# CompVis/stable-diffusion

Hardware: AMD Instinct MI355X
Metric: 512x512 images/sec, SD-v1-4 50-step PLMS CFG=7.5 (higher is better)
Workload: dtype f16

## Files before the change

### include/sdmi.h

```cpp
#ifndef SDMI_H_
#define SDMI_H_

#include <stdint.h>

#ifdef __cplusplus
extern "C" {
#endif

#define SDMI_ABI_VERSION 17

typedef struct sdmi_unet sdmi_unet;

typedef struct sdmi_unet_cfg {
  int32_t in_channels;
  int32_t out_channels;
  int32_t model_channels;
  int32_t num_res_blocks;
  int32_t n_levels;
  int32_t channel_mult[8];
  int32_t n_attention_resolutions;
  int32_t attention_resolutions[8];
  int32_t num_heads;
  int32_t transformer_depth;
  int32_t context_dim;
// ... 87 lines not shown


typedef struct sdmi_clip sdmi_clip;
typedef struct sdmi_clip_cfg {
  int32_t vocab_size;
  int32_t hidden_size;
  int32_t intermediate_size;
  int32_t num_layers;
  int32_t num_heads;
  int32_t max_positions;
} sdmi_clip_cfg;
int sdmi_clip_create(const sdmi_clip_cfg* cfg, sdmi_clip** out);
int sdmi_clip_destroy(sdmi_clip* h);
int sdmi_clip_num_weights(const sdmi_clip* h);
int sdmi_clip_weight_info(const sdmi_clip* h, int idx, char* key_buf, int key_buf_len, int64_t* shape4, int* ndim);
int sdmi_clip_set_weight(sdmi_clip* h, const char* key, const float* ptr, const int64_t* shape, int ndim, void* stream);
int sdmi_clip_finalize(sdmi_clip* h);
int64_t sdmi_clip_workspace_bytes(sdmi_clip* h, int B, int L);
int sdmi_clip_forward(sdmi_clip* h, const int64_t* ids, float* out, int B, int L, void* workspace, int64_t workspace_bytes,
                      void* stream);

typedef struct sdmi_bert sdmi_bert;
typedef struct sdmi_bert_cfg {
  int32_t vocab_size;
  int32_t dim;
  int32_t depth;
  int32_t heads;
  int32_t dim_head;
  int32_t ff_inner;
  int32_t max_seq_len;
} sdmi_bert_cfg;
int sdmi_bert_create(const sdmi_bert_cfg* cfg, sdmi_bert** out);
int sdmi_bert_destroy(sdmi_bert* h);
int sdmi_bert_num_weights(const sdmi_bert* h);
int sdmi_bert_weight_info(const sdmi_bert* h, int idx, char* key_buf, int key_buf_len, int64_t* shape4, int* ndim);
int sdmi_bert_set_weight(sdmi_bert* h, const char* key, const float* ptr, const int64_t* shape, int ndim, void* stream);
int sdmi_bert_finalize(sdmi_bert* h);
int64_t sdmi_bert_workspace_bytes(sdmi_bert* h, int B, int L);
int sdmi_bert_forward(sdmi_bert* h, const int64_t* ids, float* out, int B, int L, void* workspace, int64_t workspace_bytes,
                      void* stream);

typedef struct sdmi_igemm_desc {
  const void* a0; const void* a1; const void* a2;
  int32_t c0, c1, c2, lda0, lda1, lda2;
  int32_t B, Hin, Win, Hout, Wout, ksize, stride, up;
  const void* w;
  int32_t N;
  int32_t mode;
  const float* bias; const float* rowvec; int32_t ld_rowvec;
  const float* residual; int32_t ldr;
  float* out_f32; void* out_f16; int32_t ldo;
  void* seg_dst[3]; int32_t seg_kind[3];
  int32_t heads, dh, ntok, ntok_pad, segC;
  int32_t splitk;
  float* splitk_ws; int64_t splitk_ws_floats;
  int32_t tile;
  int32_t dma;
  int32_t asym_pad;
  int32_t gn_n; void* gn_acc[2]; int32_t gn_cpg[2]; int32_t gn_cbase[2];
  int32_t* splitk_cnt; int32_t splitk_cnt_ints;
  int32_t split16;
  const float* f16_scale; float* lnp_out;
  const float* lnf_part; int32_t lnf_npart; float lnf_eps; const float* lnf_cs; const float* lnf_d;
  const float* pgn_gamma; const float* pgn_beta; float pgn_eps; int32_t pgn_silu;
  void* pgn_out; int32_t pgn_keep_f32; int32_t* pgn_applied;
  void* out_lo;
} sdmi_igemm_desc;
int sdmi_k_igemm(const sdmi_igemm_desc* d, void* stream);
int sdmi_k_ff_tail(const sdmi_igemm_desc* proj_out, const void* ln_f16, const float* lnp, float ln_eps, const float* csd,
                   const void* wgg_f16, const void* wff2_f16, const float* bff2, const float* t, void* stream);
int sdmi_k_st_tail(const sdmi_igemm_desc* proj_out, const void* a_f16, const void* wo_f16, const float* bo, float* t, const float* ln_gamma,
                   float ln_eps, const float* csd, const void* wgg_f16, const void* wff2_f16, const float* bff2, void* stream);
int sdmi_k_gn_conv3(const sdmi_igemm_desc* conv, const float* x0, const float* x1, int c0, int c1, float* gn_ws, int64_t gn_ws_floats,
                    const float* gn_gamma, const float* gn_beta, float gn_eps, void* stream);
int sdmi_k_st_head(const float* x, float* gn_ws, int64_t gn_ws_floats, const float* gn_gamma, const float* gn_beta, float gn_eps,
                   const void* w_in3, const float* b_in, float* t, const float* ln_gamma, float ln_eps, const void* wqkv_f16,
                   const float* lnf_cs, const float* lnf_d, void* q, void* k, void* vt, int B, int ntok, int ntok_pad, int heads, int dh,
                   int C, void* stream);
int sdmi_k_st_mid(const void* a_f16, const void* wo_f16, const float* bo, float* t, const float* ln_gamma, float ln_eps, const void* wq_f16,
                  const float* lnf_cs, const float* lnf_d, void* q, int B, int ntok, int heads, int dh, int C, void* stream);
int sdmi_k_st_mid_ctx(const void* a_f16, const void* wo_f16, const float* bo, float* t, const float* ln_gamma, float ln_eps, const void* wq_f16,
                      const float* lnf_cs, const float* lnf_d, const void* ctx_k, const void* ctx_vt, int nkv, int nkv_pad, float scale, void* ao_out,
                      int B, int ntok, int heads, int dh, int C, void* stream);
int sdmi_k_ln_fold_prep(const void* w_f16, int N, int K, int ldw, const float* gamma, const float* beta, const float* bias,
                        float* cs, float* d, void* stream);
int sdmi_k_attention(const void* q, const void* k, const void* vt, void* out, int BH, int heads, int nq, int nkv,
                     int nkv_pad, int d, float scale, void* stream);
int sdmi_k_attention_split16(const void* q, const void* q_lo, const void* k, const void* k_lo, const void* vt, const void* vt_lo, void* out,
                             void* out_lo, int BH, int heads, int nq, int nkv, int nkv_pad, int d, float scale, void* stream);
int sdmi_k_attention_causal(const void* q, const void* k, const void* vt, void* out, int BH, int heads, int n, int n_pad,
                            int d, float scale, void* stream);
int sdmi_k_groupnorm(const float* x0, const float* x1, int c0, int c1, int B, int HW, const float* gamma,
                     const float* beta, float eps, int silu, void* out_f16, float* out_f32, void* raw_f16, void* out_lo,
                     void* raw_lo, float* partial_ws, int64_t partial_floats, void* stream);
int64_t sdmi_k_groupnorm_ws_floats(int B, int HW);
int sdmi_k_groupnorm_film(const float* x0, const float* x1, int c0, int c1, int B, int HW, const float* gamma, const float* beta, float eps,
                          int silu, const float* film, int film_ld, void* out_f16, float* out_f32, void* raw_f16, void* out_lo, void* raw_lo,
                          float* partial_ws, int64_t partial_floats, void* stream);
int sdmi_k_layernorm(const float* x, const float* gamma, const float* beta, void* out_f16, int M, int C, float eps,
                     void* stream);
int sdmi_k_cast_f16(const float* x, void* out_f16, void* out_lo, int64_t n, void* stream);
int sdmi_k_split_heads(const float* src, int ld, int col0, void* dst, void* dst_lo, int kind, int B, int ntok, int ntok_pad, int heads, int dh,
                       void* stream);
int sdmi_k_geglu_split(const float* src, int M, int F, void* out, void* out_lo, void* stream);
int sdmi_k_layernorm_split(const float* x, const float* gamma, const float* beta, void* out, void* out_lo, int M, int C, float eps, void* stream);
int sdmi_k_timestep_embedding(const int64_t* t_i64, const float* t_f32, float* out, int B, int dim, void* stream);
int sdmi_k_small_linear(const float* in, int ld_in, const float* w, const float* bias, float* out, int ld_out, int B,
                        int N, int K, int silu_in, void* stream);
int sdmi_k_conv_in(const float* x_nchw, const float* w_oihw, const float* bias, float* out_nhwc, int B, int Cin, int H,
                   int W, int Cout, void* stream);
int sdmi_k_conv_out(const float* h_nhwc, const float* w_ohwi, const float* bias, float* out_nchw, int B, int H, int W,
                    int Cin, int Cout, void* stream);
int sdmi_k_pack_conv_weight(const float* w_oihw, void* dst_f16, int O, int I, int KH, int KW, void* stream);
int sdmi_k_pack_conv_weight_src(const float* w_oihw, void* dst_f16, int O, int I, int KH, int KW, int c0, int c1, int c2, void* stream);
int sdmi_k_pack_conv_out(const float* w_oihw, float* dst_ohwi, int O, int I, void* stream);
int sdmi_k_pack_split3(const float* w, void* dst_f16, int N, int K, void* stream);
int sdmi_k_pack_conv_split3(const float* w_oihw, void* dst_f16, int O, int I, int KH, int KW, void* stream);
int sdmi_k_pointwise_nchw(const float* x, const float* w, const float* bias, float* out, int B, int Cin, int Cout, int HW,
                          float in_scale, void* stream);
int sdmi_k_softmax_rows(const float* S, void* P_f16, int rows, int cols, float scale, void* stream);
int sdmi_k_vq_quantize(const float* z, float z_scale, const float* codebook, float* norms_ws, int n_embed, int D, float* zq, int32_t* idx,
                       int B, int HW, void* stream);
int sdmi_k_resample2(const float* x, float* out_f32, void* out_f16, void* out_lo, int B, int H, int W, int C, int dir, void* stream);
int sdmi_k_patch_unfold(const float* x, const float* c, float* out, int B, int Cx, int Cc, int H, int W, int kh, int kw, int sy, int sx,
                        int l0, int nl, void* stream);
int sdmi_k_patch_fold(const float* o, const float* w, float* out, int B, int C, int H, int W, int kh, int kw, int sy, int sx, int uf, int df,
                      int norm_only, void* stream);
int sdmi_k_gelu_erf(const float* x, void* out_f16, int64_t n, void* stream);
int sdmi_k_pack_geglu(const float* w, const float* bias, void* wdst_f16, float* bdst, int N, int K, void* stream);
int sdmi_image_to_uint8(const float* img_nchw, void* out_nhwc_u8, int B, int C, int H, int W, void* stream);
int sdmi_range_check(int enable);
int sdmi_range_report(char* json_buf, int json_buf_len);
int sdmi_tune_begin(void);
int sdmi_tune_round(int r);
int sdmi_tune_end(const char* path, int* n_keys);
int sdmi_tune_dump(char* buf, int buflen);
int sdmi_profile_begin(void);
int sdmi_profile_end(char* json_buf, int json_buf_len);
int sdmi_k_prefetch_lines(const void* ptr, int64_t bytes, void* stream);
const void* sdmi_zero_page(void);

#ifdef __cplusplus
}
#endif
#endif
```

### stable-diffusion_amd/_lib.py

```python
import ctypes as C
import os

_HERE = os.path.dirname(os.path.abspath(__file__))
LIB_PATH = os.environ.get('SDMI_LIB_PATH') or os.path.join(_HERE, 'libsdmi.so')

c_f32p = C.c_void_p
c_ptr = C.c_void_p


class UNetCfg(C.Structure):
    _fields_ = [('in_channels', C.c_int32), ('out_channels', C.c_int32), ('model_channels', C.c_int32),
                ('num_res_blocks', C.c_int32), ('n_levels', C.c_int32), ('channel_mult', C.c_int32 * 8),
                ('n_attention_resolutions', C.c_int32), ('attention_resolutions', C.c_int32 * 8),
                ('num_heads', C.c_int32), ('transformer_depth', C.c_int32), ('context_dim', C.c_int32)]


class VaeCfg(C.Structure):
    _fields_ = [('ch', C.c_int32), ('out_ch', C.c_int32), ('n_levels', C.c_int32), ('ch_mult', C.c_int32 * 8),
                ('num_res_blocks', C.c_int32), ('in_channels', C.c_int32), ('z_channels', C.c_int32),
                ('embed_dim', C.c_int32)]


class UNetExt(C.Structure):
    _fields_ = [('attention_block', C.c_int32), ('resblock_updown', C.c_int32)]
# ... 24 lines not shown
                ('residual', c_ptr), ('ldr', C.c_int32),
                ('out_f32', c_ptr), ('out_f16', c_ptr), ('ldo', C.c_int32),
                ('seg_dst', c_ptr * 3), ('seg_kind', C.c_int32 * 3),
                ('heads', C.c_int32), ('dh', C.c_int32), ('ntok', C.c_int32), ('ntok_pad', C.c_int32),
                ('segC', C.c_int32), ('splitk', C.c_int32), ('splitk_ws', c_ptr), ('splitk_ws_floats', C.c_int64),
                ('tile', C.c_int32), ('dma', C.c_int32), ('asym_pad', C.c_int32),
                ('gn_n', C.c_int32), ('gn_acc', c_ptr * 2), ('gn_cpg', C.c_int32 * 2), ('gn_cbase', C.c_int32 * 2),
                ('splitk_cnt', c_ptr), ('splitk_cnt_ints', C.c_int32), ('split16', C.c_int32),
                ('f16_scale', c_ptr), ('lnp_out', c_ptr), ('lnf_part', c_ptr), ('lnf_npart', C.c_int32),
                ('lnf_eps', C.c_float), ('lnf_cs', c_ptr), ('lnf_d', c_ptr),
                ('pgn_gamma', c_ptr), ('pgn_beta', c_ptr), ('pgn_eps', C.c_float), ('pgn_silu', C.c_int32),
                ('pgn_out', c_ptr), ('pgn_keep_f32', C.c_int32), ('pgn_applied', C.POINTER(C.c_int32)),
                ('out_lo', c_ptr)]


_SIGS = {
    'sdmi_last_error': (C.c_char_p, []),
    'sdmi_abi_version': (C.c_int, []),
    'sdmi_unet_create': (C.c_int, [C.POINTER(UNetCfg), C.POINTER(c_ptr)]),
    'sdmi_unet_create_with_precision': (C.c_int, [C.POINTER(UNetCfg), C.c_int, C.POINTER(c_ptr)]),
    'sdmi_unet_precision': (C.c_int, [c_ptr]),
    'sdmi_unet_create_ext': (C.c_int, [C.POINTER(UNetCfg), C.POINTER(UNetExt), C.c_int, C.POINTER(c_ptr)]),
    'sdmi_unet_create_flags': (C.c_int, [C.POINTER(UNetCfg), C.POINTER(UNetExt), C.c_uint, C.c_int, C.POINTER(c_ptr)]),
    'sdmi_unet_destroy': (C.c_int, [c_ptr]),
    'sdmi_unet_num_weights': (C.c_int, [c_ptr]),
    'sdmi_unet_weight_info': (C.c_int, [c_ptr, C.c_int, C.c_char_p, C.c_int, C.POINTER(C.c_int64), C.POINTER(C.c_int)]),
    'sdmi_unet_set_weight': (C.c_int, [c_ptr, C.c_char_p, c_ptr, C.POINTER(C.c_int64), C.c_int, c_ptr]),
    'sdmi_unet_finalize': (C.c_int, [c_ptr]),
    'sdmi_unet_packed_bytes': (C.c_int64, [c_ptr]),
    'sdmi_unet_export_packed': (C.c_int, [c_ptr, c_ptr, C.c_int64, c_ptr]),
    'sdmi_unet_import_packed': (C.c_int, [c_ptr, c_ptr, C.c_int64, c_ptr]),
    'sdmi_unet_workspace_bytes': (C.c_int64, [c_ptr, C.c_int, C.c_int, C.c_int, C.c_int]),
    'sdmi_unet_cache_context': (C.c_int, [c_ptr, c_ptr, C.c_int, C.c_int, c_ptr, C.c_int64, c_ptr]),
    'sdmi_unet_reserve_context': (C.c_int, [c_ptr, C.c_int, C.c_int]),
    'sdmi_unet_cache_timesteps': (C.c_int, [c_ptr, C.POINTER(C.c_int64), C.c_int, c_ptr]),
    'sdmi_unet_hint_timestep': (C.c_int, [c_ptr, C.c_int64]),
    'sdmi_unet_tape_stats': (C.c_int, [c_ptr, C.POINTER(C.c_int64), C.POINTER(C.c_int64)]),
    'sdmi_unet_forward': (C.c_int, [c_ptr, c_ptr, c_ptr, c_ptr, c_ptr, c_ptr, C.c_int, C.c_int, C.c_int, C.c_int,
                                    c_ptr, C.c_int64, c_ptr]),
    'sdmi_sampler_step': (C.c_int, [c_ptr, C.c_int, C.c_float, c_ptr, C.c_int, c_ptr, c_ptr, c_ptr, C.c_float,
                                    C.c_float, C.c_float, C.c_float, c_ptr, c_ptr, c_ptr, c_ptr, C.c_int64, c_ptr]),
    'sdmi_dpm_solver_step': (C.c_int, [c_ptr, C.c_int, C.c_float, c_ptr, c_ptr, C.c_float, C.c_float, C.c_float, C.c_float,
                                       C.c_float, C.c_int, c_ptr, c_ptr, C.c_int64, c_ptr]),
    'sdmi_vae_create': (C.c_int, [C.POINTER(VaeCfg), C.c_int, C.POINTER(c_ptr)]),
    'sdmi_vae_destroy': (C.c_int, [c_ptr]),
    'sdmi_vae_create_ext': (C.c_int, [C.POINTER(VaeCfg), C.POINTER(VaeExt), C.c_int, C.POINTER(c_ptr)]),
    'sdmi_vae_create_precision': (C.c_int, [C.POINTER(VaeCfg), C.POINTER(VaeExt), C.c_int, C.c_int, C.POINTER(c_ptr)]),
    'sdmi_vae_precision': (C.c_int, [c_ptr]),
    'sdmi_vae_decode_vq': (C.c_int, [c_ptr, c_ptr, C.c_float, C.c_int, c_ptr, C.c_int, C.c_int, C.c_int, c_ptr, C.c_int64, c_ptr]),
    'sdmi_k_vq_quantize': (C.c_int, [c_ptr, C.c_float, c_ptr, c_ptr, C.c_int, C.c_int, c_ptr, c_ptr, C.c_int, C.c_int, c_ptr]),
    'sdmi_k_patch_unfold': (C.c_int, [c_ptr, c_ptr, c_ptr] + [C.c_int] * 11 + [c_ptr]),
    'sdmi_k_patch_fold': (C.c_int, [c_ptr, c_ptr, c_ptr] + [C.c_int] * 11 + [c_ptr]),
    'sdmi_k_resample2': (C.c_int, [c_ptr, c_ptr, c_ptr, c_ptr, C.c_int, C.c_int, C.c_int, C.c_int, C.c_int, c_ptr]),
    'sdmi_vae_num_weights': (C.c_int, [c_ptr]),
    'sdmi_vae_weight_info': (C.c_int, [c_ptr, C.c_int, C.c_char_p, C.c_int, C.POINTER(C.c_int64), C.POINTER(C.c_int)]),
    'sdmi_vae_set_weight': (C.c_int, [c_ptr, C.c_char_p, c_ptr, C.POINTER(C.c_int64), C.c_int, c_ptr]),
    'sdmi_vae_finalize': (C.c_int, [c_ptr]),
    'sdmi_vae_decode_workspace_bytes': (C.c_int64, [c_ptr, C.c_int, C.c_int, C.c_int]),
    'sdmi_vae_decode': (C.c_int, [c_ptr, c_ptr, C.c_float, c_ptr, C.c_int, C.c_int, C.c_int, c_ptr, C.c_int64, c_ptr]),
    'sdmi_vae_encode_workspace_bytes': (C.c_int64, [c_ptr, C.c_int, C.c_int, C.c_int]),
    'sdmi_vae_encode': (C.c_int, [c_ptr, c_ptr, c_ptr, C.c_int, C.c_int, C.c_int, c_ptr, C.c_int64, c_ptr]),
    'sdmi_clip_create': (C.c_int, [C.POINTER(ClipCfg), C.POINTER(c_ptr)]),
    'sdmi_clip_destroy': (C.c_int, [c_ptr]),
    'sdmi_clip_num_weights': (C.c_int, [c_ptr]),
    'sdmi_clip_weight_info': (C.c_int, [c_ptr, C.c_int, C.c_char_p, C.c_int, C.POINTER(C.c_int64), C.POINTER(C.c_int)]),
    'sdmi_clip_set_weight': (C.c_int, [c_ptr, C.c_char_p, c_ptr, C.POINTER(C.c_int64), C.c_int, c_ptr]),
    'sdmi_clip_finalize': (C.c_int, [c_ptr]),
    'sdmi_clip_workspace_bytes': (C.c_int64, [c_ptr, C.c_int, C.c_int]),
    'sdmi_clip_forward': (C.c_int, [c_ptr, c_ptr, c_ptr, C.c_int, C.c_int, c_ptr, C.c_int64, c_ptr]),
    'sdmi_bert_create': (C.c_int, [C.POINTER(BertCfg), C.POINTER(c_ptr)]),
    'sdmi_bert_destroy': (C.c_int, [c_ptr]),
    'sdmi_bert_num_weights': (C.c_int, [c_ptr]),
    'sdmi_bert_weight_info': (C.c_int, [c_ptr, C.c_int, C.c_char_p, C.c_int, C.POINTER(C.c_int64), C.POINTER(C.c_int)]),
    'sdmi_bert_set_weight': (C.c_int, [c_ptr, C.c_char_p, c_ptr, C.POINTER(C.c_int64), C.c_int, c_ptr]),
    'sdmi_bert_finalize': (C.c_int, [c_ptr]),
    'sdmi_bert_workspace_bytes': (C.c_int64, [c_ptr, C.c_int, C.c_int]),
    'sdmi_bert_forward': (C.c_int, [c_ptr, c_ptr, c_ptr, C.c_int, C.c_int, c_ptr, C.c_int64, c_ptr]),
    'sdmi_has_experiments': (C.c_int, []),
    'sdmi_k_igemm': (C.c_int, [C.POINTER(IGemmDesc), c_ptr]),
    'sdmi_k_ff_tail': (C.c_int, [C.POINTER(IGemmDesc), c_ptr, c_ptr, C.c_float, c_ptr, c_ptr, c_ptr, c_ptr, c_ptr, c_ptr]),
    'sdmi_k_gn_conv3': (C.c_int, [C.POINTER(IGemmDesc), c_ptr, c_ptr, C.c_int, C.c_int, c_ptr, C.c_int64, c_ptr, c_ptr, C.c_float, c_ptr]),
    'sdmi_k_st_mid_ctx': (C.c_int, [c_ptr, c_ptr, c_ptr, c_ptr, c_ptr, C.c_float, c_ptr, c_ptr, c_ptr, c_ptr, c_ptr, C.c_int, C.c_int, C.c_float, c_ptr,
                                    C.c_int, C.c_int, C.c_int, C.c_int, C.c_int, c_ptr]),
    'sdmi_k_st_tail': (C.c_int, [C.POINTER(IGemmDesc), c_ptr, c_ptr, c_ptr, c_ptr, c_ptr, C.c_float, c_ptr, c_ptr, c_ptr, c_ptr, c_ptr]),
    'sdmi_k_st_mid': (C.c_int, [c_ptr, c_ptr, c_ptr, c_ptr, c_ptr, C.c_float, c_ptr, c_ptr, c_ptr, c_ptr, C.c_int, C.c_int, C.c_int, C.c_int,
                                C.c_int, c_ptr]),
    'sdmi_k_st_head': (C.c_int, [c_ptr, c_ptr, C.c_int64, c_ptr, c_ptr, C.c_float, c_ptr, c_ptr, c_ptr, c_ptr, C.c_float, c_ptr, c_ptr, c_ptr,
                                 c_ptr, c_ptr, c_ptr, C.c_int, C.c_int, C.c_int, C.c_int, C.c_int, C.c_int, c_ptr]),
    'sdmi_k_attention_split16': (C.c_int, [c_ptr, c_ptr, c_ptr, c_ptr, c_ptr, c_ptr, c_ptr, c_ptr, C.c_int, C.c_int, C.c_int, C.c_int,
                                           C.c_int, C.c_int, C.c_float, c_ptr]),
    'sdmi_k_attention_causal': (C.c_int, [c_ptr, c_ptr, c_ptr, c_ptr, C.c_int, C.c_int, C.c_int, C.c_int, C.c_int, C.c_float,
                                          c_ptr]),
    'sdmi_k_pointwise_nchw': (C.c_int, [c_ptr, c_ptr, c_ptr, c_ptr, C.c_int, C.c_int, C.c_int, C.c_int, C.c_float, c_ptr]),
    'sdmi_k_softmax_rows': (C.c_int, [c_ptr, c_ptr, C.c_int, C.c_int, C.c_float, c_ptr]),
    'sdmi_k_gelu_erf': (C.c_int, [c_ptr, c_ptr, C.c_int64, c_ptr]),
    'sdmi_k_attention': (C.c_int, [c_ptr, c_ptr, c_ptr, c_ptr, C.c_int, C.c_int, C.c_int, C.c_int, C.c_int, C.c_int,
                                   C.c_float, c_ptr]),
    'sdmi_k_groupnorm': (C.c_int, [c_ptr, c_ptr, C.c_int, C.c_int, C.c_int, C.c_int, c_ptr, c_ptr, C.c_float, C.c_int,
                                   c_ptr, c_ptr, c_ptr, c_ptr, c_ptr, c_ptr, C.c_int64, c_ptr]),
    'sdmi_k_groupnorm_ws_floats': (C.c_int64, [C.c_int, C.c_int]),
    'sdmi_k_groupnorm_film': (C.c_int, [c_ptr, c_ptr, C.c_int, C.c_int, C.c_int, C.c_int, c_ptr, c_ptr, C.c_float, C.c_int, c_ptr, C.c_int,
                                        c_ptr, c_ptr, c_ptr, c_ptr, c_ptr, c_ptr, C.c_int64, c_ptr]),
    'sdmi_k_layernorm': (C.c_int, [c_ptr, c_ptr, c_ptr, c_ptr, C.c_int, C.c_int, C.c_float, c_ptr]),
    'sdmi_k_cast_f16': (C.c_int, [c_ptr, c_ptr, c_ptr, C.c_int64, c_ptr]),
    'sdmi_k_split_heads': (C.c_int, [c_ptr, C.c_int, C.c_int, c_ptr, c_ptr, C.c_int, C.c_int, C.c_int, C.c_int, C.c_int, C.c_int,
                                     c_ptr]),
    'sdmi_k_geglu_split': (C.c_int, [c_ptr, C.c_int, C.c_int, c_ptr, c_ptr, c_ptr]),
    'sdmi_k_layernorm_split': (C.c_int, [c_ptr, c_ptr, c_ptr, c_ptr, c_ptr, C.c_int, C.c_int, C.c_float, c_ptr]),
    'sdmi_k_timestep_embedding': (C.c_int, [c_ptr, c_ptr, c_ptr, C.c_int, C.c_int, c_ptr]),
    'sdmi_k_small_linear': (C.c_int, [c_ptr, C.c_int, c_ptr, c_ptr, c_ptr, C.c_int, C.c_int, C.c_int, C.c_int,
                                      C.c_int, c_ptr]),
    'sdmi_k_conv_in': (C.c_int, [c_ptr, c_ptr, c_ptr, c_ptr, C.c_int, C.c_int, C.c_int, C.c_int, C.c_int, c_ptr]),
    'sdmi_k_conv_out': (C.c_int, [c_ptr, c_ptr, c_ptr, c_ptr, C.c_int, C.c_int, C.c_int, C.c_int, C.c_int, c_ptr]),
    'sdmi_k_pack_conv_weight': (C.c_int, [c_ptr, c_ptr, C.c_int, C.c_int, C.c_int, C.c_int, c_ptr]),
    'sdmi_k_pack_conv_weight_src': (C.c_int, [c_ptr, c_ptr, C.c_int, C.c_int, C.c_int, C.c_int, C.c_int, C.c_int, C.c_int, c_ptr]),
    'sdmi_k_pack_conv_out': (C.c_int, [c_ptr, c_ptr, C.c_int, C.c_int, c_ptr]),
    'sdmi_k_pack_split3': (C.c_int, [c_ptr, c_ptr, C.c_int, C.c_int, c_ptr]),
    'sdmi_k_pack_conv_split3': (C.c_int, [c_ptr, c_ptr, C.c_int, C.c_int, C.c_int, C.c_int, c_ptr]),
    'sdmi_k_pack_geglu': (C.c_int, [c_ptr, c_ptr, c_ptr, c_ptr, C.c_int, C.c_int, c_ptr]),
    'sdmi_k_ln_fold_prep': (C.c_int, [c_ptr, C.c_int, C.c_int, C.c_int, c_ptr, c_ptr, c_ptr, c_ptr, c_ptr, c_ptr]),
    'sdmi_image_to_uint8': (C.c_int, [c_ptr, c_ptr, C.c_int, C.c_int, C.c_int, C.c_int, c_ptr]),
    'sdmi_range_check': (C.c_int, [C.c_int]),
    'sdmi_range_report': (C.c_int, [C.c_char_p, C.c_int]),
    'sdmi_tune_begin': (C.c_int, []),
    'sdmi_tune_round': (C.c_int, [C.c_int]),
    'sdmi_tune_end': (C.c_int, [C.c_char_p, C.POINTER(C.c_int)]),
    'sdmi_tune_dump': (C.c_int, [C.c_char_p, C.c_int]),
    'sdmi_profile_begin': (C.c_int, []),
    'sdmi_profile_end': (C.c_int, [C.c_char_p, C.c_int]),
    'sdmi_k_prefetch_lines': (C.c_int, [c_ptr, C.c_int64, c_ptr]),
    'sdmi_zero_page': (c_ptr, []),
}

_lib = None


class SdmiError(RuntimeError):
    pass


def load():
    global _lib
    if _lib is None:
        if not os.path.exists(LIB_PATH):
            raise SdmiError(f'{LIB_PATH} not found: build it with `python stable-diffusion_amd/build.py` '
                            '(the MI355X path has no fallback implementation)')
        lib = C.CDLL(LIB_PATH)
        for name, (res, args) in _SIGS.items():
            fn = getattr(lib, name)
            fn.restype = res
            fn.argtypes = args
        if lib.sdmi_abi_version() != 17:
            raise SdmiError('libsdmi ABI version mismatch')
        _lib = lib
    return _lib


def exported_symbols():
    return sorted(_SIGS)


def check(rc):
    if rc != 0:
        raise SdmiError(load().sdmi_last_error().decode('utf-8', 'replace'))


# ... 8 lines not shown
```

### stable-diffusion_amd/build.py

```python
import concurrent.futures as cf
import hashlib
import os
import subprocess
import sys

HERE = os.path.dirname(os.path.abspath(__file__))
CSRC = os.path.join(HERE, 'csrc')
EXTRA = os.environ.get('SDMI_CXXFLAGS', '').split()
LIB = os.path.join(HERE, os.environ.get('SDMI_LIB_OUT', 'libsdmi.so'))
OBJ = os.path.join(HERE, 'build' if os.path.basename(LIB) == 'libsdmi.so' else 'build_' + os.path.splitext(os.path.basename(LIB))[0])
SOURCES = ['igemm_t1.hip', 'igemm_t0.hip', 'igemm_t2.hip', 'igemm_h1.hip', 'igemm_h0.hip', 'igemm_h2.hip', 'igemm.hip', 'conv3halo.hip', 'gemm_split16.hip', 'rowchain.hip', 'gnconv.hip', 'range.hip', 'attn.hip', 'attn_wide.hip', 'attn_split16.hip', 'attn_wide_split16.hip', 'split_ops.hip', 'norm.hip', 'small.hip', 'sampler.hip', 'inpaint.hip', 'patch.hip', 'weights.cpp', 'unet.cpp', 'vae.cpp', 'clip.cpp', 'bert.cpp', 'api.cpp', 'prof.cpp']
FLAGS = ['--offload-arch=gfx950', '-O3', '-std=c++17', '-fPIC', '-munsafe-fp-atomics', '-Wall', '-Wno-unused-function',
         '-Wno-unused-variable']


def _hipcc():
    for c in (os.environ.get('HIPCC'), '/opt/rocm/bin/hipcc', 'hipcc'):
        if c and (not os.path.isabs(c) or os.path.exists(c)):
            return c
    raise RuntimeError('hipcc not found')


def _stamp():
    h = hashlib.sha256()
    for root in (CSRC, os.path.join(os.path.dirname(HERE), 'include')):
        for fn in sorted(os.listdir(root)):
            with open(os.path.join(root, fn), 'rb') as f:
                h.update(fn.encode())
                h.update(f.read())
    h.update(' '.join(FLAGS + EXTRA).encode())
    return h.hexdigest()


def is_current():
    stamp_file = os.path.join(OBJ, 'stamp')
    return os.path.exists(LIB) and os.path.exists(stamp_file) and open(stamp_file).read() == _stamp()


def build(force=False, verbose=True):
    os.makedirs(OBJ, exist_ok=True)
    stamp_file = os.path.join(OBJ, 'stamp')
    if not force and is_current():
        return LIB
    hipcc = _hipcc()
    stamp_now = _stamp()

    inc_dirs = (CSRC, os.path.join(os.path.dirname(HERE), 'include'))

    def deps_hash(src):
        import re
        seen, todo, h = set(), [os.path.join(CSRC, src)], hashlib.sha256()
        while todo:
            path = todo.pop()
            if path in seen:
                continue
            seen.add(path)
            with open(path, 'rb') as f:
                data = f.read()
            h.update(os.path.basename(path).encode())
            h.update(data)
            for inc in re.findall(rb'^\s*#\s*include\s*"([^"]+)"', data, re.M):
                for d in (os.path.dirname(path),) + inc_dirs:
                    cand = os.path.join(d, inc.decode())
                    if os.path.exists(cand):
                        todo.append(os.path.normpath(cand))
                        break
        return h.hexdigest()

    def compile_one(src):
        obj = os.path.join(OBJ, os.path.splitext(src)[0] + '.o')
        extra = ['-ffp-contract=off'] if src == 'sampler.hip' else []
        cmd = [hipcc] + FLAGS + EXTRA + extra + (['-x', 'hip'] if src.endswith('.hip') else []) + ['-c', os.path.join(CSRC, src), '-o', obj]
        key = hashlib.sha256((deps_hash(src) + ' '.join(cmd)).encode()).hexdigest()
        if not force and os.path.exists(obj) and os.path.exists(obj + '.key') and open(obj + '.key').read() == key:
            return obj
        r = subprocess.run(cmd, capture_output=True, text=True)
        if r.returncode != 0:
            raise RuntimeError(f'hipcc failed for {src}:\n{r.stdout}\n{r.stderr}')
        if verbose and r.stderr.strip():
            print(r.stderr, file=sys.stderr)
        with open(obj + '.key', 'w') as f:
            f.write(key)
        return obj

    with cf.ThreadPoolExecutor(max_workers=min(8, len(SOURCES))) as ex:
        objs = list(ex.map(compile_one, SOURCES))
    cmd = [hipcc, '--offload-arch=gfx950', '-shared', '-fPIC', '-o', LIB] + objs
    r = subprocess.run(cmd, capture_output=True, text=True)
    if r.returncode != 0:
        raise RuntimeError(f'link failed:\n{r.stdout}\n{r.stderr}')
    with open(stamp_file, 'w') as f:
        f.write(stamp_now)
    if verbose:
        print(f'built {LIB} ({os.path.getsize(LIB) / 1e6:.1f} MB)')
# ... 6 lines not shown
```

### stable-diffusion_amd/csrc/api.cpp

```cpp
#include <string.h>

#include <new>

#include "prof.h"
#include "split16.h"
#include "unet.h"
#include "vae.h"
#include "clip.h"

namespace sdmi {
static thread_local std::string g_err;
void set_error(const std::string& msg) { g_err = msg; }
int fail(const std::string& msg) { g_err = msg; return -1; }
}

struct sdmi_unet { sdmi::UNet impl; };
struct sdmi_vae { sdmi::Vae impl; };
struct sdmi_clip { sdmi::ClipText impl; };
struct sdmi_bert { sdmi::BertText impl; };

using namespace sdmi;

static int weight_info(const WeightStore& w, int idx, char* key_buf, int key_buf_len, int64_t* shape4, int* ndim) {
  SDMI_CHECK(key_buf && shape4 && ndim, "null argument");
// ... 319 lines not shown
  p.pgn_out = (f16*)d->pgn_out; p.pgn_keep_f32 = d->pgn_keep_f32; p.pgn_applied = d->pgn_applied;
  p.out_lo = (f16*)d->out_lo;
  return zero_page(&p.zero_page);
}
int sdmi_k_igemm(const sdmi_igemm_desc* d, void* stream) {
  SDMI_CHECK(d, "null descriptor");
  IGemmParams p = IGemmParams();
  if (igemm_params_of(d, p)) return -1;
  IGemmTune t; t.tile = d->tile; t.dma = d->dma;
  return launch_igemm(p, t, (hipStream_t)stream);
}
int sdmi_k_ff_tail(const sdmi_igemm_desc* proj_out, const void* ln_f16, const float* lnp, float ln_eps, const float* csd,
                   const void* wgg_f16, const void* wff2_f16, const float* bff2, const float* t, void* stream) {
  SDMI_CHECK(proj_out, "null descriptor");
  FfTailParams q = FfTailParams();
  if (igemm_params_of(proj_out, q.epi)) return -1;
  SDMI_CHECK(proj_out->split16 && proj_out->ksize == 1, "ff_tail: the proj_out descriptor is a split-fp16 1x1 (w = sdmi_k_pack_split3)");
  q.ln = (const f16*)ln_f16; q.lnp = lnp; q.ln_eps = ln_eps; q.csd = csd; q.wgg = (const f16*)wgg_f16; q.wff2 = (const f16*)wff2_f16;
  q.bff2 = bff2; q.t = t; q.wpo = (const f16*)proj_out->w;
  return launch_ff_tail(q, (hipStream_t)stream);
}
int sdmi_k_st_tail(const sdmi_igemm_desc* proj_out, const void* a_f16, const void* wo_f16, const float* bo, float* t, const float* ln_gamma,
                   float ln_eps, const float* csd, const void* wgg_f16, const void* wff2_f16, const float* bff2, void* stream) {
  SDMI_CHECK(proj_out && a_f16, "null argument");
  FfTailParams q = FfTailParams();
  if (igemm_params_of(proj_out, q.epi)) return -1;
  SDMI_CHECK(proj_out->split16 && proj_out->ksize == 1, "st_tail: the proj_out descriptor is a split-fp16 1x1 (w = sdmi_k_pack_split3)");
  q.a16 = (const f16*)a_f16; q.wo = (const f16*)wo_f16; q.bo = bo; q.ln_gamma = ln_gamma; q.ln_eps = ln_eps; q.csd = csd;
  q.wgg = (const f16*)wgg_f16; q.wff2 = (const f16*)wff2_f16; q.bff2 = bff2; q.t = t; q.wpo = (const f16*)proj_out->w;
  return launch_ff_tail(q, (hipStream_t)stream);
}
int sdmi_k_gn_conv3(const sdmi_igemm_desc* conv, const float* x0, const float* x1, int c0, int c1, float* gn_ws, int64_t gn_ws_floats,
                    const float* gn_gamma, const float* gn_beta, float gn_eps, void* stream) {
  SDMI_CHECK(conv && x0 && gn_ws && gn_gamma && gn_beta, "gn_conv3: null argument");
  GnConvParams q = GnConvParams();
  if (igemm_params_of(conv, q.epi)) return -1;
  const int B = q.epi.B;
  SDMI_CHECK(gn_ws_floats >= gn_acc_words(B) * 2, "groupnorm workspace too small");
  SDMI_HIP_OK(hipMemsetAsync(gn_ws, 0, gn_acc_words(B) * sizeof(long long), (hipStream_t)stream));
  GroupNormParams g = GroupNormParams();
  g.x0 = x0; g.c0 = c0; g.x1 = x1; g.c1 = c1; g.B = B; g.HW = q.epi.Hout * q.epi.Wout; g.gamma = gn_gamma; g.beta = gn_beta; g.eps = gn_eps;
  g.stats_only = 1; g.acc = (long long*)gn_ws;
  if (launch_groupnorm(g, (hipStream_t)stream)) return -1;
  q.x0 = x0; q.x1 = x1; q.c0 = c0; q.c1 = c1; q.gn_acc = (const long long*)gn_ws; q.gn_gamma = gn_gamma; q.gn_beta = gn_beta; q.gn_eps = gn_eps;
  q.w = (const f16*)conv->w;
  return launch_gn_conv3(q, (hipStream_t)stream);
}
int sdmi_k_st_head(const float* x, float* gn_ws, int64_t gn_ws_floats, const float* gn_gamma, const float* gn_beta, float gn_eps,
                   const void* w_in3, const float* b_in, float* t, const float* ln_gamma, float ln_eps, const void* wqkv_f16,
                   const float* lnf_cs, const float* lnf_d, void* q, void* k, void* vt, int B, int ntok, int ntok_pad, int heads, int dh,
                   int C, void* stream) {
  SDMI_CHECK(x && gn_ws && gn_gamma && gn_beta, "st_head: null argument");
  SDMI_CHECK(gn_ws_floats >= gn_acc_words(B) * 2, "groupnorm workspace too small");
  SDMI_HIP_OK(hipMemsetAsync(gn_ws, 0, gn_acc_words(B) * sizeof(long long), (hipStream_t)stream));
  GroupNormParams g = GroupNormParams();
  g.x0 = x; g.c0 = C; g.B = B; g.HW = ntok; g.gamma = gn_gamma; g.beta = gn_beta; g.eps = gn_eps; g.stats_only = 1; g.acc = (long long*)gn_ws;
  if (launch_groupnorm(g, (hipStream_t)stream)) return -1;
  StHeadParams p = StHeadParams();
  p.x = x; p.gn_acc = (const long long*)gn_ws; p.gn_gamma = gn_gamma; p.gn_beta = gn_beta; p.gn_eps = gn_eps;
  p.w_in = (const f16*)w_in3; p.b_in = b_in; p.t = t; p.ln_gamma = ln_gamma; p.ln_eps = ln_eps; p.wqkv = (const f16*)wqkv_f16;
  p.lnf_cs = lnf_cs; p.lnf_d = lnf_d; p.q = (f16*)q; p.k = (f16*)k; p.vt = (f16*)vt;
  p.M = B * ntok; p.B = B; p.ntok = ntok; p.ntok_pad = ntok_pad; p.heads = heads; p.dh = dh; p.C = C;
  return launch_st_head(p, (hipStream_t)stream);
}
int sdmi_k_st_mid(const void* a_f16, const void* wo_f16, const float* bo, float* t, const float* ln_gamma, float ln_eps, const void* wq_f16,
                  const float* lnf_cs, const float* lnf_d, void* q, int B, int ntok, int heads, int dh, int C, void* stream) {
  StHeadParams p = StHeadParams();
  p.a16 = (const f16*)a_f16; p.w_in = (const f16*)wo_f16; p.b_in = bo; p.t = t; p.ln_gamma = ln_gamma; p.ln_eps = ln_eps;
  p.wqkv = (const f16*)wq_f16; p.lnf_cs = lnf_cs; p.lnf_d = lnf_d; p.q = (f16*)q;
  p.M = B * ntok; p.B = B; p.ntok = ntok; p.ntok_pad = ntok; p.heads = heads; p.dh = dh; p.C = C;
  return launch_st_mid(p, (hipStream_t)stream);
}
int sdmi_k_st_mid_ctx(const void* a_f16, const void* wo_f16, const float* bo, float* t, const float* ln_gamma, float ln_eps, const void* wq_f16,
                      const float* lnf_cs, const float* lnf_d, const void* ctx_k, const void* ctx_vt, int nkv, int nkv_pad, float scale, void* ao_out,
                      int B, int ntok, int heads, int dh, int C, void* stream) {
  StHeadParams p = StHeadParams();
  p.a16 = (const f16*)a_f16; p.w_in = (const f16*)wo_f16; p.b_in = bo; p.t = t; p.ln_gamma = ln_gamma; p.ln_eps = ln_eps;
  p.wqkv = (const f16*)wq_f16; p.lnf_cs = lnf_cs; p.lnf_d = lnf_d;
  p.ctx_k = (const f16*)ctx_k; p.ctx_vt = (const f16*)ctx_vt; p.ctx_nkv = nkv; p.ctx_nkv_pad = nkv_pad; p.ctx_scale = scale; p.ao_out = (f16*)ao_out;
  SDMI_CHECK(ctx_k && ctx_vt && ao_out, "st_mid_ctx: null argument");
  p.M = B * ntok; p.B = B; p.ntok = ntok; p.ntok_pad = ntok; p.heads = heads; p.dh = dh; p.C = C;
  return launch_st_mid(p, (hipStream_t)stream);
}
int sdmi_k_ln_fold_prep(const void* w_f16, int N, int K, int ldw, const float* gamma, const float* beta, const float* bias,
                        float* cs, float* d, void* stream) {
  return launch_ln_fold_prep((const f16*)w_f16, N, K, ldw, gamma, beta, bias, cs, d, (hipStream_t)stream);
}
int sdmi_k_attention(const void* q, const void* k, const void* vt, void* out, int BH, int heads, int nq, int nkv,
                     int nkv_pad, int d, float scale, void* stream) {
  AttnParams a = AttnParams();
  a.q = (const f16*)q; a.k = (const f16*)k; a.vt = (const f16*)vt; a.out = (f16*)out;
  a.BH = BH; a.heads = heads; a.nq = nq; a.nkv = nkv; a.nkv_pad = nkv_pad; a.d = d; a.scale = scale;
  if (const char* e = getenv("SDMI_ATTN_NW")) a.nw = atoi(e);
  return launch_attention(a, (hipStream_t)stream);
}
int sdmi_k_attention_split16(const void* q, const void* q_lo, const void* k, const void* k_lo, const void* vt, const void* vt_lo, void* out,
                             void* out_lo, int BH, int heads, int nq, int nkv, int nkv_pad, int d, float scale, void* stream) {
  AttnSplitParams a = AttnSplitParams();
  a.q = (const f16*)q; a.q_lo = (const f16*)q_lo; a.k = (const f16*)k; a.k_lo = (const f16*)k_lo; a.vt = (const f16*)vt;
  a.vt_lo = (const f16*)vt_lo; a.out = (f16*)out; a.out_lo = (f16*)out_lo;
  a.BH = BH; a.heads = heads; a.nq = nq; a.nkv = nkv; a.nkv_pad = nkv_pad; a.d = d; a.scale = scale;
  return launch_attention_split16(a, (hipStream_t)stream);
}
int64_t sdmi_k_groupnorm_ws_floats(int B, int HW) { (void)HW; return gn_acc_words(B) * 2; }
int sdmi_k_groupnorm(const float* x0, const float* x1, int c0, int c1, int B, int HW, const float* gamma,
                     const float* beta, float eps, int silu, void* out_f16, float* out_f32, void* raw_f16, void* out_lo,
                     void* raw_lo, float* partial_ws, int64_t partial_floats, void* stream) {
  SDMI_CHECK(partial_floats >= gn_acc_words(B) * 2, "groupnorm workspace too small");
  SDMI_HIP_OK(hipMemsetAsync(partial_ws, 0, gn_acc_words(B) * sizeof(long long), (hipStream_t)stream));
  GroupNormParams g = GroupNormParams();
  g.x0 = x0; g.x1 = x1; g.c0 = c0; g.c1 = c1; g.B = B; g.HW = HW; g.gamma = gamma; g.beta = beta; g.eps = eps;
  g.silu = silu; g.out_f16 = (f16*)out_f16; g.out_f32 = out_f32; g.raw_f16 = (f16*)raw_f16; g.out_lo = (f16*)out_lo; g.raw_lo = (f16*)raw_lo;
  g.acc = (long long*)partial_ws;
  return launch_groupnorm(g, (hipStream_t)stream);
}
int sdmi_k_groupnorm_film(const float* x0, const float* x1, int c0, int c1, int B, int HW, const float* gamma, const float* beta, float eps,
                          int silu, const float* film, int film_ld, void* out_f16, float* out_f32, void* raw_f16, void* out_lo, void* raw_lo,
                          float* partial_ws, int64_t partial_floats, void* stream) {
  SDMI_CHECK(partial_floats >= gn_acc_words(B) * 2, "groupnorm workspace too small");
  SDMI_HIP_OK(hipMemsetAsync(partial_ws, 0, gn_acc_words(B) * sizeof(long long), (hipStream_t)stream));
  GroupNormParams g = GroupNormParams();
  g.x0 = x0; g.x1 = x1; g.c0 = c0; g.c1 = c1; g.B = B; g.HW = HW; g.gamma = gamma; g.beta = beta; g.eps = eps;
  g.silu = silu; g.out_f16 = (f16*)out_f16; g.out_f32 = out_f32; g.raw_f16 = (f16*)raw_f16; g.out_lo = (f16*)out_lo; g.raw_lo = (f16*)raw_lo;
  g.film = film; g.film_ld = film_ld;
  g.acc = (long long*)partial_ws;
  return launch_groupnorm(g, (hipStream_t)stream);
}
int sdmi_k_layernorm(const float* x, const float* gamma, const float* beta, void* out_f16, int M, int C, float eps,
                     void* stream) {
  return launch_layernorm(x, gamma, beta, (f16*)out_f16, M, C, eps, (hipStream_t)stream);
}
int sdmi_k_cast_f16(const float* x, void* out_f16, void* out_lo, int64_t n, void* stream) {
  return launch_cast_f16(x, (f16*)out_f16, (f16*)out_lo, n, (hipStream_t)stream);
}
int sdmi_k_split_heads(const float* src, int ld, int col0, void* dst, void* dst_lo, int kind, int B, int ntok, int ntok_pad, int heads, int dh,
                       void* stream) {
  return launch_split_heads(src, ld, col0, (f16*)dst, (f16*)dst_lo, kind, B, ntok, ntok_pad, heads, dh, (hipStream_t)stream);
}
int sdmi_k_geglu_split(const float* src, int M, int F, void* out, void* out_lo, void* stream) {
  return launch_geglu_split(src, M, F, (f16*)out, (f16*)out_lo, (hipStream_t)stream);
}
int sdmi_k_layernorm_split(const float* x, const float* gamma, const float* beta, void* out, void* out_lo, int M, int C, float eps, void* stream) {
  return launch_layernorm_split(x, gamma, beta, (f16*)out, (f16*)out_lo, M, C, eps, (hipStream_t)stream);
}
int sdmi_k_timestep_embedding(const int64_t* t_i64, const float* t_f32, float* out, int B, int dim, void* stream) {
  return launch_timestep_embedding(t_i64, t_f32, out, B, dim, (hipStream_t)stream);
}
int sdmi_k_small_linear(const float* in, int ld_in, const float* w, const float* bias, float* out, int ld_out, int B,
                        int N, int K, int silu_in, void* stream) {
  return launch_small_linear(in, ld_in, w, bias, out, ld_out, B, N, K, silu_in, (hipStream_t)stream);
}
int sdmi_k_conv_in(const float* x, const float* w, const float* bias, float* out, int B, int Cin, int H, int W, int Cout,
                   void* stream) {
  return launch_conv_in(x, w, bias, out, B, Cin, H, W, Cout, (hipStream_t)stream);
}
int sdmi_k_conv_out(const float* h, const float* w, const float* bias, float* out, int B, int H, int W, int Cin, int Cout,
                    void* stream) {
  return launch_conv_out(h, w, bias, out, B, H, W, Cin, Cout, (hipStream_t)stream);
}
int sdmi_k_pack_conv_weight(const float* w, void* dst, int O, int I, int KH, int KW, void* stream) {
  return launch_pack_conv_weight(w, (f16*)dst, O, I, KH, KW, (hipStream_t)stream);
}
int sdmi_k_pack_conv_weight_src(const float* w, void* dst, int O, int I, int KH, int KW, int c0, int c1, int c2, void* stream) {
  return launch_pack_conv_weight_src(w, (f16*)dst, O, I, KH, KW, c0, c1, c2, (hipStream_t)stream);
}
int sdmi_k_pack_conv_out(const float* w, float* dst, int O, int I, void* stream) {
// ... 55 lines not shown
```

### stable-diffusion_amd/csrc/common.h

```cpp
#pragma once
#include <hip/hip_runtime.h>
#include <stdint.h>
#include <algorithm>
#include <string>

#include "tape.h"

typedef _Float16 f16;
typedef _Float16 f16x2 __attribute__((ext_vector_type(2)));
typedef _Float16 f16x4 __attribute__((ext_vector_type(4)));
typedef _Float16 f16x8 __attribute__((ext_vector_type(8)));
typedef float f32x4 __attribute__((ext_vector_type(4)));
typedef float f32x16 __attribute__((ext_vector_type(16)));

#ifdef __HIPCC__
__device__ __forceinline__ float gn_apply_elem(float v, float mean, float rstd, float gamma, float beta, int silu) {
  float t = __builtin_fmaf((v - mean) * rstd, gamma, beta);
  if (silu) t = t * __builtin_amdgcn_rcpf(1.0f + __expf(-t));
  return t;
}
__device__ __forceinline__ float gn_apply_film_elem(float v, float mean, float rstd, float gamma, float beta, float scale, float shift,
                                                    int silu) {
  float t = __builtin_fmaf((v - mean) * rstd, gamma, beta);
  t = __builtin_fmaf(t, 1.0f + scale, shift);
// ... 135 lines not shown
  unsigned long long gn_magic[2] = {0, 0};
  const float* pgn_gamma = nullptr; const float* pgn_beta = nullptr; float pgn_eps = 1e-5f; int pgn_silu = 1;
  f16* pgn_out = nullptr;
  int pgn_keep_f32 = 0;
  int* pgn_applied = nullptr;
  unsigned long long magic_hw = 0, magic_w = 0, magic_w2 = 0;
  int log2w = 0;
  const float* xf0 = nullptr; const float* xf1 = nullptr;
  const long long* gn_in_acc = nullptr;
  const float* gn_in_gamma = nullptr; const float* gn_in_beta = nullptr; float gn_in_eps = 1e-5f; int gn_in_silu = 1;
  f16* raw_hi = nullptr; f16* raw_lo = nullptr;
  f16* gn_scratch = nullptr;
  unsigned long long magic_cpg_in = 0;
  int halo_thi = 0, halo_ipt = 1, log2_tpi = 30;
  unsigned long long magic_hpi = 0;
};

constexpr int SDMI_NUM_TILES = 22;
struct IGemmTune {
  int tile = -1;
  int dma = -1;
};

int launch_igemm(const IGemmParams& p, const IGemmTune& tune, hipStream_t stream);
bool range_check_enabled();
uint64_t tune_generation();
bool tune_collecting();
int range_check_set(int enable);
int range_scan(const char* what, const f16* p, int64_t n, hipStream_t stream);
int range_report(std::string* json);

int tune_begin();
int tune_round(int r);
int tune_end(const char* path, int* n_keys);
int tune_dump(std::string* out);
int launch_splitk_reduce(const IGemmParams& p, int nsplit, hipStream_t stream);

struct FfTailParams {
  const f16* ln = nullptr;
  const float* lnp = nullptr;
  float ln_eps = 1e-5f;
  const float* csd = nullptr;
  const f16* wgg = nullptr;
  const f16* wff2 = nullptr;
  const float* bff2 = nullptr;
  const float* t = nullptr;
  const f16* wpo = nullptr;
  const f16* a16 = nullptr;
  const f16* wo = nullptr;
  const float* bo = nullptr;
  const float* ln_gamma = nullptr;
#ifdef SDMI_RC_TIMING
  long long* dbg = nullptr;
#endif
  IGemmParams epi;
};
bool ff_tail_supported(int C, int M, int rows_per_sample);
int launch_ff_tail(const FfTailParams& p, hipStream_t stream);

struct StHeadParams {
  const f16* a16 = nullptr;
  const float* x = nullptr;
  const long long* gn_acc = nullptr;
  const float* gn_gamma = nullptr; const float* gn_beta = nullptr; float gn_eps = 1e-6f;
  const f16* w_in = nullptr;
  const float* b_in = nullptr;
  float* t = nullptr;
  const float* ln_gamma = nullptr;
  float ln_eps = 1e-5f;
  const f16* wqkv = nullptr;
  const float* lnf_cs = nullptr; const float* lnf_d = nullptr;
  f16* q = nullptr; f16* k = nullptr;
  f16* vt = nullptr;
  int M = 0, B = 0, ntok = 0, ntok_pad = 0, heads = 0, dh = 0, C = 0;
  const f16* ctx_k = nullptr; const f16* ctx_vt = nullptr; int ctx_nkv = 0, ctx_nkv_pad = 0; float ctx_scale = 0.f; f16* ao_out = nullptr;
#ifdef SDMI_RC_TIMING
  long long* dbg = nullptr;
#endif
};
bool st_head_supported(int C, int M, int ntok, int ntok_pad, int heads, int dh);
int launch_st_head(const StHeadParams& p, hipStream_t stream);
int launch_st_mid(const StHeadParams& p, hipStream_t stream);

struct GnConvParams {
  const float* x0 = nullptr; const float* x1 = nullptr; int c0 = 0, c1 = 0;
  const long long* gn_acc = nullptr;
  const float* gn_gamma = nullptr; const float* gn_beta = nullptr; float gn_eps = 1e-5f;
  const f16* w = nullptr;
#ifdef SDMI_RC_TIMING
  long long* dbg = nullptr;
#endif
  IGemmParams epi;
};
bool gn_conv3_supported(int B, int H, int W, int c0, int c1, int Cout);
int launch_gn_conv3(const GnConvParams& p, hipStream_t stream);

struct AttnParams {
  const f16* q = nullptr;
  const f16* k = nullptr;
  const f16* vt = nullptr;
  f16* out = nullptr;
  int BH = 0, heads = 0, nq = 0, nkv = 0, nkv_pad = 0, d = 0;
  float scale = 1.f;
  int nw = 0;
  int causal = 0;
  int prio = 0;
  int pingpong = 0;
};
int launch_attention(const AttnParams& p, hipStream_t stream);
int launch_attention_wide(const AttnParams& p, hipStream_t stream);

struct GroupNormParams {
  const float* x0 = nullptr; const float* x1 = nullptr; int c0 = 0, c1 = 0;
  int B = 0, HW = 0;
  const float* gamma = nullptr; const float* beta = nullptr; float eps = 1e-5f;
  int silu = 0;
  int stats_only = 0;
  int skip_stats = 0;
  f16* out_f16 = nullptr;
  float* out_f32 = nullptr;
  f16* raw_f16 = nullptr;
  f16* out_lo = nullptr;
  f16* raw_lo = nullptr;
  const float* film = nullptr; int film_ld = 0;
  long long* acc = nullptr;
};
constexpr int GN_SLOTS = 8;
constexpr int GN_MAX_CALLS = 96;
constexpr int GN_WORDS = 4;
constexpr int GN_STRIDE = 16;
static inline int64_t gn_acc_words(int B) { return (int64_t)B * 32 * GN_SLOTS * GN_STRIDE; }
int launch_groupnorm(const GroupNormParams& p, hipStream_t stream);

int launch_layernorm(const float* x, const float* gamma, const float* beta, f16* out, int M, int C, float eps,
                     hipStream_t stream, float* out_f32 = nullptr);
int launch_cast_f16(const float* x, f16* out, f16* out_lo, int64_t n, hipStream_t stream);

int launch_timestep_embedding(const int64_t* t_i64, const float* t_f32, float* out, int B, int dim, hipStream_t s);
int launch_small_linear(const float* in, int ld_in, const float* w, const float* bias, float* out, int ld_out,
                        int B, int N, int K, int silu_in, hipStream_t s);
int launch_ctx1_broadcast(const f16* vt, int ld_v, f16* ao, int B, int ntok, int C, hipStream_t s);
int launch_conv_in(const float* x_nchw, const float* w, const float* bias, float* out_nhwc, int B, int Cin, int H,
                   int W, int Cout, hipStream_t s, int gn_n = 0, long long* const* gn_acc = nullptr, const int* gn_cpg = nullptr,
                   const int* gn_cbase = nullptr);
int launch_conv_out(const float* h_nhwc, const float* w_khwc, const float* bias, float* out_nchw, int B, int H, int W,
                    int Cin, int Cout, hipStream_t s);

struct DpmStepParams {
  const float* eps_model = nullptr;
  int cfg = 0; float scale = 1.f;
  const float* x = nullptr;
  const float* m_prev = nullptr;
  float alpha_s = 1.f, sigma_s = 0.f;
  float cx = 1.f, a = 0.f, inv_r0 = 0.f;
  int order = 1;
  float* m_out = nullptr;
  float* x_next = nullptr;
  int64_t n = 0;
};
int launch_dpm_step(const DpmStepParams& p, hipStream_t s);

int launch_embed_tokens(const int64_t* ids, const float* tok_emb, const float* pos_emb, float* out, int M, int L, int C,
                        int vocab, hipStream_t s);
int launch_quick_gelu(const float* x, f16* out, int64_t n, hipStream_t s);
int launch_gelu_erf(const float* x, f16* out, int64_t n, hipStream_t s);

// ... 43 lines not shown
```

### stable-diffusion_amd/csrc/igemm_dev.h

```cpp
#pragma once
#include "common.h"
#include "prof.h"

namespace sdmi {
typedef unsigned u32x4 __attribute__((ext_vector_type(4)));

int launch_splitk_reduce(const IGemmParams& p, int nsplit, hipStream_t stream);
int launch_generic_tile_g0(int tile, const IGemmParams& p, bool dma, int splitk, hipStream_t stream);
int launch_generic_tile_g1(int tile, const IGemmParams& p, bool dma, int splitk, hipStream_t stream);
int launch_generic_tile_g2(int tile, const IGemmParams& p, bool dma, int splitk, hipStream_t stream);
int launch_generic_tile_h0(int tile, const IGemmParams& p, bool dma, int splitk, hipStream_t stream);
int launch_generic_tile_h1(int tile, const IGemmParams& p, bool dma, int splitk, hipStream_t stream);
int launch_generic_tile_h2(int tile, const IGemmParams& p, bool dma, int splitk, hipStream_t stream);

static int env_int(const char* name, int dflt) {
  const char* v = getenv(name);
  return v ? atoi(v) : dflt;
}

namespace {

constexpr int BK = 64;
constexpr int BKH = 32;
static inline int src_chunks(int c) { return (c + BK - 1) / BK; }
// ... 23 lines not shown
#define SDMI_VMCNT_CASE(k) case k: asm volatile("s_waitcnt vmcnt(" #k ")" ::: "memory"); break
    SDMI_VMCNT_CASE(0); SDMI_VMCNT_CASE(1); SDMI_VMCNT_CASE(2); SDMI_VMCNT_CASE(3); SDMI_VMCNT_CASE(4);
    SDMI_VMCNT_CASE(5); SDMI_VMCNT_CASE(6); SDMI_VMCNT_CASE(7); SDMI_VMCNT_CASE(8); SDMI_VMCNT_CASE(9);
    SDMI_VMCNT_CASE(10); SDMI_VMCNT_CASE(11); SDMI_VMCNT_CASE(12); SDMI_VMCNT_CASE(13); SDMI_VMCNT_CASE(14);
    SDMI_VMCNT_CASE(15); SDMI_VMCNT_CASE(16); SDMI_VMCNT_CASE(17); SDMI_VMCNT_CASE(18); SDMI_VMCNT_CASE(19);
    SDMI_VMCNT_CASE(20); SDMI_VMCNT_CASE(21); SDMI_VMCNT_CASE(22); SDMI_VMCNT_CASE(23); SDMI_VMCNT_CASE(24);
    SDMI_VMCNT_CASE(25); SDMI_VMCNT_CASE(26); SDMI_VMCNT_CASE(27); SDMI_VMCNT_CASE(28); SDMI_VMCNT_CASE(29);
    SDMI_VMCNT_CASE(30); SDMI_VMCNT_CASE(31); SDMI_VMCNT_CASE(32); SDMI_VMCNT_CASE(33); SDMI_VMCNT_CASE(34);
    SDMI_VMCNT_CASE(35); SDMI_VMCNT_CASE(36); SDMI_VMCNT_CASE(37); SDMI_VMCNT_CASE(38); SDMI_VMCNT_CASE(39);
    SDMI_VMCNT_CASE(40); SDMI_VMCNT_CASE(41); SDMI_VMCNT_CASE(42); SDMI_VMCNT_CASE(43); SDMI_VMCNT_CASE(44);
    SDMI_VMCNT_CASE(45); SDMI_VMCNT_CASE(46); SDMI_VMCNT_CASE(47); SDMI_VMCNT_CASE(48);
#undef SDMI_VMCNT_CASE
    default: __builtin_trap();
  }
}
template <int N>
__device__ __forceinline__ void wait_vmcnt() {
  static_assert(N >= 0 && N <= 48, "add the literal");
  wait_vmcnt_n(N);
}

enum : int { KIND_1X1 = 0, KIND_3X3 = 1, KIND_3X3_UP = 2 };

__device__ __forceinline__ int fast_div(int m, unsigned long long magic) {
  return (int)(((unsigned long long)(unsigned)m * magic) >> 40);
}
__device__ __forceinline__ int fast_div_hw(int m, unsigned long long magic) {
  return (int)(((unsigned long long)(unsigned)m * magic) >> 48);
}

#if defined(__HIP_DEVICE_COMPILE__)
template <int WTN> constexpr int SLAB_LPR = WTN / 4;
template <int WTN> constexpr int SLAB_RPI = 64 / (WTN / 4);
template <int WTN> constexpr int SLAB_NPASS = 32 / (64 / (WTN / 4));
template <int NWAVES, int WTN, int LDS_BYTES>
constexpr int SLAB_LSTR = (NWAVES * 32 * (WTN + 4) * 4 <= LDS_BYTES) ? WTN + 4 : WTN;
template <int NWAVES, int WTN, int LDS_BYTES>
__device__ __forceinline__ float* slab_base(unsigned char* smem, int wave) {
  static_assert(WTN == 32 || WTN == 64, "lane mapping of the 16-byte epilogue");
  static_assert(NWAVES * 32 * SLAB_LSTR<NWAVES, WTN, LDS_BYTES> * 4 <= LDS_BYTES, "LDS too small for the epilogue slabs");
  return (float*)smem + wave * (32 * SLAB_LSTR<NWAVES, WTN, LDS_BYTES>);
}
template <int TN, int LSTR>
__device__ __forceinline__ void slab_put(float* wl, const f32x16 (&a)[TN], int l31, int lg) {
#pragma unroll
  for (int j = 0; j < TN; ++j)
#pragma unroll
    for (int r = 0; r < 16; ++r) wl[((r & 3) + 8 * (r >> 2) + 4 * lg) * LSTR + j * 32 + l31] = a[j][r];
  asm volatile("s_waitcnt lgkmcnt(0)" ::: "memory");
}
template <int TN, int LSTR>
__device__ __forceinline__ void slab_get(const float* wl, f32x16 (&a)[TN], int l31, int lg) {
  asm volatile("s_waitcnt lgkmcnt(0)" ::: "memory");
#pragma unroll
  for (int j = 0; j < TN; ++j)
#pragma unroll
    for (int r = 0; r < 16; ++r) a[j][r] = wl[((r & 3) + 8 * (r >> 2) + 4 * lg) * LSTR + j * 32 + l31];
  asm volatile("s_waitcnt lgkmcnt(0)" ::: "memory");
}

constexpr int LNF_MAXP = 40;
__device__ __forceinline__ void lnf_request(const IGemmParams& p, int m, float2 (&pv)[LNF_MAXP]) {
  const float2* src = (const float2*)p.lnf_part + m;
#pragma unroll
  for (int j = 0; j < 20; ++j) pv[j] = src[(size_t)min(j, p.lnf_npart - 1) * p.M];
  if (p.lnf_npart > 20) {
#pragma unroll
    for (int j = 20; j < LNF_MAXP; ++j) pv[j] = src[(size_t)min(j, p.lnf_npart - 1) * p.M];
  } else {
#pragma unroll
    for (int j = 20; j < LNF_MAXP; ++j) pv[j] = float2{0.f, 0.f};
  }
}
__device__ __forceinline__ void lnf_finish(const IGemmParams& p, const float2 (&pv)[LNF_MAXP], float* mean, float* rstd) {
  float s = 0.f, q = 0.f;
#pragma unroll
  for (int j = 0; j < LNF_MAXP; ++j)
    if (j < p.lnf_npart) { s += pv[j].x; q += pv[j].y; }
  const float inv_c = 1.0f / (32.0f * (float)p.lnf_npart);
  const float mu = s * inv_c;
  const float var = fmaxf(q * inv_c - mu * mu, 0.f);
  *mean = mu;
  *rstd = 1.0f / sqrtf(var + p.lnf_eps);
}
__device__ __forceinline__ float sum8_dpp(float v) {
  v += __builtin_bit_cast(float, __builtin_amdgcn_update_dpp(0, __builtin_bit_cast(int, v), 0xB1, 0xF, 0xF, true));
  v += __builtin_bit_cast(float, __builtin_amdgcn_update_dpp(0, __builtin_bit_cast(int, v), 0x4E, 0xF, 0xF, true));
  v += __builtin_bit_cast(float, __builtin_amdgcn_update_dpp(0, __builtin_bit_cast(int, v), 0x141, 0xF, 0xF, true));
  return v;
}

template <int BM, int BN, int WARPS_M, int WARPS_N, int LDS_BYTES>
__device__ __forceinline__ void igemm_epilogue(const IGemmParams& p_arg, f32x16 (&acc)[BM / WARPS_M / 32][BN / WARPS_N / 32],
                                               const int m0, const int n0, const int split, const int tile_m,
                                               const int tile_n, unsigned char* smem, const float lnf_mean = 0.f,
                                               const float lnf_rstd = 1.f) {
#ifdef SDMI_IGEMM_TIMING
  IGemmParams p = p_arg;
  if (p.dbg_abl & 1) p.residual = nullptr;
  if (p.dbg_abl & 4) { p.out_f32 = nullptr; p.out_f16 = nullptr; p.out_lo = nullptr; }
#else
  const IGemmParams& p = p_arg;
#endif
  constexpr int NT = WARPS_M * WARPS_N * 64;
  constexpr int WTM = BM / WARPS_M, WTN = BN / WARPS_N;
  constexpr int TM = WTM / 32, TN = WTN / 32;
  constexpr int LSTR = SLAB_LSTR<WARPS_M * WARPS_N, WTN, LDS_BYTES>;
  const int tid = threadIdx.x;
  const int lane = tid & 63;
  const int wave = tid >> 6;
  const int wm = wave / WARPS_N, wn = wave - wm * WARPS_N;
  const int l31 = lane & 31, lg = lane >> 5;
  const int HWout = p.Hout * p.Wout;
  const int mw = m0 + wm * WTM, nw = n0 + wn * WTN;
  const bool full = (m0 + BM <= p.M) && (n0 + BN <= p.N);
  if (p.splitk > 1 && p.splitk_fused) {
    constexpr int SC1 = 16;
    const int tile_lin = tile_m * ((p.N + BN - 1) / BN) + tile_n;
    const __amdgpu_buffer_rsrc_t ws = __builtin_amdgcn_make_buffer_rsrc(
        (void*)(p.splitk_ws + (size_t)tile_lin * p.splitk * (BM * BN)), 0, p.splitk * (BM * BN) * 4, 0x00020000);
    const int my_off = (split * (BM * BN) + tid * 4) * 4;
#pragma unroll
    for (int i = 0; i < TM; ++i)
#pragma unroll
      for (int j = 0; j < TN; ++j)
#pragma unroll
        for (int r4 = 0; r4 < 4; ++r4) {
          const f32x4 v = {acc[i][j][4 * r4], acc[i][j][4 * r4 + 1], acc[i][j][4 * r4 + 2], acc[i][j][4 * r4 + 3]};
          __builtin_amdgcn_raw_buffer_store_b128(__builtin_bit_cast(u32x4, v), ws, my_off + ((i * TN + j) * 4 + r4) * (NT * 16), 0, SC1);
        }
    asm volatile("s_waitcnt vmcnt(0)" ::: "memory");
    __syncthreads();
    if (tid == 0) *(volatile int*)smem = __hip_atomic_fetch_add(p.splitk_cnt + tile_lin, 1, __ATOMIC_RELAXED, __HIP_MEMORY_SCOPE_AGENT);
    __syncthreads();
    const int ticket = *(volatile int*)smem;
    if (ticket != p.splitk - 1) return;
    if (tid == 0) __hip_atomic_store(p.splitk_cnt + tile_lin, 0, __ATOMIC_RELAXED, __HIP_MEMORY_SCOPE_AGENT);
#pragma unroll
    for (int i = 0; i < TM; ++i)
#pragma unroll
      for (int j = 0; j < TN; ++j)
#pragma unroll
        for (int r = 0; r < 16; ++r) acc[i][j][r] = 0.f;
    constexpr int QPS = TM * TN * 4;
    constexpr int SB = QPS >= 16 ? 1 : 16 / QPS;
    for (int s0 = 0; s0 < p.splitk; s0 += SB) {
      f32x4 v[SB][QPS];
#pragma unroll
      for (int ss = 0; ss < SB; ++ss) {
        const int off = (min(s0 + ss, p.splitk - 1) * (BM * BN) + tid * 4) * 4;
#pragma unroll
        for (int e = 0; e < QPS; ++e)
          v[ss][e] = __builtin_bit_cast(f32x4, __builtin_amdgcn_raw_buffer_load_b128(ws, off + e * (NT * 16), 0, SC1));
      }
#pragma unroll
      for (int ss = 0; ss < SB; ++ss) {
        if (s0 + ss < p.splitk) {
#pragma unroll
          for (int i = 0; i < TM; ++i)
#pragma unroll
            for (int j = 0; j < TN; ++j)
#pragma unroll
              for (int r4 = 0; r4 < 4; ++r4)
#pragma unroll
                for (int e = 0; e < 4; ++e) acc[i][j][4 * r4 + e] += v[ss][(i * TN + j) * 4 + r4][e];
        }
      }
    }
    __syncthreads();
  }
  if (p.splitk > 1 && !p.splitk_fused && p.slab_tiled) {
    constexpr int SC1 = 16;
    const int tiles_n_all = (p.N + BN - 1) / BN, ntiles = ((p.M + BM - 1) / BM) * tiles_n_all;
    const int tile_lin = tile_m * tiles_n_all + tile_n;
    const __amdgpu_buffer_rsrc_t ws = __builtin_amdgcn_make_buffer_rsrc(
        (void*)(p.splitk_ws + ((size_t)split * ntiles + tile_lin) * (size_t)(BM * BN)), 0, BM * BN * 4, 0x00020000);
#pragma unroll
    for (int i = 0; i < TM; ++i)
#pragma unroll
      for (int j = 0; j < TN; ++j)
#pragma unroll
        for (int r4 = 0; r4 < 4; ++r4) {
          const f32x4 v = {acc[i][j][4 * r4], acc[i][j][4 * r4 + 1], acc[i][j][4 * r4 + 2], acc[i][j][4 * r4 + 3]};
          __builtin_amdgcn_raw_buffer_store_b128(__builtin_bit_cast(u32x4, v), ws, (tid * 4 + ((i * TN + j) * 4 + r4) * (NT * 4)) * 4, 0, SC1);
        }
    return;
  }
  if (p.lnf_part) {
    __syncthreads();
    float2* const tab = (float2*)smem;
    if (tid < BM) tab[tid] = float2{lnf_mean, lnf_rstd};
    __syncthreads();
#pragma unroll
    for (int j = 0; j < TN; ++j) {
      const int n = min(nw + j * 32 + l31, p.N - 1);
      const float cs = p.lnf_cs[n], dn = p.lnf_d[n];
#pragma unroll
      for (int i = 0; i < TM; ++i)
#pragma unroll
        for (int r = 0; r < 16; ++r) {
          const float2 mr = tab[wm * WTM + i * 32 + (r & 3) + 8 * (r >> 2) + 4 * lg];
          acc[i][j][r] = fmaf(mr.y, acc[i][j][r] - mr.x * cs, dn);
        }
    }
    __syncthreads();
  }
  const bool unfused_split = p.splitk > 1 && !p.splitk_fused;
  if (p.mode == EPI_PLAIN) {
    const bool atomic = unfused_split;
    float* slab = atomic ? (p.splitk_ws + (size_t)split * p.M * p.N) : nullptr;
    const int b_first = m0 / HWout;
    const bool one_batch = ((m0 + BM - 1) / HWout == b_first);
    if (full && one_batch && p.epi_vec && !atomic) {
      __syncthreads();
      float* const wl = slab_base<WARPS_M * WARPS_N, WTN, LDS_BYTES>(smem, wave);
      const int rl = lane / SLAB_LPR<WTN>, c4 = (lane % SLAB_LPR<WTN>) * 4;
      f32x4 colv = {0.f, 0.f, 0.f, 0.f};
      if (p.bias) colv = *(const f32x4*)(p.bias + nw + c4);
      if (p.rowvec) colv += *(const f32x4*)(p.rowvec + (size_t)b_first * p.ld_rowvec + nw + c4);
      f32x4 g4 = {1.f, 1.f, 1.f, 1.f};
      if (p.f16_scale) g4 = *(const f32x4*)(p.f16_scale + nw + c4);
#pragma unroll
      for (int i = 0; i < TM; ++i) {
        slab_put<TN, LSTR>(wl, acc[i], l31, lg);
        constexpr int NP = SLAB_NPASS<WTN>, RPI = SLAB_RPI<WTN>;
        f32x4 resv[NP];
        if (p.residual) {
#pragma unroll
          for (int q = 0; q < NP; ++q)
            resv[q] = *(const f32x4*)(p.residual + (size_t)(mw + i * 32 + q * RPI + rl) * p.ldr + nw + c4);
        } else {
#pragma unroll
          for (int q = 0; q < NP; ++q) resv[q] = f32x4{0.f, 0.f, 0.f, 0.f};
        }
#pragma unroll
        for (int q = 0; q < NP; ++q) {
          const int row = q * RPI + rl;
          float* const lp = wl + row * LSTR + c4;
          const f32x4 v = *(const f32x4*)lp + colv + resv[q];
          const size_t ro = (size_t)(mw + i * 32 + row) * p.ldo + nw + c4;
          if (p.out_f32) SDMI_ST_F32X4(p.out_f32, ro, v);
          const f32x4 vs = v * g4;
          const f16x4 h = {(f16)vs[0], (f16)vs[1], (f16)vs[2], (f16)vs[3]};
          if (p.out_f16) SDMI_ST_F16X4(p.out_f16, ro, h);
          if (p.out_lo)
            *(f16x4*)(p.out_lo + ro) = f16x4{(f16)(v[0] - (float)h[0]), (f16)(v[1] - (float)h[1]), (f16)(v[2] - (float)h[2]),
                                            (f16)(v[3] - (float)h[3])};
          if (p.lnp_out) {
            float s1 = (v[0] + v[1]) + (v[2] + v[3]);
            float s2 = (v[0] * v[0] + v[1] * v[1]) + (v[2] * v[2] + v[3] * v[3]);
            s1 = sum8_dpp(s1); s2 = sum8_dpp(s2);
            if ((lane & 7) == 0)
              *(float2*)(p.lnp_out + 2 * ((size_t)((nw + c4) >> 5) * p.M + (size_t)(mw + i * 32 + row))) = float2{s1, s2};
          }
          if (p.gn_n > 0) *(f32x4*)lp = v;
        }
        if (p.gn_n > 0) slab_get<TN, LSTR>(wl, acc[i], l31, lg);
        else asm volatile("s_waitcnt lgkmcnt(0)" ::: "memory");
      }
    } else if (full && one_batch) {
      if (atomic) {
#pragma unroll
        for (int i = 0; i < TM; ++i)
#pragma unroll
          for (int r = 0; r < 16; ++r) {
            float* row = slab + (size_t)(mw + i * 32 + (r & 3) + 8 * (r >> 2) + 4 * lg) * p.N + nw + l31;
#pragma unroll
            for (int j = 0; j < TN; ++j) row[j * 32] = acc[i][j][r];
          }
      } else {
        float colv[TN];
#pragma unroll
        for (int j = 0; j < TN; ++j) {
          const int n = nw + j * 32 + l31;
          colv[j] = p.bias ? p.bias[n] : 0.f;
          if (p.rowvec) colv[j] += p.rowvec[(size_t)b_first * p.ld_rowvec + n];
        }
#pragma unroll
        for (int i = 0; i < TM; ++i) {
          float resv[16][TN];
          if (p.residual) {
#pragma unroll
            for (int r = 0; r < 16; ++r) {
              const float* row = p.residual + (size_t)(mw + i * 32 + (r & 3) + 8 * (r >> 2) + 4 * lg) * p.ldr + nw + l31;
#pragma unroll
// ... 322 lines not shown
```

### stable-diffusion_amd/csrc/rowchain.hip

```cpp
#include <utility>

#include "igemm_dev.h"

namespace sdmi {
namespace {

constexpr int RC_ROWS = 32;
constexpr int RC_NWC = 5;
constexpr int RC_NTC = RC_NWC * 64;
constexpr int RC_UROWS = 160;
constexpr int RC_UNIT = RC_UROWS * 128;
constexpr int RC_UPIECES = RC_UNIT / 1024;
constexpr int RC_NS = 4;
constexpr int RC_NLD_DEFAULT = 2;
#ifndef SDMI_RC_PFD
#define SDMI_RC_PFD 24
#endif
constexpr int RC_PFD = SDMI_RC_PFD;
#if defined(__HIP_DEVICE_COMPILE__)
__device__ __forceinline__ int rc_pf_row(int lane, int* sector) {
  const int ntiles = gridDim.x, bid = blockIdx.x;
  const bool ok = (ntiles & 7) == 0;
  const int nslots = ok ? max(ntiles >> 3, 10) : 1, slot = ok ? (bid >> 3) : 1;
  const int idx = slot + (lane >> 2) * nslots;
  *sector = (lane & 3) * 32;
  return (slot < nslots && idx < 160) ? 64 * (idx >> 5) + (idx & 31) : -1;
}
#endif

constexpr int FT_C = 320, FT_KT = FT_C / 64, FT_HID = 4 * FT_C, FT_NCHUNK = 4;
constexpr int FT_BLK = 2 * FT_KT;
constexpr int FT_NU = (3 * FT_NCHUNK) * FT_BLK + 2 * FT_BLK;
constexpr int FT_NUH = FT_NU + FT_BLK;
struct FtUnitTab {
  int soff[FT_NUH];
  int sel[FT_NUH];
  int aux[FT_NUH];
};
constexpr FtUnitTab ft_make_tab() {
  FtUnitTab t{};
  int u = 0;
  for (int i = 0; i < FT_NUH; ++i) t.aux[i] = -1;
  for (int kt = 0; kt < FT_KT; ++kt)
    for (int half = 0; half < 2; ++half) { t.soff[u] = (32 * half) * (FT_C * 2) + kt * 128; t.sel[u] = 3; ++u; }
  for (int h = 0; h <= FT_NCHUNK; ++h) {
    if (h < FT_NCHUNK) {
      for (int pass = 0; pass < 2; ++pass) {
        if (pass == 1 && h + 1 < FT_NCHUNK) t.aux[u] = h + 1;
        for (int kt = 0; kt < FT_KT; ++kt)
          for (int half = 0; half < 2; ++half) { t.soff[u] = (2 * FT_C * h + FT_C * pass + 32 * half) * (FT_C * 2) + kt * 128; t.sel[u] = 0; ++u; }
      }
    } else {
      t.aux[u] = -2;
    }
    if (h >= 1)
      for (int kt = 0; kt < FT_KT; ++kt)
        for (int half = 0; half < 2; ++half) { t.soff[u] = (32 * half) * (FT_HID * 2) + (FT_C * (h - 1) + 64 * kt) * 2; t.sel[u] = 1; ++u; }
  }
  for (int kt = 0; kt < FT_KT; ++kt)
    for (int half = 0; half < 2; ++half)
      for (int lo = 0; lo < 2; ++lo) { t.soff[u] = (32 * half) * (3 * FT_C * 2) + (64 * kt + (lo ? 2 * FT_C : 0)) * 2; t.sel[u] = 2; ++u; }
  return t;
}
__device__ const FtUnitTab kFtTab = ft_make_tab();

#if defined(__HIP_DEVICE_COMPILE__)
__device__ __forceinline__ int strip_off(int row, int col) {
  return (col >> 6) * (RC_ROWS * 128) + row * 128 + (((((col & 63) >> 3)) ^ ((row >> 1) & 7)) << 4) + (col & 7) * 2;
}
template <int... I, class F>
__device__ __forceinline__ void rc_static_for_impl(std::integer_sequence<int, I...>, F&& f) { (f(std::integral_constant<int, I>{}), ...); }
template <int N, class F>
__device__ __forceinline__ void rc_static_for(F&& f) { rc_static_for_impl(std::make_integer_sequence<int, N>{}, f); }
#endif

template <int C, int NLD, int ABL = 0, int NS = RC_NS, bool HEAD = false, bool PF = false>
__global__ void __launch_bounds__(RC_NTC + 64 * NLD + (PF ? 64 : 0)) ff_tail_kernel(const FfTailParams rp) {
#if defined(__HIP_DEVICE_COMPILE__)
  static_assert(C == FT_C, "unit geometry: five waves x 64 columns = C; the unit table is generated for it");
  constexpr int KT = C / 64;
  constexpr int XBYTES = RC_ROWS * C * 2;
  constexpr int HID = 4 * C, NCHUNK = HID / C;
  constexpr int NU = HEAD ? FT_NUH : FT_NU;
  constexpr int TB = HEAD ? 0 : FT_BLK;
// ... 270 lines not shown
    zero2(accA);
    block(OFF_XA, accA[0], accA[1], [&](auto uc) {
      if constexpr (HEAD && decltype(uc)::value == 0) { if (h == 0) ln_table(); }
      if (h > 0) geglu_rows(uc, accB[0], accB[1], h - 1, 1);
    });
    zero2(accB);
    block(OFF_XA, accB[0], accB[1], [&](auto uc) { geglu_rows(uc, accA[0], accA[1], h, 0); });
    if (h > 0) block(OFF_XG + ((h - 1) & 1) * XBYTES, acc2[0], acc2[1], [&](auto uc) { if (h == NCHUNK - 1) geglu_rows(uc, accB[0], accB[1], h, 1); });
  }
  float T[2][16], bff[2];
#pragma unroll
  for (int j = 0; j < 2; ++j) {
    const int col = wave * 64 + j * 32 + l31;
    bff[j] = rp.bff2[col];
#pragma unroll
    for (int r = 0; r < 16; ++r) T[j][r] = rp.t[(size_t)(m0 + (r & 3) + 8 * (r >> 2) + 4 * lg) * C + col];
  }
  block(OFF_XG + ((NCHUNK - 1) & 1) * XBYTES, acc2[0], acc2[1], no_carry);
  wait_vmcnt<0>();
  if constexpr (ABL != 1) {
#pragma unroll
    for (int j = 0; j < 2; ++j) {
      const int col = wave * 64 + j * 32 + l31;
#pragma unroll
      for (int r = 0; r < 16; ++r) {
        const int row = (r & 3) + 8 * (r >> 2) + 4 * lg;
        const float v = acc2[j][r] + bff[j] + T[j][r];
        const f16 hi = (f16)v;
        const int o = strip_off(row, col);
        *(f16*)(smem + OFF_XA + o) = hi;
        *(f16*)(smem + OFF_XG + o) = (f16)(v - (float)hi);
      }
    }
  }
  RC_STAMP();
  f32x16 acc[1][2];
  zero2(acc[0]);
  rc_static_for<KT>([&](auto ktc) {
    constexpr int kt = decltype(ktc)::value;
    f16x8 ah[4], al[4];
    rc_static_for<2>([&](auto hc) {
      constexpr int half = decltype(hc)::value;
      f16x8 bh[4], bl[4];
      unit_sync();
      if constexpr (ABL != 1) {
#pragma unroll
        for (int ks = 0; ks < 4; ++ks) bh[ks] = frag(cur * RC_UNIT + b_frag, ks);
        if constexpr (half == 0) {
#pragma unroll
          for (int ks = 0; ks < 4; ++ks) {
            ah[ks] = frag(OFF_XA + kt * (RC_ROWS * 128) + a_frag, ks);
            al[ks] = frag(OFF_XG + kt * (RC_ROWS * 128) + a_frag, ks);
          }
        }
      }
      unit_end();
      unit_sync();
      if constexpr (ABL != 1) {
#pragma unroll
        for (int ks = 0; ks < 4; ++ks) bl[ks] = frag(cur * RC_UNIT + b_frag, ks);
#pragma unroll
        for (int ks = 0; ks < 4; ++ks) {
          acc[0][half] = __builtin_amdgcn_mfma_f32_32x32x16_f16(ah[ks], bh[ks], acc[0][half], 0, 0, 0);
          acc[0][half] = __builtin_amdgcn_mfma_f32_32x32x16_f16(al[ks], bh[ks], acc[0][half], 0, 0, 0);
          acc[0][half] = __builtin_amdgcn_mfma_f32_32x32x16_f16(ah[ks], bl[ks], acc[0][half], 0, 0, 0);
        }
      }
      unit_end();
    });
    RC_STAMP();
  });
  asm volatile("s_waitcnt lgkmcnt(0)\n\ts_barrier" ::: "memory");
  RC_STAMP();
  igemm_epilogue<RC_ROWS, C, 1, RC_NWC, RING>(ep, acc, m0, 0, 0, (int)blockIdx.x, 0, smem);
#ifdef SDMI_RC_TIMING
  RC_STAMP();
  __syncthreads();
  if (rp.dbg && tid < 128) rp.dbg[(size_t)blockIdx.x * 128 + tid] = tid < n_stamp ? ((const long long*)(smem + OFF_DBG))[tid] : 0;
#endif
#endif
}


typedef float f32x2 __attribute__((ext_vector_type(2)));
#if defined(__HIP_DEVICE_COMPILE__)
__device__ __forceinline__ void rc_swap_halves(float& a, float& b) {
  asm volatile("s_nop 1\n\tv_permlane32_swap_b32 %0, %1\n\ts_nop 1" : "+v"(a), "+v"(b));
}
__device__ __forceinline__ float rc_max_across_halves(float x) {
  float a = x, b = x;
  rc_swap_halves(a, b);
  return fmaxf(a, b);
}
#endif
constexpr int SH_NU = 2 * FT_BLK + 3 * FT_BLK;
struct ShUnitTab { int soff[2][SH_NU]; int sel[2][SH_NU]; };
constexpr ShUnitTab sh_make_tab() {
  ShUnitTab t{};
  int u = 0;
  for (int kt = 0; kt < FT_KT; ++kt)
    for (int half = 0; half < 2; ++half)
      for (int lo = 0; lo < 2; ++lo) { t.soff[0][u] = (32 * half) * (3 * FT_C * 2) + (64 * kt + (lo ? 2 * FT_C : 0)) * 2; t.sel[0][u] = 0; ++u; }
  for (int b = 0; b < 3; ++b)
    for (int kt = 0; kt < FT_KT; ++kt)
      for (int half = 0; half < 2; ++half) { t.soff[0][u] = (FT_C * b + 32 * half) * (FT_C * 2) + kt * 128; t.sel[0][u] = 1; ++u; }
  u = 0;
  for (int b = 0; b < 2; ++b)
    for (int kt = 0; kt < FT_KT; ++kt)
      for (int half = 0; half < 2; ++half) { t.soff[1][u] = (32 * half) * (FT_C * 2) + kt * 128; t.sel[1][u] = b; ++u; }
  for (; u < SH_NU; ++u) { t.soff[1][u] = t.soff[1][2 * FT_BLK - 1]; t.sel[1][u] = 1; }
  return t;
}
__device__ const ShUnitTab kShTab = sh_make_tab();

template <int C, int NLD, int KIND, int NS = RC_NS, bool PF = false, bool CTX = false>
__global__ void __launch_bounds__(RC_NTC + 64 * NLD + (PF ? 64 : 0)) st_head_kernel(const StHeadParams rp) {
#if defined(__HIP_DEVICE_COMPILE__)
  static_assert(C == FT_C, "unit geometry: five waves x 64 columns = C");
  static_assert(NLD == 1 || NLD == 2, "loader waves");
  constexpr int KT = C / 64;
  constexpr int XBYTES = RC_ROWS * C * 2;
  constexpr int NU = KIND == 0 ? SH_NU : 2 * FT_BLK;
  constexpr int NU1 = KIND == 0 ? 2 * FT_BLK : FT_BLK;
  constexpr int RING = NS * RC_UNIT;
  constexpr int OFF_XH = RING, OFF_XL = OFF_XH + XBYTES, OFF_XN = OFF_XL + XBYTES;
  constexpr int OFF_GTAB = OFF_XN + XBYTES;
  constexpr int OFF_LTAB = OFF_GTAB + 32 * 8;
  constexpr int OFF_LNP = OFF_LTAB + RC_ROWS * 8;
  constexpr int OFF_PF = OFF_LNP + RC_ROWS * (C / 32) * 8;
  constexpr int LDS_TOTAL = OFF_PF + (PF ? 256 : 0);
  constexpr int LSTR = 64;
  static_assert(RC_NWC * 32 * LSTR * 4 <= 2 * XBYTES, "the epilogue slabs live in the (dead) proj_in operand strips");
  constexpr int LPIECES = RC_UPIECES / NLD, LD_WAIT = LPIECES * (NS - 2);
  static_assert(NS >= 3 && LD_WAIT + LPIECES <= 63 && LD_WAIT <= 48, "vmcnt is a 6-bit counter");
#ifdef SDMI_RC_TIMING
  constexpr int OFF_DBG = LDS_TOTAL;
  static_assert(LDS_TOTAL + 1024 <= 160 * 1024, "LDS budget");
  __shared__ __attribute__((aligned(16))) unsigned char smem[LDS_TOTAL + 1024];
  int n_stamp = 0;
#else
  static_assert(LDS_TOTAL <= 160 * 1024, "LDS budget");
  __shared__ __attribute__((aligned(16))) unsigned char smem[LDS_TOTAL];
#endif
  const int tid = threadIdx.x;
  const int lane = tid & 63, wave = tid >> 6;
  const int wave_u = __builtin_amdgcn_readfirstlane(wave);
  const int m0 = blockIdx.x * RC_ROWS;
  constexpr int OOB = (int)0x80000000;

  if (PF && wave_u == RC_NWC + NLD) {
    const __amdgpu_buffer_rsrc_t rs_in = __builtin_amdgcn_make_buffer_rsrc((void*)rp.w_in, 0, OOB, 0x00020000);
    const __amdgpu_buffer_rsrc_t rs_qkv = __builtin_amdgcn_make_buffer_rsrc((void*)rp.wqkv, 0, OOB, 0x00020000);
    int sector;
    const int prow = rc_pf_row(lane, &sector);
    const int v_c = prow >= 0 ? prow * (C * 2) + sector : OOB, v_3 = prow >= 0 ? prow * (3 * C * 2) + sector : OOB;
    auto touch = [&](int u) {
      if (u >= NU) return;
      const int soff = __builtin_amdgcn_readfirstlane(kShTab.soff[KIND][u]);
      const int sel = __builtin_amdgcn_readfirstlane(kShTab.sel[KIND][u]);
      __builtin_amdgcn_raw_ptr_buffer_load_lds(sel == 0 ? rs_in : rs_qkv, (__attribute__((address_space(3))) void*)(smem + OFF_PF), 4,
                                               (KIND == 0 && sel == 0) ? v_3 : v_c, soff, 0, 0);
    };
    for (int u = NS - 1; u < RC_PFD; ++u) touch(u);
    asm volatile("s_barrier" ::: "memory");
    for (int g = 0; g < NU; ++g) {
      if (g == NU1) asm volatile("s_barrier" ::: "memory");
      asm volatile("s_barrier" ::: "memory");
      touch(g + RC_PFD);
    }
    wait_vmcnt<0>();
    asm volatile("s_barrier" ::: "memory");
    return;
  }
  if (wave_u >= RC_NWC) {
    const int lw = wave_u - RC_NWC;
    const __amdgpu_buffer_rsrc_t rs_in = __builtin_amdgcn_make_buffer_rsrc((void*)rp.w_in, 0, OOB, 0x00020000);
    const __amdgpu_buffer_rsrc_t rs_qkv = __builtin_amdgcn_make_buffer_rsrc((void*)rp.wqkv, 0, OOB, 0x00020000);
// ... 150 lines not shown
#pragma unroll
      for (int ks = 0; ks < 4; ++ks) a[1] = __builtin_amdgcn_mfma_f32_32x32x16_f16(fa[ks], fb[ks], a[1], 0, 0, 0);
      unit_end();
    });
  };
  auto nothing = []() {};
  f32x16 acc[2];
  zero2(acc);
  if constexpr (KIND == 1) block(acc, OFF_XH, nothing);
  if constexpr (KIND == 0)
  rc_static_for<KT>([&](auto ktc) {
    constexpr int kt = decltype(ktc)::value;
    f16x8 ah[4], al[4];
    rc_static_for<2>([&](auto hc) {
      constexpr int half = decltype(hc)::value;
      f16x8 bh[4], bl[4];
      unit_sync();
#pragma unroll
      for (int ks = 0; ks < 4; ++ks) bh[ks] = frag(cur * RC_UNIT + b_frag, ks);
      if constexpr (half == 0) {
#pragma unroll
        for (int ks = 0; ks < 4; ++ks) {
          ah[ks] = frag(OFF_XH + kt * (RC_ROWS * 128) + a_frag, ks);
          al[ks] = frag(OFF_XL + kt * (RC_ROWS * 128) + a_frag, ks);
        }
      }
      unit_end();
      unit_sync();
#pragma unroll
      for (int ks = 0; ks < 4; ++ks) bl[ks] = frag(cur * RC_UNIT + b_frag, ks);
#pragma unroll
      for (int ks = 0; ks < 4; ++ks) {
        acc[half] = __builtin_amdgcn_mfma_f32_32x32x16_f16(ah[ks], bh[ks], acc[half], 0, 0, 0);
        acc[half] = __builtin_amdgcn_mfma_f32_32x32x16_f16(al[ks], bh[ks], acc[half], 0, 0, 0);
        acc[half] = __builtin_amdgcn_mfma_f32_32x32x16_f16(ah[ks], bl[ks], acc[half], 0, 0, 0);
      }
      unit_end();
    });
  });
  SH_STAMP();
  asm volatile("s_waitcnt lgkmcnt(0)\n\ts_barrier" ::: "memory");
  float* const wl = (float*)(smem + OFF_XH) + wave * (32 * LSTR);
  {
    const f32x4 colv = *(const f32x4*)(rp.b_in + nw + c4);
    const f32x4 g4 = *(const f32x4*)(rp.ln_gamma + nw + c4);
    slab_put<2, LSTR>(wl, acc, l31, lg);
    float2* const lnp = (float2*)(smem + OFF_LNP);
#pragma unroll
    for (int q = 0; q < 8; ++q) {
      const int row = q * 4 + rl;
      f32x4 v = *(const f32x4*)(wl + row * LSTR + c4) + colv;
      if constexpr (KIND == 1) v = v + resv[q];
      SDMI_ST_F32X4(rp.t, (size_t)(m0 + row) * C + nw + c4, v);
      const f32x4 vs = v * g4;
      *(f16x4*)(smem + OFF_XN + strip_off(row, nw + c4)) = f16x4{(f16)vs[0], (f16)vs[1], (f16)vs[2], (f16)vs[3]};
      float s1 = (v[0] + v[1]) + (v[2] + v[3]);
      float s2 = (v[0] * v[0] + v[1] * v[1]) + (v[2] * v[2] + v[3] * v[3]);
      s1 = sum8_dpp(s1); s2 = sum8_dpp(s2);
      if ((lane & 7) == 0) lnp[row * (C / 32) + ((nw + c4) >> 5)] = float2{s1, s2};
    }
    asm volatile("s_waitcnt lgkmcnt(0)" ::: "memory");
  }
  SH_STAMP();

  auto ln_table = [&]() {
    if (tid < RC_ROWS) {
      IGemmParams lq;
      lq.lnf_npart = C / 32; lq.lnf_eps = rp.ln_eps;
      const float2* pp = (const float2*)(smem + OFF_LNP) + tid * (C / 32);
      float2 pv[LNF_MAXP];
#pragma unroll
      for (int j = 0; j < LNF_MAXP; ++j) pv[j] = j < C / 32 ? pp[j] : float2{0.f, 0.f};
      float mu, rs_;
      lnf_finish(lq, pv, &mu, &rs_);
      ltab[tid] = float2{mu, rs_};
    }
  };
  auto fold = [&](f32x16 (&a)[2], const float (&cs_)[2], const float (&dn_)[2]) {
#pragma unroll
    for (int j = 0; j < 2; ++j)
#pragma unroll
      for (int r = 0; r < 16; ++r) {
        const float2 mr = ltab[(r & 3) + 8 * (r >> 2) + 4 * lg];
        a[j][r] = fmaf(mr.y, a[j][r] - mr.x * cs_[j], dn_[j]);
      }
  };
  auto rows_out = [&](f32x16 (&a)[2], f16* dst) {
    slab_put<2, LSTR>(wl, a, l31, lg);
    const int n = nw + c4;
    const int head = n / rp.dh, dd = n - head * rp.dh;
    f16* const base = dst + (((size_t)bsample * rp.heads + head) * rp.ntok + tok0) * rp.dh + dd;
#pragma unroll
    for (int q = 0; q < 8; ++q) {
      const int row = q * 4 + rl;
      const f32x4 v = *(const f32x4*)(wl + row * LSTR + c4);
      SDMI_ST(f16x4, base + (size_t)row * rp.dh, (f16x4{(f16)v[0], (f16)v[1], (f16)v[2], (f16)v[3]}));
    }
    asm volatile("s_waitcnt lgkmcnt(0)" ::: "memory");
  };

  zero2(acc);
  block(acc, OFF_XN, ln_table);
  SH_STAMP();
  if constexpr (KIND == 1 && CTX) {
    static_assert(C == 320, "head dim 40: eight heads of five 16-byte chunks");
    constexpr int D = 40, DKS = 3, DVT = 2, KVT = 64;
    const float sc = rp.ctx_scale * 1.4426950408889634f;
    const int nt = (rp.ctx_nkv + KVT - 1) / KVT;
    const int nheads = (rp.heads - wave + RC_NWC - 1) / RC_NWC;
    const int nsteps = nheads * nt;
    auto load_frags = [&](int i, u32x4 (&kf)[2][DKS], u32x4 (&vf)[2][2][DVT]) {
      const int head = wave + RC_NWC * (nt == 2 ? (i >> 1) : i), t = nt == 2 ? (i & 1) : 0;
      const int bh = bsample * rp.heads + head;
      const __amdgpu_buffer_rsrc_t rsrc_k = __builtin_amdgcn_make_buffer_rsrc((void*)(rp.ctx_k + (size_t)bh * rp.ctx_nkv * D), 0, rp.ctx_nkv * D * 2, 0x00020000);
      const __amdgpu_buffer_rsrc_t rsrc_v = __builtin_amdgcn_make_buffer_rsrc((void*)(rp.ctx_vt + (size_t)bh * D * rp.ctx_nkv_pad), 0, D * rp.ctx_nkv_pad * 2, 0x00020000);
#pragma unroll
      for (int kvb = 0; kvb < 2; ++kvb) {
        const int row = kvb * 32 + l31;
        const int key = t * KVT + ((row & ~12) | ((row & 4) << 1) | ((row & 8) >> 1));
#pragma unroll
        for (int ks = 0; ks < DKS; ++ks) kf[kvb][ks] = __builtin_amdgcn_raw_buffer_load_b128(rsrc_k, key * (D * 2) + (ks * 2 + lg) * 16, 0, 0);
#pragma unroll
        for (int s2 = 0; s2 < 2; ++s2)
#pragma unroll
          for (int dt = 0; dt < DVT; ++dt) {
            const int d = dt * 32 + l31;
            const unsigned one2 = d == D ? 0x3C003C00u : 0u;
            u32x4 v = {one2, one2, one2, one2};
            if (d < D) v = __builtin_amdgcn_raw_buffer_load_b128(rsrc_v, d * (rp.ctx_nkv_pad * 2) + t * (KVT * 2) + (4 * kvb + 2 * s2 + lg) * 16, 0, 0);
            vf[kvb][s2][dt] = v;
          }
      }
    };
    f16x8 qf[DKS];
    f32x16 o[DVT];
    float m_run = -1e30f;
    auto step = [&](int i, const u32x4 (&kf)[2][DKS], const u32x4 (&vf)[2][2][DVT]) {
      const int head = wave + RC_NWC * (nt == 2 ? (i >> 1) : i), t = nt == 2 ? (i & 1) : 0;
      if (t == 0) {
#pragma unroll
        for (int ks = 0; ks < DKS; ++ks) {
          const int dcol = ks * 16 + lg * 8;
          f16x8 v = {0, 0, 0, 0, 0, 0, 0, 0};
          if (dcol < D) v = *(const f16x8*)(smem + OFF_XN + strip_off(l31, head * D + dcol));
          qf[ks] = v;
        }
#pragma unroll
        for (int dt = 0; dt < DVT; ++dt)
#pragma unroll
          for (int r = 0; r < 16; ++r) o[dt][r] = 0.f;
        m_run = -1e30f;
      }
      f32x16 sa[2];
#pragma unroll
      for (int kvb = 0; kvb < 2; ++kvb) {
#pragma unroll
        for (int r = 0; r < 16; ++r) sa[kvb][r] = 0.f;
#pragma unroll
        for (int ks = 0; ks < DKS; ++ks)
          sa[kvb] = __builtin_amdgcn_mfma_f32_32x32x16_f16(__builtin_bit_cast(f16x8, kf[kvb][ks]), qf[ks], sa[kvb], 0, 0, 0);
      }
      const int kv0 = t * KVT;
      if (kv0 + KVT > rp.ctx_nkv) {
#pragma unroll
        for (int kvb = 0; kvb < 2; ++kvb)
#pragma unroll
          for (int r = 0; r < 16; ++r) {
            const int kv = kv0 + kvb * 32 + (r & 3) + 4 * ((r >> 2) & 1) + 8 * lg + 16 * (r >> 3);
            if (kv >= rp.ctx_nkv) sa[kvb][r] = -1e30f;
          }
      }
      float mx = -1e30f;
#pragma unroll
      for (int kvb = 0; kvb < 2; ++kvb)
#pragma unroll
        for (int r = 0; r < 16; ++r) mx = fmaxf(mx, sa[kvb][r]);
      mx = rc_max_across_halves(mx);
      const float m_new = fmaxf(m_run, mx * sc);
      if (__any(m_new > m_run)) {
        const float alpha = __builtin_amdgcn_exp2f(m_run - m_new);
        m_run = m_new;
#pragma unroll
        for (int dt = 0; dt < DVT; ++dt)
#pragma unroll
          for (int r = 0; r < 16; ++r) o[dt][r] *= alpha;
      }
      const f32x2 sc2 = {sc, sc}, nm2 = {-m_run, -m_run};
#pragma unroll
      for (int kvb = 0; kvb < 2; ++kvb)
#pragma unroll
        for (int r = 0; r < 16; r += 2) {
          const f32x2 sv = {sa[kvb][r], sa[kvb][r + 1]};
          const f32x2 e = __builtin_elementwise_fma(sv, sc2, nm2);
          sa[kvb][r] = __builtin_amdgcn_exp2f(e[0]);
          sa[kvb][r + 1] = __builtin_amdgcn_exp2f(e[1]);
        }
#pragma unroll
      for (int kvb = 0; kvb < 2; ++kvb)
#pragma unroll
        for (int s2 = 0; s2 < 2; ++s2) {
          f16x8 pf;
#pragma unroll
          for (int e = 0; e < 8; ++e) pf[e] = (f16)sa[kvb][8 * s2 + e];
#pragma unroll
          for (int dt = 0; dt < DVT; ++dt)
            o[dt] = __builtin_amdgcn_mfma_f32_32x32x16_f16(__builtin_bit_cast(f16x8, vf[kvb][s2][dt]), pf, o[dt], 0, 0, 0);
        }
      if (t == nt - 1) {
        float la = o[D / 32][4], lb = la;
        rc_swap_halves(la, lb);
        const float inv = 1.0f / la;
        f16* orow = rp.ao_out + (size_t)(m0 + l31) * C + (size_t)head * D;
#pragma unroll
        for (int dt = 0; dt < DVT; ++dt)
#pragma unroll
          for (int r4 = 0; r4 < 4; ++r4) {
            const int dd = dt * 32 + 8 * r4 + 4 * lg;
            if (dd < D) {
              const f16x4 v = {(f16)(o[dt][r4 * 4 + 0] * inv), (f16)(o[dt][r4 * 4 + 1] * inv), (f16)(o[dt][r4 * 4 + 2] * inv), (f16)(o[dt][r4 * 4 + 3] * inv)};
              SDMI_ST(f16x4, orow + dd, v);
            }
          }
      }
    };
    u32x4 kfa[2][DKS], vfa[2][2][DVT], kfb[2][DKS], vfb[2][2][DVT];
    if (nsteps > 0) load_frags(0, kfa, vfa);
    if (nsteps > 1) load_frags(1, kfb, vfb);
    asm volatile("s_waitcnt lgkmcnt(0)\n\ts_barrier" ::: "memory");
    fold(acc, fcs[0], fdn[0]);
    slab_put<2, LSTR>(wl, acc, l31, lg);
#pragma unroll
    for (int qq = 0; qq < 8; ++qq) {
      const int row = qq * 4 + rl;
      const f32x4 v = *(const f32x4*)(wl + row * LSTR + c4);
      *(f16x4*)(smem + OFF_XN + strip_off(row, nw + c4)) = f16x4{(f16)v[0], (f16)v[1], (f16)v[2], (f16)v[3]};
    }
    asm volatile("s_waitcnt lgkmcnt(0)\n\ts_barrier" ::: "memory");
    if (nsteps > 0) { step(0, kfa, vfa); if (nsteps > 2) load_frags(2, kfa, vfa); }
    if (nsteps > 1) { step(1, kfb, vfb); if (nsteps > 3) load_frags(3, kfb, vfb); }
    if (nsteps > 2) step(2, kfa, vfa);
    if (nsteps > 3) step(3, kfb, vfb);
    return;
  }
  if constexpr (KIND == 1) {
    asm volatile("s_waitcnt lgkmcnt(0)\n\ts_barrier" ::: "memory");
    fold(acc, fcs[0], fdn[0]);
    rows_out(acc, rp.q);
#ifdef SDMI_RC_TIMING
    SH_STAMP();
    if (rp.dbg && tid < 64) rp.dbg[(size_t)blockIdx.x * 128 + tid] = tid < n_stamp ? ((const long long*)(smem + OFF_DBG))[tid] : 0;
#endif
    return;
  }
  fold(acc, fcs[0], fdn[0]);
  rows_out(acc, rp.q);
  SH_STAMP();
  zero2(acc);
  block(acc, OFF_XN, nothing);
  SH_STAMP();
  fold(acc, fcs[NB > 1 ? 1 : 0], fdn[NB > 1 ? 1 : 0]);
  rows_out(acc, rp.k);
  SH_STAMP();
  zero2(acc);
  block(acc, OFF_XN, nothing);
  SH_STAMP();
  asm volatile("s_waitcnt lgkmcnt(0)\n\ts_barrier" ::: "memory");
  fold(acc, fcs[NB > 2 ? 2 : 0], fdn[NB > 2 ? 2 : 0]);
#pragma unroll
  for (int j = 0; j < 2; ++j) {
    const int n = nw + j * 32 + l31;
    const int head = n / rp.dh, dd = n - head * rp.dh;
    f16* const base = rp.vt + (((size_t)bsample * rp.heads + head) * rp.dh + dd) * rp.ntok_pad + tok0 + 4 * lg;
#pragma unroll
    for (int r4 = 0; r4 < 4; ++r4)
      *(f16x4*)(base + 8 * r4) = f16x4{(f16)acc[j][r4 * 4 + 0], (f16)acc[j][r4 * 4 + 1], (f16)acc[j][r4 * 4 + 2], (f16)acc[j][r4 * 4 + 3]};
  }
#ifdef SDMI_RC_TIMING
  SH_STAMP();
  asm volatile("s_waitcnt lgkmcnt(0)" ::: "memory");
  if (rp.dbg && tid < 64) rp.dbg[(size_t)blockIdx.x * 128 + tid] = tid < n_stamp ? ((const long long*)(smem + OFF_DBG))[tid] : 0;
#endif
#endif
}

}

bool ff_tail_supported(int C, int M, int hw) { return C == 320 && M % RC_ROWS == 0 && hw % RC_ROWS == 0 && (int64_t)M * C * 4 < ((int64_t)1 << 31); }

#ifdef SDMI_RC_TIMING
static long long* g_rc_dbg = nullptr;
static int g_rc_abl = 0;
extern "C" int sdmi_k_ff_tail_dbg(void* stamps, int abl) { g_rc_dbg = (long long*)stamps; g_rc_abl = abl; return 0; }
#endif

int launch_ff_tail(const FfTailParams& p, hipStream_t stream) {
  const IGemmParams& e = p.epi;
  const int C = e.N;
  SDMI_CHECK(ff_tail_supported(C, e.M, e.Hout * e.Wout), "ff_tail: C = 320, rows (per sample) multiples of 32");
  const bool head = p.a16 != nullptr;
  SDMI_CHECK((head || (p.ln && p.lnp)) && p.csd && p.wgg && p.wff2 && p.bff2 && p.t && p.wpo, "ff_tail: null operand");
  SDMI_CHECK(!head || (p.wo && p.bo && p.ln_gamma), "ff_tail: the out-projection in front needs wo, bo and the norm3 weight");
  SDMI_CHECK(e.mode == EPI_PLAIN && e.K == C && e.M == e.B * e.Hout * e.Wout && e.out_f32 && e.ldo % 4 == 0, "ff_tail: proj_out descriptor");
  SDMI_CHECK(e.residual && e.ldr >= C, "ff_tail: proj_out adds the SpatialTransformer's input (residual)");
  SDMI_CHECK(!e.lnf_part && !e.lnp_out && !e.f16_scale && !e.ln_out && !e.out_lo && !e.rowvec, "ff_tail: plain proj_out epilogue only");
  if (e.gn_n) {
    SDMI_CHECK(e.gn_n <= 2 && (e.Hout * e.Wout) % 32 == 0, "GroupNorm statistics need Hout*Wout % 32 == 0");
// ... 98 lines not shown
```

### stable-diffusion_amd/csrc/unet.cpp

```cpp
#include "unet.h"

extern "C" char** environ;
#include "prof.h"
#include "split16.h"

#include <math.h>
#include <stdio.h>
#include <string.h>

#include <algorithm>

namespace sdmi {

static bool in_list(const int* v, int n, int x) {
  for (int i = 0; i < n; ++i)
    if (v[i] == x) return true;
  return false;
}

thread_local Tape* g_tape_rec = nullptr;

namespace {
uint64_t sdmi_env_hash() {
  uint64_t h = 1469598103934665603ull;
  for (char** e = environ; e && *e; ++e) {
    if (strncmp(*e, "SDMI_", 5) != 0) continue;
    for (const char* c = *e; *c; ++c) { h ^= (unsigned char)*c; h *= 1099511628211ull; }
    h ^= 0xff; h *= 1099511628211ull;
  }
  return h;
}
struct TapeRecGuard {
  explicit TapeRecGuard(Tape* t) { g_tape_rec = t; }
  ~TapeRecGuard() { g_tape_rec = nullptr; }
};
}

int UNet::build(const sdmi_unet_cfg& c, int precision, const sdmi_unet_ext* ext, unsigned flags) {
  cfg_ = c;
  precision_ = precision;
  if (ext) ext_ = *ext;
  SDMI_CHECK((flags & ~((unsigned)SDMI_UNET_SCALE_SHIFT_NORM | (unsigned)SDMI_UNET_NUM_HEAD_CHANNELS_MASK)) == 0, "unknown UNet creation flag");
  scale_shift_ = (flags & SDMI_UNET_SCALE_SHIFT_NORM) != 0;
  num_head_channels_ = (int)((flags & SDMI_UNET_NUM_HEAD_CHANNELS_MASK) >> SDMI_UNET_NUM_HEAD_CHANNELS_SHIFT);
  SDMI_CHECK(!scale_shift_ || (ext_.attention_block == 1 && ext_.resblock_updown == 1),
             "SDMI_UNET_SCALE_SHIFT_NORM needs attention_block = 1 and resblock_updown = 1");
  SDMI_CHECK(ext_.attention_block == 0 || ext_.attention_block == 1, "attention_block must be 0 (SpatialTransformer) or 1 (AttentionBlock)");
  SDMI_CHECK(ext_.resblock_updown == 0 || ext_.resblock_updown == 1, "resblock_updown must be 0 or 1");
  SDMI_CHECK(c.n_levels >= 1 && c.n_levels <= 8 && c.n_attention_resolutions >= 0 && c.n_attention_resolutions <= 8,
             "bad level / attention_resolutions count");
  SDMI_CHECK(num_head_channels_ == 0 || ext_.attention_block == 1,
             "num_head_channels is expressed for the AttentionBlock family only (attention_block = 1); a SpatialTransformer takes num_heads");
  if (ext_.attention_block == 1) SDMI_CHECK(c.model_channels > 0 && c.model_channels % 32 == 0, "model_channels must be a multiple of 32 on this path");
  else SDMI_CHECK(c.model_channels % 64 == 0, "model_channels must be a multiple of 64 on this path (SpatialTransformer family)");
  if (has_ctx()) SDMI_CHECK(c.context_dim % 64 == 0, "context_dim must be a multiple of 64 on this path");
  else SDMI_CHECK(c.context_dim == 0, "a UNet of AttentionBlocks has no cross-attention: context_dim must be 0");
  SDMI_CHECK((c.num_heads >= 1 || num_head_channels_ > 0) && c.transformer_depth >= 1, "num_heads / transformer_depth");
  const int mc = c.model_channels;
  te_ = 4 * mc;
  if (const char* e = getenv("SDMI_FUSE_GN_STATS")) fuse_gn_stats_ = atoi(e) != 0;
  if (const char* e = getenv("SDMI_LN_FOLD")) ln_fold_ = atoi(e) != 0;
  if (const char* e = getenv("SDMI_LN_FOLD_MIN_ROWS")) ln_fold_min_rows_ = atoi(e);

  int cur_ds = 1;
  auto add_res = [&](const std::string& p, int cin, int cout) {
    Layer L; L.kind = L_RES; L.prefix = p; L.cin = cin; L.cout = cout;
    L.emb_off = emb_total_; emb_total_ += scale_shift_ ? 2 * cout : cout;
    L.p1x1 = full() || (precise_1x1_ && cur_ds < precise_1x1_max_ds_);
    L.precise3 = full();
    return L;
  };
  auto add_attn = [&](const std::string& p, int ch) {
    Layer L; L.kind = has_ctx() ? L_ATTN : L_ATTN_LEGACY; L.prefix = p; L.cin = ch; L.cout = ch;
    if (num_head_channels_ > 0) { L.heads = ch / num_head_channels_; L.dh = num_head_channels_; }
    else { L.heads = c.num_heads; L.dh = ch / c.num_heads; }
    L.attn_index = n_attn_++;
    L.p1x1 = full() || (precise_1x1_ && cur_ds < precise_1x1_max_ds_);
    return L;
  };
  auto add_updown = [&](const std::string& p, int ch, int dir) {
    Layer L = add_res(p, ch, ch);
    L.updown = dir;
    return L;
  };

  {
    Layer L; L.kind = L_CONV_IN; L.prefix = "input_blocks.0.0"; L.cin = c.in_channels; L.cout = mc;
    input_blocks_.push_back({L});
  }
  std::vector<int> chans{mc};
  int ch = mc, ds = 1;
  for (int level = 0; level < c.n_levels; ++level) {
    const int mult = c.channel_mult[level];
    for (int r = 0; r < c.num_res_blocks; ++r) {
      const int n = (int)input_blocks_.size();
      std::vector<Layer> blk;
      cur_ds = ds;
      blk.push_back(add_res("input_blocks." + std::to_string(n) + ".0", ch, mult * mc));
      ch = mult * mc;
      if (in_list(c.attention_resolutions, c.n_attention_resolutions, ds))
        blk.push_back(add_attn("input_blocks." + std::to_string(n) + ".1", ch));
      input_blocks_.push_back(blk);
      chans.push_back(ch);
    }
    if (level != c.n_levels - 1) {
// ... 215 lines not shown
constexpr int64_t PK_ALIGN = 256;
constexpr int PK_NHC_SHIFT = 16;
constexpr int32_t PK_NHC_MASK = 0xfff << PK_NHC_SHIFT;
constexpr int32_t PK_FULL = 4;
}

int UNet::packed_layout(std::vector<std::pair<void**, size_t>>* bufs, int64_t* total) const {
  int64_t off = (int64_t)round_up((int64_t)sizeof(PackedHeader), PK_ALIGN);
  for (const auto& b : store_.buffers()) {
    if (bufs) bufs->push_back(b);
    off += (int64_t)round_up((int64_t)b.second, PK_ALIGN);
  }
  *total = off;
  return 0;
}

int UNet::export_packed(void* host_buf, int64_t bytes, hipStream_t stream) {
  SDMI_CHECK(finalized_, "export needs a finalized handle");
  std::vector<std::pair<void**, size_t>> bufs;
  int64_t total = 0;
  packed_layout(&bufs, &total);
  SDMI_CHECK(host_buf && bytes >= total, "packed buffer too small: need " + std::to_string(total) + " bytes");
  PackedHeader h{};
  memcpy(h.magic, "SDMIPK01", 8);
  h.abi = SDMI_ABI_VERSION; h.precise_1x1 = precise_1x1_ ? 1 : 0; h.n_buffers = (int32_t)bufs.size(); h.cfg = cfg_;
  h.reserved = (precise_kv_ ? 1 : 0) | (precise_last_res_ ? 2 : 0) | (precise_1x1_max_ds_ << 8);
  h.reserved |= (ext_.attention_block << 4) | (ext_.resblock_updown << 5) | ((scale_shift_ ? 1 : 0) << 6);
  h.reserved |= num_head_channels_ << PK_NHC_SHIFT;
  if (full()) h.reserved |= PK_FULL;
  h.total_bytes = total;
  memcpy(host_buf, &h, sizeof(h));
  int64_t off = (int64_t)round_up((int64_t)sizeof(PackedHeader), PK_ALIGN);
  for (auto& b : bufs) {
    SDMI_HIP_OK(hipMemcpyAsync((char*)host_buf + off, *b.first, b.second, hipMemcpyDeviceToHost, stream));
    off += (int64_t)round_up((int64_t)b.second, PK_ALIGN);
  }
  SDMI_HIP_OK(hipStreamSynchronize(stream));
  return 0;
}

int UNet::import_packed(const void* host_buf, int64_t bytes, hipStream_t stream) {
  SDMI_CHECK(host_buf && bytes >= (int64_t)sizeof(PackedHeader), "packed blob truncated");
  PackedHeader h;
  memcpy(&h, host_buf, sizeof(h));
  SDMI_CHECK(memcmp(h.magic, "SDMIPK01", 8) == 0, "not a libsdmi packed-weight blob");
  SDMI_CHECK(h.abi == SDMI_ABI_VERSION, "packed blob was written by a different ABI version: repack it");
  SDMI_CHECK(memcmp(&h.cfg, &cfg_, sizeof(cfg_)) == 0, "packed blob was written for a different UNet configuration");
  SDMI_CHECK(((h.reserved & PK_FULL) != 0) == full(), std::string("packed blob was written by a ") +
             ((h.reserved & PK_FULL) ? "full" : "mixed") + "-precision UNet handle and cannot be imported into a " + (full() ? "full" : "mixed") +
             "-precision one: repack it with a handle of this precision");
  SDMI_CHECK((h.precise_1x1 != 0) == precise_1x1_, "packed blob was written with a different precision allocation (split-fp16 1x1 convs)");
  SDMI_CHECK((h.reserved & (7 << 4)) == ((ext_.attention_block << 4) | (ext_.resblock_updown << 5) | ((scale_shift_ ? 1 : 0) << 6)),
             "packed blob was written for a different UNet family (attention_block / resblock_updown / scale-shift norm)");
  SDMI_CHECK(((h.reserved & PK_NHC_MASK) >> PK_NHC_SHIFT) == num_head_channels_,
             "packed blob was written for num_head_channels " + std::to_string((h.reserved & PK_NHC_MASK) >> PK_NHC_SHIFT) + ", this handle has " +
             std::to_string(num_head_channels_) + ": repack it");
  SDMI_CHECK((h.reserved & ~PK_FULL & ~(7 << 4) & ~PK_NHC_MASK) == ((precise_kv_ ? 1 : 0) | (precise_last_res_ ? 2 : 0) | (precise_1x1_max_ds_ << 8)),
             "packed blob was written with a different precision allocation (context K / V, last ResBlock, 1x1 conv levels)");
  std::vector<std::pair<void**, size_t>> bufs;
  int64_t total = 0;
  packed_layout(&bufs, &total);
  SDMI_CHECK(h.n_buffers == (int32_t)bufs.size() && h.total_bytes == total && bytes >= total, "packed blob truncated or inconsistent");
  int64_t off = (int64_t)round_up((int64_t)sizeof(PackedHeader), PK_ALIGN);
  for (auto& b : bufs) {
    if (store_.alloc(b.first, b.second)) return -1;
    SDMI_HIP_OK(hipMemcpyAsync(*b.first, (const char*)host_buf + off, b.second, hipMemcpyHostToDevice, stream));
    off += (int64_t)round_up((int64_t)b.second, PK_ALIGN);
  }
  SDMI_HIP_OK(hipStreamSynchronize(stream));
  store_.mark_all_set();
  ctx_valid_ = false;
  drop_timestep_table();
  return finalize();
}

struct Fwd : FwdBase {
  UNet* u; int Lctx;
  bool ln_fold_on = false;
  bool ff_tail_on = false;
  bool st_head_on = false;
  bool st_mid_on = false;
  bool st_tail_on = false;
  bool st_mid_ctx_on = false;
  bool ctx1_on = false;
  bool gn_conv_on = false;
  float* emb_all = nullptr;
  int emb_ld = 0;
  bool emb_caller = false;
  const f16* ctx16 = nullptr;
  const f16* ctx16_lo = nullptr;

  Act res_block(Layer& L, const Act& x0, const Act* x1) {
    const int H = x0.H, W = x0.W, M = B * H * W;
    const int Cin = x0.C + (x1 ? x1->C : 0), Cout = L.cout;
    if (Cin != L.cin) { ok(fail("res block channel mismatch at " + L.prefix)); }
    if (Cin == Cout && x1) ok(fail("identity skip with a concatenated input at " + L.prefix));
    const size_t mark = scratch.off;
    f16* raw = (Cin != Cout) ? S<f16>((size_t)M * Cin) : nullptr;
    const bool p1 = L.p1x1;
    const bool p3 = L.precise3;
    f16* raw_lo = (Cin != Cout && p1) ? S<f16>((size_t)M * Cin) : nullptr;
    float* h = S<float>((size_t)M * Cout);
    Act out = make_act(P<float>((size_t)M * Cout), Cout, H, W, true);
    Act hact = make_act(h, Cout, H, W, true);
    f16* a2 = nullptr;
    int& gn2_applied = u->gn2_applied_;
    gn2_applied = 0;
    const bool ss = u->scale_shift_;
    const float* const film = ss ? emb_all + L.emb_off : nullptr;
    const bool gc1 = gn_conv_on && !ss && !p3 && Cin == Cout && gn_conv3_supported(B, H, W, x0.C, x1 ? x1->C : 0, Cout);
    const bool gc2 = gn_conv_on && !ss && !p3 && gn_conv3_supported(B, H, W, Cout, 0, Cout);
    auto gn_conv = [&](const Act& a0, const Act* a1, const float* gamma, const float* beta, const f16* w, IGemmParams& e) {
      GnConvParams g = GnConvParams();
      g.gn_acc = groupnorm(a0, a1, gamma, beta, 1e-5f, 1, nullptr, nullptr, nullptr, nullptr, nullptr, true);
      g.x0 = a0.p; g.c0 = a0.C; g.x1 = a1 ? a1->p : nullptr; g.c1 = a1 ? a1->C : 0;
      g.gn_gamma = gamma; g.gn_beta = beta; g.gn_eps = 1e-5f; g.w = w; g.epi = e;
      if (!dry && !rc) ok(launch_gn_conv3(g, s));
    };
    if (gc1) {
      IGemmParams p = conv3(nullptr, Cin, H, W, H, W, 1, 0, L.w16[0], Cout);
      p.bias = L.f32[2]; p.rowvec = emb_all + L.emb_off; p.ld_rowvec = emb_ld;
      p.out_f32 = h; p.ldo = Cout;
      attach_gn_targets(p, hact);
      TapeCaller tc(Tape::R_EMB, emb_caller ? p.rowvec : nullptr);
      gn_conv(x0, x1, L.f32[0], L.f32[1], L.w16[0], p);
    } else {
      f16* a = S<f16>((size_t)M * Cin);
      f16* a_lo = p3 ? S<f16>((size_t)M * Cin) : nullptr;
      groupnorm(x0, x1, L.f32[0], L.f32[1], 1e-5f, 1, a, nullptr, raw, a_lo, raw_lo);
      IGemmParams p = conv3(a, Cin, H, W, H, W, 1, 0, L.w16[0], Cout);
      if (p3) split3(p, a, a_lo, Cin);
      p.bias = L.f32[2];
      if (!ss) { p.rowvec = emb_all + L.emb_off; p.ld_rowvec = emb_ld; }
      p.out_f32 = h; p.ldo = Cout;
      attach_gn_targets(p, hact);
      if (!gc2 && !p3 && !ss) {
        a2 = S<f16>((size_t)M * Cout);
        p.pgn_gamma = L.f32[3]; p.pgn_beta = L.f32[4]; p.pgn_eps = 1e-5f; p.pgn_silu = 1; p.pgn_out = a2; p.pgn_applied = &gn2_applied;
      }
      TapeCaller tc(Tape::R_EMB, emb_caller ? p.rowvec : nullptr);
      gemm(p);
    }
    const float* residual = x0.p;
    if (Cin != Cout) {
      IGemmParams p = dense1x1(raw, raw_lo, M, Cin, L.w16[2], Cout, H * W, p1);
      p.bias = L.f32[6]; p.out_f32 = out.p; p.ldo = Cout;
      gemm(p);
      residual = out.p;
    }
    if (gc2) {
      IGemmParams p = conv3(nullptr, Cout, H, W, H, W, 1, 0, L.w16[1], Cout);
      p.bias = L.f32[5]; p.residual = residual; p.ldr = Cout; p.out_f32 = out.p; p.ldo = Cout;
      attach_gn_targets(p, out);
      attach_f16_copy(p, out);
      gn_conv(hact, nullptr, L.f32[3], L.f32[4], L.w16[1], p);
    } else {
      f16* a2_lo = nullptr;
      if (p3) { a2 = S<f16>((size_t)M * Cout); a2_lo = S<f16>((size_t)M * Cout); }
      if (ss && !a2) a2 = S<f16>((size_t)M * Cout);
      {
        TapeCaller tc(Tape::R_EMB, emb_caller ? film : nullptr);
        groupnorm(hact, nullptr, L.f32[3], L.f32[4], 1e-5f, 1, a2, nullptr, nullptr, a2_lo, nullptr, false, gn2_applied != 0, film, emb_ld);
      }
      IGemmParams p = conv3(a2, Cout, H, W, H, W, 1, 0, L.w16[1], Cout);
      if (p3) split3(p, a2, a2_lo, Cout);
      p.bias = L.f32[5]; p.residual = residual; p.ldr = Cout; p.out_f32 = out.p; p.ldo = Cout;
// ... 106 lines not shown
    long long* gn_stats = nullptr;
    if (chain_head) gn_stats = groupnorm(x, nullptr, L.f32[0], L.f32[1], 1e-6f, 0, nullptr, nullptr, nullptr, nullptr, nullptr, true);
    else groupnorm(x, nullptr, L.f32[0], L.f32[1], 1e-6f, 0, xn, nullptr, nullptr, xn_lo, nullptr);
    float* t = S<float>((size_t)M * C);
    f16* ln = S<f16>((size_t)M * C);
    f16* q = S<f16>((size_t)M * C);
    f16* k = S<f16>((size_t)M * C);
    f16* vt = S<f16>((size_t)B * C * Np);
    f16* ao = S<f16>((size_t)M * C);
    f16* gg = S<f16>((size_t)M * 4 * C);
    float* lnp = fold_ln ? S<float>((size_t)(C / 32) * M * 2) : nullptr;
    auto with_ln = [&](IGemmParams& p, const float* gamma, const float* beta) {
      if (fold_ln) { p.out_f16 = ln; p.f16_scale = gamma; p.lnp_out = lnp; p.splitk = 1; }
      else { p.ln_gamma = gamma; p.ln_beta = beta; p.ln_out = ln; p.ln_eps = 1e-5f; }
    };
    auto fold_in = [&](IGemmParams& p, const float* cs, const float* dn) {
      if (!fold_ln) return;
      p.lnf_part = lnp; p.lnf_npart = C / 32; p.lnf_eps = 1e-5f; p.lnf_cs = cs; p.lnf_d = dn; p.bias = nullptr;
    };
    if (chain_head) {
      TBlock& T = L.tb[0];
      StHeadParams h = StHeadParams();
      h.x = x.p; h.gn_acc = gn_stats; h.gn_gamma = L.f32[0]; h.gn_beta = L.f32[1]; h.gn_eps = 1e-6f;
      h.w_in = L.w16[0]; h.b_in = L.f32[2]; h.t = t; h.ln_gamma = T.ln[0]; h.ln_eps = 1e-5f;
      h.wqkv = T.wqkv; h.lnf_cs = T.lnf[0]; h.lnf_d = T.lnf[1]; h.q = q; h.k = k; h.vt = vt;
      h.M = M; h.B = B; h.ntok = N; h.ntok_pad = Np; h.heads = L.heads; h.dh = L.dh; h.C = C;
      if (!dry && !rc && Np != N) {
        hipError_t e = memset_async(vt, 0, (size_t)B * C * Np * sizeof(f16), s);
        if (e != hipSuccess) ok(fail(std::string("hipMemsetAsync: ") + hipGetErrorString(e)));
      }
      if (!dry && !rc) ok(launch_st_head(h, s));
    } else {
      IGemmParams p = dense1x1(xn, xn_lo, M, C, L.w16[0], C, N, p1);
      p.bias = L.f32[2]; p.out_f32 = t; p.ldo = C;
      with_ln(p, L.tb[0].ln[0], L.tb[0].ln[1]);
      gemm(p);
    }
    const int depth = (int)L.tb.size();
    const bool chain_ff = ff_tail_on && fold_ln && p1 && depth == 1 && L.tb[0].lnf_csd != nullptr && ff_tail_supported(C, M, N) &&
                          dense1x1(nullptr, nullptr, M, C, L.w16[1], C, N, p1).split16;
    const bool chain_tail = chain_ff && st_tail_on;
    for (int d = 0; d < depth; ++d) {
      TBlock& T = L.tb[d];
      if (!(chain_head && d == 0)) {
        IGemmParams p = dense(ln, M, C, T.wqkv, 3 * C, N);
        p.mode = EPI_HEADS; p.seg_dst[0] = q; p.seg_dst[1] = k; p.seg_dst[2] = vt;
        p.seg_kind[0] = 0; p.seg_kind[1] = 0; p.seg_kind[2] = 1;
        p.heads = L.heads; p.dh = L.dh; p.ntok = N; p.ntok_pad = Np; p.segC = C; p.splitk = 1;
        fold_in(p, T.lnf[0], T.lnf[1]);
        if (!dry && !rc && Np != N) {
          hipError_t e = memset_async(vt, 0, (size_t)B * C * Np * sizeof(f16), s);
          if (e != hipSuccess) ok(fail(std::string("hipMemsetAsync: ") + hipGetErrorString(e)));
        }
        gemm(p);
      }
      attention(q, k, vt, ao, L, N, N, Np, scale);
      bool chain_ctx = false;
      const bool chain_mid = st_mid_on && fold_ln && T.lnf[2] != nullptr && st_head_supported(C, M, N, Np, L.heads, L.dh);
      if (chain_mid) {
        StHeadParams h = StHeadParams();
        h.a16 = ao; h.w_in = T.wo1; h.b_in = T.bo1; h.t = t; h.ln_gamma = T.ln[2]; h.ln_eps = 1e-5f;
        h.wqkv = T.wq2; h.lnf_cs = T.lnf[2]; h.lnf_d = T.lnf[3]; h.q = q;
        h.M = M; h.B = B; h.ntok = N; h.ntok_pad = Np; h.heads = L.heads; h.dh = L.dh; h.C = C;
        if (ctx16) context_kv(L, d);
        chain_ctx = st_mid_ctx_on && L.dh == 40 && Lctx <= 128;
        if (chain_ctx) { h.ctx_k = T.ck; h.ctx_vt = T.cvt; h.ctx_nkv = Lctx; h.ctx_nkv_pad = Lp; h.ctx_scale = scale; h.ao_out = ao; }
        if (!dry && !rc) ok(launch_st_mid(h, s));
      } else {
        IGemmParams p = dense(ao, M, C, T.wo1, C, N);
        p.bias = T.bo1; p.residual = t; p.ldr = C; p.out_f32 = t; p.ldo = C;
        with_ln(p, T.ln[2], T.ln[3]);
        gemm(p);
      }
      if (ctx16 && !chain_mid) context_kv(L, d);
      if (chain_mid) {
        if (!chain_ctx) attention(q, T.ck, T.cvt, ao, L, N, Lctx, Lp, scale);
      } else if (ctx1_on && Lctx == 1) {
        if (!dry && !rc) ok(launch_ctx1_broadcast(T.cvt, Lp, ao, B, N, C, s));
      } else {
        IGemmParams p = dense(ln, M, C, T.wq2, C, N);
        p.mode = EPI_HEADS; p.seg_dst[0] = q; p.seg_kind[0] = 0;
        p.heads = L.heads; p.dh = L.dh; p.ntok = N; p.ntok_pad = Np; p.segC = C; p.splitk = 1;
        fold_in(p, T.lnf[2], T.lnf[3]);
        gemm(p);
        attention(q, T.ck, T.cvt, ao, L, N, Lctx, Lp, scale);
      }
      if (!chain_tail) {
        IGemmParams p = dense(ao, M, C, T.wo2, C, N);
        p.bias = T.bo2; p.residual = t; p.ldr = C; p.out_f32 = t; p.ldo = C;
        with_ln(p, T.ln[4], T.ln[5]);
        gemm(p);
      }
      if (chain_ff) break;
      {
        IGemmParams p = dense(ln, M, C, T.wgg, 8 * C, N);
        p.mode = EPI_GEGLU; p.bias = T.bgg; p.out_f16 = gg; p.ldo = 4 * C; p.splitk = 1;
        fold_in(p, T.lnf[4], T.lnf[5]);
        gemm(p);
      }
      {
        IGemmParams p = dense(gg, M, 4 * C, T.wff2, C, N);
        p.bias = T.bff2; p.residual = t; p.ldr = C; p.ldo = C;
        if (d + 1 < depth) {
          p.out_f32 = t;
          with_ln(p, L.tb[d + 1].ln[0], L.tb[d + 1].ln[1]);
        } else {
          p.out_f16 = ln; p.out_lo = xn_lo;
        }
        gemm(p);
      }
    }
    Act out = make_act(P<float>((size_t)M * C), C, H, W, true);
    {
      IGemmParams p = dense1x1(ln, xn_lo, M, C, L.w16[1], C, N, p1);
      p.Hout = H * W;
      p.bias = L.f32[3]; p.residual = x.p; p.ldr = C; p.out_f32 = out.p; p.ldo = C;
      attach_gn_targets(p, out);
      attach_f16_copy(p, out);
      if (chain_ff) {
        TBlock& T = L.tb[0];
        FfTailParams q = FfTailParams();
        q.ln = ln; q.lnp = lnp; q.ln_eps = 1e-5f; q.csd = T.lnf_csd; q.wgg = T.wgg; q.wff2 = T.wff2; q.bff2 = T.bff2; q.t = t; q.wpo = L.w16[1];
        if (chain_tail) { q.a16 = ao; q.wo = T.wo2; q.bo = T.bo2; q.ln_gamma = T.ln[4]; }
        q.epi = p;
        if (!dry && !rc) ok(launch_ff_tail(q, s));
      } else {
        gemm(p);
      }
    }
    scratch.off = mark;
    return out;
  }

  void attention(const f16* q, const f16* k, const f16* vt, f16* out, Layer& L, int nq, int nkv, int nkv_pad, float scale) {
    AttnParams a = AttnParams();
    a.q = q; a.k = k; a.vt = vt; a.out = out; a.BH = B * L.heads; a.heads = L.heads; a.nq = nq; a.nkv = nkv;
    a.nkv_pad = nkv_pad; a.d = L.dh; a.scale = scale;
    if (!dry && !rc) ok(launch_attention(a, s));
  }

  Act resample(Layer& L, const Act& x, bool up) {
    const int Hin = x.H, Win = x.W, C = x.C;
    const int Hout = up ? 2 * Hin : (Hin - 1) / 2 + 1, Wout = up ? 2 * Win : (Win - 1) / 2 + 1;
    const size_t mark = scratch.off;
    if (u->full()) {
      const int64_t n = (int64_t)B * Hin * Win * C;
      f16* hi = S<f16>((size_t)n); f16* lo = S<f16>((size_t)n);
      if (!dry && !rc) ok(launch_cast_f16(x.p, hi, lo, n, s));
      Act out = make_act(P<float>((size_t)B * Hout * Wout * C), L.cout, Hout, Wout, true);
      IGemmParams p = conv3(hi, C, Hin, Win, Hout, Wout, up ? 1 : 2, up ? 1 : 0, L.w16[0], L.cout);
      split3(p, hi, lo, C);
      p.bias = L.f32[0]; p.out_f32 = out.p; p.ldo = L.cout;
      attach_gn_targets(p, out);
      gemm(p);
      scratch.off = mark;
      return out;
    }
    const f16* x16 = nullptr;
    if (dry) { if (!want_f16_copy(x)) (void)S<f16>((size_t)B * Hin * Win * C); }
    else {
      x16 = f16_copy(x);
      if (!x16) {
        f16* c = S<f16>((size_t)B * Hin * Win * C);
        if (!rc) ok(launch_cast_f16(x.p, c, nullptr, (int64_t)B * Hin * Win * C, s));
        x16 = c;
      }
    }
    Act out = make_act(P<float>((size_t)B * Hout * Wout * C), L.cout, Hout, Wout, true);
// ... 193 lines not shown
              int64_t* bytes_needed) {
  SDMI_CHECK(dry || finalized_, "sdmi_unet_finalize() has not succeeded yet");
  SDMI_CHECK(B >= 1 && B <= 8, "batch (CFG rows) must be 1..8 per call");
  if (has_ctx()) SDMI_CHECK(H >= 1 && W >= 1 && Lctx >= 1, "bad shape");
  else SDMI_CHECK(H >= 1 && W >= 1 && Lctx == 0 && ctx == nullptr && !ctx_only,
                  "bad shape: this UNet has no cross-attention (AttentionBlocks): pass ctx = NULL and Lctx = 0");
  const int down = 1 << (cfg_.n_levels - 1);
  if (ext_.resblock_updown)
    SDMI_CHECK(H % down == 0 && W % down == 0, "latent H and W must be multiples of " + std::to_string(down) +
               " for resblock_updown (the down ResBlocks' avg_pool2d rounds down, the skip concat needs the sizes back)");
  SDMI_CHECK(H % down == 0 && W % down == 0, "H and W must be divisible by 2^(levels-1) (the UNet's skip concat requires it)");

  const int hint_row = emb_hint_row_;
  if (!dry && !ctx_only) emb_hint_row_ = -1;

  const char* e_rp = getenv("SDMI_REPLAY"); const char* e_rv = getenv("SDMI_REPLAY_VERIFY");
  const bool replay_on = !(e_rp && atoi(e_rp) == 0);
  const bool replay_verify = e_rv && atoi(e_rv) != 0;
  const bool hinted = t_i64 != nullptr && hint_row >= 0 && hint_row < (int)emb_tab_t_.size();
  auto in_ws = [&](const void* p, size_t bytes) {
    return p && (uintptr_t)p < (uintptr_t)workspace + (uint64_t)ws_bytes && (uintptr_t)workspace < (uintptr_t)p + bytes;
  };
  const size_t img = (size_t)B * H * W * sizeof(float);
  const bool tape_ok = replay_on && !dry && !ctx_only && !prof_enabled() && !tune_collecting() && !range_check_enabled() &&
                       workspace != nullptr && (t_i64 || t_f32) && !in_ws(x, img * cfg_.in_channels) && !in_ws(eps_out, img * cfg_.out_channels) &&
                       !in_ws(t_i64 ? (const void*)t_i64 : t_f32, (size_t)B * (t_i64 ? 8 : 4)) &&
                       !in_ws(ctx, (size_t)B * Lctx * cfg_.context_dim * sizeof(float));
  TapeKey tkey;
  uintptr_t caller[Tape::R_COUNT] = {0, 0, 0, 0, 0};
  Tape* rec = nullptr;
  std::unique_ptr<Tape> verify_against;
  if (tape_ok) {
    tkey.B = B; tkey.H = H; tkey.W = W; tkey.Lctx = Lctx; tkey.mode = hinted ? 0 : (t_i64 ? 1 : 2);
    tkey.ws = workspace; tkey.ws_bytes = ws_bytes; tkey.have_ctx = ctx != nullptr;
    tkey.env = sdmi_env_hash() ^ (tune_generation() * 0x9e3779b97f4a7c15ull); tkey.weights_gen = weights_gen_; tkey.ctx_gen = ctx_gen_;
    auto low4 = [](const void* p, int shift) { return (unsigned)((uintptr_t)p & 15) << shift; };
    tkey.align = low4(x, 0) | low4(eps_out, 4) | low4(ctx, 8) | low4(t_i64 ? (const void*)t_i64 : t_f32, 12);
    caller[Tape::R_X] = (uintptr_t)x; caller[Tape::R_OUT] = (uintptr_t)eps_out;
    caller[Tape::R_T] = hinted ? 0 : (t_i64 ? (uintptr_t)t_i64 : (uintptr_t)t_f32);
    caller[Tape::R_CTX] = (uintptr_t)ctx;
    caller[Tape::R_EMB] = hinted ? (uintptr_t)(emb_tab_ + (size_t)hint_row * emb_total_) : 0;
    for (size_t i = 0; i < tapes_.size(); ++i) {
      if (!(tapes_[i].first == tkey)) continue;
      std::unique_ptr<Tape> hit = std::move(tapes_[i].second);
      tapes_.erase(tapes_.begin() + (long)i);
      SDMI_CHECK(finalized_, "sdmi_unet_finalize() has not succeeded yet");
      if (ensure_ctx_cache(B, Lctx, false)) return -1;
      if (!ctx && has_ctx()) SDMI_CHECK(ctx_valid_, "ctx == NULL but no cached context for this (B, Lctx); call sdmi_unet_cache_context first");
      hit->retarget(caller);
      if (replay_verify) { verify_against = std::move(hit); break; }
      const int e = hit->replay(stream);
      const bool sets = hit->sets_ctx_valid;
      const int64_t need = hit->bytes_needed;
      tapes_.emplace_back(tkey, std::move(hit));
      if (e) return fail(std::string("launch tape replay: ") + hipGetErrorString((hipError_t)e));
      if (sets) ctx_valid_ = true;
      if (bytes_needed) *bytes_needed = need;
      ++tape_hits_;
      return 0;
    }
  }
  std::unique_ptr<Tape> fresh;
  if (tape_ok) {
    fresh.reset(new Tape());
    memcpy(fresh->caller, caller, sizeof(caller));
    rec = fresh.get();
  }

  Fwd f;
  f.u = this; f.s = stream; f.dry = dry; f.B = B; f.Lctx = Lctx; f.zero = store_.zero(); f.precise_1x1 = precise_1x1_;
  {
    const char* e_fold = getenv("SDMI_LN_FOLD"); const char* e_vec = getenv("SDMI_EPI_VEC");
    f.ln_fold_on = (e_fold ? atoi(e_fold) != 0 : ln_fold_) && !(e_vec && atoi(e_vec) == 0);
    const char* e_ff = getenv("SDMI_FF_TAIL");
    f.ff_tail_on = e_ff ? atoi(e_ff) != 0 : ff_tail_;
    const char* e_sh = getenv("SDMI_ST_HEAD");
    f.st_head_on = e_sh ? atoi(e_sh) != 0 : st_head_;
    const char* e_sm = getenv("SDMI_ST_MID");
    f.st_mid_on = e_sm ? atoi(e_sm) != 0 : st_head_;
    const char* e_st = getenv("SDMI_ST_TAIL");
    f.st_tail_on = e_st ? atoi(e_st) != 0 : ff_tail_;
    const char* e_mc = getenv("SDMI_ST_MID_CTX");
    f.st_mid_ctx_on = e_mc ? atoi(e_mc) != 0 : st_head_;
    const char* e_c1 = getenv("SDMI_CTX1");
    f.ctx1_on = !(e_c1 && atoi(e_c1) == 0);
    const char* e_gc = getenv("SDMI_GN_CONV");
    f.gn_conv_on = e_gc ? atoi(e_gc) != 0 : false;
    if (full()) {
      f.ln_fold_on = f.ff_tail_on = f.st_head_on = f.st_mid_on = f.st_tail_on = f.st_mid_ctx_on = f.gn_conv_on = false;
    }
  }
  int64_t persist_bytes = 0, scratch_bytes = 0;
  for (int pass = 0; pass < 2; ++pass) {
    const bool d = (pass == 0) ? true : false;
    if (pass == 1 && dry) break;
    f.dry = d; f.rc = 0;
    f.n_acts = 0;
    TapeRecGuard tape_guard(d ? nullptr : rec);
    f.plan = fuse_gn_stats_ ? &gn_plan_ : nullptr;
    if (d) gn_plan_.clear();
    f.persist = Arena(); f.scratch = Arena();
    f.persist.dry = f.scratch.dry = d;
    if (!d) {
      SDMI_CHECK(persist_bytes + scratch_bytes <= ws_bytes, "workspace too small: need " +
                 std::to_string(persist_bytes + scratch_bytes) + " bytes, got " + std::to_string(ws_bytes));
      SDMI_CHECK(workspace != nullptr, "workspace is NULL");
      f.persist.base = (char*)workspace; f.persist.cap = (size_t)persist_bytes;
      f.scratch.base = (char*)workspace + persist_bytes; f.scratch.cap = (size_t)scratch_bytes;
      if (ensure_ctx_cache(B, Lctx, ctx_only)) return -1;
    }
    const int mc = cfg_.model_channels;
    if (f.begin_pass((int64_t)12 << 20)) return -1;
    f16* ctx16 = f.P<f16>((size_t)B * Lctx * cfg_.context_dim);
    f16* ctx16_lo = precise_kv_ ? f.P<f16>((size_t)B * Lctx * cfg_.context_dim) : nullptr;
    const bool have_ctx = has_ctx() && ((ctx != nullptr) || d);
    if (!has_ctx()) {
      f.ctx16 = nullptr; f.ctx16_lo = nullptr;
    } else if (have_ctx) {
      if (!d) {
        TapeCaller tc(Tape::R_CTX, ctx);
        int r = launch_cast_f16(ctx, ctx16, ctx16_lo, (int64_t)B * Lctx * cfg_.context_dim, stream);
        if (r) return r;
      }
      f.ctx16 = ctx16; f.ctx16_lo = ctx16_lo;
    } else {
      SDMI_CHECK(ctx_valid_, "ctx == NULL but no cached context for this (B, Lctx); call sdmi_unet_cache_context first");
      f.ctx16 = nullptr; f.ctx16_lo = nullptr;
    }
    if (ctx_only) {
      for_each_layer([&](Layer& L) -> int {
        if (L.kind == L_ATTN) for (int dd = 0; dd < (int)L.tb.size(); ++dd) f.context_kv(L, dd);
        return 0;
      });
    } else {
      float* temb = f.P<float>((size_t)B * mc);
      float* e1 = f.P<float>((size_t)B * te_);
      float* emb = f.P<float>((size_t)B * te_);
      f.emb_all = f.P<float>((size_t)B * emb_total_);
      f.emb_ld = emb_total_;
      if (!d && t_i64 != nullptr && hint_row >= 0 && hint_row < (int)emb_tab_t_.size()) {
        f.emb_all = emb_tab_ + (size_t)hint_row * emb_total_;
        f.emb_ld = 0;
        f.emb_caller = true;
      } else if (!d) {
        int r;
        {
          TapeCaller tc(Tape::R_T, t_i64 ? (const void*)t_i64 : t_f32);
          r = launch_timestep_embedding(t_i64, t_f32, temb, B, mc, stream);
        }
        if (!r) r = launch_small_linear(temb, mc, te_w0_, te_b0_, e1, te_, B, te_, mc, 0, stream);
        if (!r) r = launch_small_linear(e1, te_, te_w2_, te_b2_, emb, te_, B, te_, te_, 1, stream);
        if (!r) r = launch_small_linear(emb, te_, emb_w_, emb_b_, f.emb_all, emb_total_, B, emb_total_, te_, 1, stream);
        if (r) return r;
      }
      std::vector<Act> hs;
      Act h;
      {
        Layer& L = input_blocks_[0][0];
        const char* e_cis = getenv("SDMI_CONV_IN_STATS");
        h = f.make_act(f.P<float>((size_t)B * H * W * mc), mc, H, W, (H * W) % 16 == 0 && !(e_cis && atoi(e_cis) == 0));
        IGemmParams st = IGemmParams();
        f.attach_gn_targets(st, h);
        if (!d) {
          TapeCaller tc(Tape::R_X, x);
          int r = launch_conv_in(x, L.w32[0], L.f32[0], h.p, B, cfg_.in_channels, H, W, mc, stream, st.gn_n, st.gn_acc, st.gn_cpg, st.gn_cbase);
          if (r) return r;
        }
        hs.push_back(h);
      }
      for (size_t bi = 1; bi < input_blocks_.size(); ++bi) {
        for (auto& L : input_blocks_[bi]) h = f.run_layer(L, h, nullptr);
        hs.push_back(h);
// ... 58 lines not shown
```

Before: 3.685.

## Fuse cross-attention Q projection with context attention in one kernel

Adds a q_ctx kernel that computes the LayerNorm-folded Q projection GEMM tile and then runs cross-attention against the short text context directly from registers/LDS, writing the attention output. The shared flash-style context attention routine is factored into a reusable header. It is enabled by default for head dims 80 and 160 with context length up to 128, and removes the Q write/read round trip and one kernel launch per cross-attention. In exchange it adds a complex kernel with its own tiling and register pressure, and may lose some GEMM efficiency.

New measurement: 3.709, median of 6. Within noise of the previous version (+0.7%).

```diff
diff --git a/include/sdmi.h b/include/sdmi.h
--- a/include/sdmi.h
+++ b/include/sdmi.h
@@ -193,6 +193,9 @@
 int sdmi_k_st_mid_ctx(const void* a_f16, const void* wo_f16, const float* bo, float* t, const float* ln_gamma, float ln_eps, const void* wq_f16,
                       const float* lnf_cs, const float* lnf_d, const void* ctx_k, const void* ctx_vt, int nkv, int nkv_pad, float scale, void* ao_out,
                       int B, int ntok, int heads, int dh, int C, void* stream);
+int sdmi_k_q_ctx(const void* a_f16, const void* wq_f16, const float* lnf_part, float lnf_eps, const float* lnf_cs, const float* lnf_d,
+                 const void* ctx_k, const void* ctx_vt, int nkv, int nkv_pad, float scale, void* ao_out, int B, int ntok, int heads, int dh,
+                 int row_block, void* stream);
 int sdmi_k_ln_fold_prep(const void* w_f16, int N, int K, int ldw, const float* gamma, const float* beta, const float* bias,
                         float* cs, float* d, void* stream);
 int sdmi_k_attention(const void* q, const void* k, const void* vt, void* out, int BH, int heads, int nq, int nkv,
diff --git a/stable-diffusion_amd/_lib.py b/stable-diffusion_amd/_lib.py
--- a/stable-diffusion_amd/_lib.py
+++ b/stable-diffusion_amd/_lib.py
@@ -130,6 +130,8 @@
     'sdmi_k_gn_conv3': (C.c_int, [C.POINTER(IGemmDesc), c_ptr, c_ptr, C.c_int, C.c_int, c_ptr, C.c_int64, c_ptr, c_ptr, C.c_float, c_ptr]),
     'sdmi_k_st_mid_ctx': (C.c_int, [c_ptr, c_ptr, c_ptr, c_ptr, c_ptr, C.c_float, c_ptr, c_ptr, c_ptr, c_ptr, c_ptr, C.c_int, C.c_int, C.c_float, c_ptr,
                                     C.c_int, C.c_int, C.c_int, C.c_int, C.c_int, c_ptr]),
+    'sdmi_k_q_ctx': (C.c_int, [c_ptr, c_ptr, c_ptr, C.c_float, c_ptr, c_ptr, c_ptr, c_ptr, C.c_int, C.c_int, C.c_float, c_ptr,
+                               C.c_int, C.c_int, C.c_int, C.c_int, C.c_int, c_ptr]),
     'sdmi_k_st_tail': (C.c_int, [C.POINTER(IGemmDesc), c_ptr, c_ptr, c_ptr, c_ptr, c_ptr, C.c_float, c_ptr, c_ptr, c_ptr, c_ptr, c_ptr]),
     'sdmi_k_st_mid': (C.c_int, [c_ptr, c_ptr, c_ptr, c_ptr, c_ptr, C.c_float, c_ptr, c_ptr, c_ptr, c_ptr, C.c_int, C.c_int, C.c_int, C.c_int,
                                 C.c_int, c_ptr]),
diff --git a/stable-diffusion_amd/build.py b/stable-diffusion_amd/build.py
--- a/stable-diffusion_amd/build.py
+++ b/stable-diffusion_amd/build.py
@@ -9,7 +9,7 @@
 EXTRA = os.environ.get('SDMI_CXXFLAGS', '').split()
 LIB = os.path.join(HERE, os.environ.get('SDMI_LIB_OUT', 'libsdmi.so'))
 OBJ = os.path.join(HERE, 'build' if os.path.basename(LIB) == 'libsdmi.so' else 'build_' + os.path.splitext(os.path.basename(LIB))[0])
-SOURCES = ['igemm_t1.hip', 'igemm_t0.hip', 'igemm_t2.hip', 'igemm_h1.hip', 'igemm_h0.hip', 'igemm_h2.hip', 'igemm.hip', 'conv3halo.hip', 'gemm_split16.hip', 'rowchain.hip', 'gnconv.hip', 'range.hip', 'attn.hip', 'attn_wide.hip', 'attn_split16.hip', 'attn_wide_split16.hip', 'split_ops.hip', 'norm.hip', 'small.hip', 'sampler.hip', 'inpaint.hip', 'patch.hip', 'weights.cpp', 'unet.cpp', 'vae.cpp', 'clip.cpp', 'bert.cpp', 'api.cpp', 'prof.cpp']
+SOURCES = ['igemm_t1.hip', 'igemm_t0.hip', 'igemm_t2.hip', 'igemm_h1.hip', 'igemm_h0.hip', 'igemm_h2.hip', 'igemm.hip', 'conv3halo.hip', 'gemm_split16.hip', 'rowchain.hip', 'qctx.hip', 'gnconv.hip', 'range.hip', 'attn.hip', 'attn_wide.hip', 'attn_split16.hip', 'attn_wide_split16.hip', 'split_ops.hip', 'norm.hip', 'small.hip', 'sampler.hip', 'inpaint.hip', 'patch.hip', 'weights.cpp', 'unet.cpp', 'vae.cpp', 'clip.cpp', 'bert.cpp', 'api.cpp', 'prof.cpp']
 FLAGS = ['--offload-arch=gfx950', '-O3', '-std=c++17', '-fPIC', '-munsafe-fp-atomics', '-Wall', '-Wno-unused-function',
          '-Wno-unused-variable']
 
diff --git a/stable-diffusion_amd/csrc/api.cpp b/stable-diffusion_amd/csrc/api.cpp
--- a/stable-diffusion_amd/csrc/api.cpp
+++ b/stable-diffusion_amd/csrc/api.cpp
@@ -425,6 +425,23 @@
   p.M = B * ntok; p.B = B; p.ntok = ntok; p.ntok_pad = ntok; p.heads = heads; p.dh = dh; p.C = C;
   return launch_st_mid(p, (hipStream_t)stream);
 }
+int sdmi_k_q_ctx(const void* a_f16, const void* wq_f16, const float* lnf_part, float lnf_eps, const float* lnf_cs, const float* lnf_d,
+                 const void* ctx_k, const void* ctx_vt, int nkv, int nkv_pad, float scale, void* ao_out, int B, int ntok, int heads, int dh,
+                 int row_block, void* stream) {
+  SDMI_CHECK(a_f16 && wq_f16 && ctx_k && ctx_vt && ao_out, "q_ctx: null argument");
+  SDMI_CHECK(B > 0 && ntok > 0 && heads > 0 && dh > 0, "q_ctx: bad shape");
+  SDMI_CHECK(lnf_part == nullptr || (lnf_cs && lnf_d), "q_ctx: the LayerNorm fold needs its column terms");
+  const int C = heads * dh;
+  QCtxParams q = QCtxParams();
+  IGemmParams& p = q.g;
+  p.a0 = (const f16*)a_f16; p.c0 = C; p.lda0 = C; p.B = B; p.Hin = p.Hout = ntok; p.Win = p.Wout = 1; p.ksize = 1;
+  p.w = (const f16*)wq_f16; p.M = B * ntok; p.N = C; p.K = C; p.mode = EPI_HEADS; p.splitk = 1;
+  p.heads = heads; p.dh = dh; p.ntok = ntok; p.ntok_pad = (int)round_up(ntok, 8); p.segC = C;
+  if (lnf_part) { p.lnf_part = lnf_part; p.lnf_npart = C / 32; p.lnf_eps = lnf_eps; p.lnf_cs = lnf_cs; p.lnf_d = lnf_d; }
+  q.ctx_k = (const f16*)ctx_k; q.ctx_vt = (const f16*)ctx_vt; q.nkv = nkv; q.nkv_pad = nkv_pad; q.scale = scale; q.out = (f16*)ao_out;
+  q.bm = row_block;
+  return launch_q_ctx(q, (hipStream_t)stream);
+}
 int sdmi_k_ln_fold_prep(const void* w_f16, int N, int K, int ldw, const float* gamma, const float* beta, const float* bias,
                         float* cs, float* d, void* stream) {
   return launch_ln_fold_prep((const f16*)w_f16, N, K, ldw, gamma, beta, bias, cs, d, (hipStream_t)stream);
diff --git a/stable-diffusion_amd/csrc/common.h b/stable-diffusion_amd/csrc/common.h
--- a/stable-diffusion_amd/csrc/common.h
+++ b/stable-diffusion_amd/csrc/common.h
@@ -241,6 +241,19 @@
 int launch_st_head(const StHeadParams& p, hipStream_t stream);
 int launch_st_mid(const StHeadParams& p, hipStream_t stream);
 
+struct QCtxParams {
+  IGemmParams g;
+  const f16* ctx_k = nullptr;
+  const f16* ctx_vt = nullptr;
+  int nkv = 0, nkv_pad = 0;
+  float scale = 0.f;
+  f16* out = nullptr;
+  int bm = 0;
+};
+int q_ctx_row_block(int bm);
+bool q_ctx_supported(const QCtxParams& p);
+int launch_q_ctx(const QCtxParams& p, hipStream_t stream);
+
 struct GnConvParams {
   const float* x0 = nullptr; const float* x1 = nullptr; int c0 = 0, c1 = 0;
   const long long* gn_acc = nullptr;
diff --git a/stable-diffusion_amd/csrc/ctx_attn.h b/stable-diffusion_amd/csrc/ctx_attn.h
--- /dev/null
+++ b/stable-diffusion_amd/csrc/ctx_attn.h
@@ -0,0 +1,157 @@
+#pragma once
+#include "common.h"
+
+namespace sdmi {
+namespace {
+
+#if defined(__HIP_DEVICE_COMPILE__)
+typedef float ca_f32x2 __attribute__((ext_vector_type(2)));
+typedef unsigned ca_u32x4 __attribute__((ext_vector_type(4)));
+
+__device__ __forceinline__ void ca_swap_halves(float& a, float& b) {
+  asm volatile("s_nop 1\n\tv_permlane32_swap_b32 %0, %1\n\ts_nop 1" : "+v"(a), "+v"(b));
+}
+__device__ __forceinline__ float ca_max_across_halves(float x) {
+  float a = x, b = x;
+  ca_swap_halves(a, b);
+  return fmaxf(a, b);
+}
+__device__ __forceinline__ float ca_sum_across_halves(float x) {
+  float a = x, b = x;
+  ca_swap_halves(a, b);
+  return a + b;
+}
+
+template <int D>
+struct CtxAttn {
+  static constexpr int DKS = (D + 15) / 16;
+  static constexpr int DVT = (D + 31) / 32;
+  static constexpr int KVT = 64;
+  static constexpr bool ONES = DVT * 32 > D;
+  static_assert(D % 8 == 0, "16-byte fragments");
+
+  f32x16 o[DVT];
+  float m_run, l_run;
+
+  __device__ __forceinline__ void begin() {
+#pragma unroll
+    for (int dt = 0; dt < DVT; ++dt)
+#pragma unroll
+      for (int r = 0; r < 16; ++r) o[dt][r] = 0.f;
+    m_run = -1e30f;
+    l_run = 0.f;
+  }
+
+  template <class KF, class VF>
+  __device__ __forceinline__ void tile(const f16x8 (&qf)[DKS], KF&& kfrag, VF&& vfrag, const int kv0, const int nkv, const float sc, const int lg) {
+    f32x16 sa[2];
+#pragma unroll
+    for (int kvb = 0; kvb < 2; ++kvb) {
+#pragma unroll
+      for (int r = 0; r < 16; ++r) sa[kvb][r] = 0.f;
+#pragma unroll
+      for (int ks = 0; ks < DKS; ++ks) sa[kvb] = __builtin_amdgcn_mfma_f32_32x32x16_f16(kfrag(kvb, ks), qf[ks], sa[kvb], 0, 0, 0);
+    }
+    if (kv0 + KVT > nkv) {
+#pragma unroll
+      for (int kvb = 0; kvb < 2; ++kvb)
+#pragma unroll
+        for (int r = 0; r < 16; ++r) {
+          const int kv = kv0 + kvb * 32 + (r & 3) + 4 * ((r >> 2) & 1) + 8 * lg + 16 * (r >> 3);
+          if (kv >= nkv) sa[kvb][r] = -1e30f;
+        }
+    }
+    float mx = -1e30f;
+#pragma unroll
+    for (int kvb = 0; kvb < 2; ++kvb)
+#pragma unroll
+      for (int r = 0; r < 16; ++r) mx = fmaxf(mx, sa[kvb][r]);
+    mx = ca_max_across_halves(mx);
+    const float m_new = fmaxf(m_run, mx * sc);
+    if (__any(m_new > m_run)) {
+      const float alpha = __builtin_amdgcn_exp2f(m_run - m_new);
+      m_run = m_new;
+      if (!ONES) l_run *= alpha;
+#pragma unroll
+      for (int dt = 0; dt < DVT; ++dt)
+#pragma unroll
+        for (int r = 0; r < 16; ++r) o[dt][r] *= alpha;
+    }
+    ca_f32x2 psum2 = {0.f, 0.f};
+    const ca_f32x2 sc2 = {sc, sc}, nm2 = {-m_run, -m_run};
+#pragma unroll
+    for (int kvb = 0; kvb < 2; ++kvb)
+#pragma unroll
+      for (int r = 0; r < 16; r += 2) {
+        const ca_f32x2 sv = {sa[kvb][r], sa[kvb][r + 1]};
+        const ca_f32x2 e = __builtin_elementwise_fma(sv, sc2, nm2);
+        const ca_f32x2 pv = {__builtin_amdgcn_exp2f(e[0]), __builtin_amdgcn_exp2f(e[1])};
+        sa[kvb][r] = pv[0];
+        sa[kvb][r + 1] = pv[1];
+        if (!ONES) psum2 += pv;
+      }
+    if (!ONES) l_run += psum2[0] + psum2[1];
+#pragma unroll
+    for (int kvb = 0; kvb < 2; ++kvb)
+#pragma unroll
+      for (int s2 = 0; s2 < 2; ++s2) {
+        f16x8 pf;
+#pragma unroll
+        for (int e = 0; e < 8; ++e) pf[e] = (f16)sa[kvb][8 * s2 + e];
+#pragma unroll
+        for (int dt = 0; dt < DVT; ++dt) o[dt] = __builtin_amdgcn_mfma_f32_32x32x16_f16(vfrag(kvb, s2, dt), pf, o[dt], 0, 0, 0);
+      }
+  }
+
+  __device__ __forceinline__ void finish(f16* orow, const int lg) {
+    float l_tot;
+    if constexpr (ONES) {
+      constexpr int rl = D % 32, r_l = (rl & 3) + 4 * (rl >> 3), lg_l = (rl >> 2) & 1;
+      float a = o[D / 32][r_l], b = a;
+      ca_swap_halves(a, b);
+      l_tot = lg_l == 0 ? a : b;
+    } else {
+      l_tot = ca_sum_across_halves(l_run);
+    }
+    const float inv = 1.0f / l_tot;
+#pragma unroll
+    for (int dt = 0; dt < DVT; ++dt)
+#pragma unroll
+      for (int r4 = 0; r4 < 4; ++r4) {
+        const int dd = dt * 32 + 8 * r4 + 4 * lg;
+        if (dd < D) {
+          const f16x4 v = {(f16)(o[dt][r4 * 4 + 0] * inv), (f16)(o[dt][r4 * 4 + 1] * inv), (f16)(o[dt][r4 * 4 + 2] * inv), (f16)(o[dt][r4 * 4 + 3] * inv)};
+          SDMI_ST(f16x4, orow + dd, v);
+        }
+      }
+  }
+};
+
+template <int D>
+__device__ __forceinline__ void ctx_load_frags(const f16* k_bh, const f16* vt_bh, const int nkv, const int nkv_pad, const int t, const int l31,
+                                               const int lg, ca_u32x4 (&kf)[2][CtxAttn<D>::DKS], ca_u32x4 (&vf)[2][2][CtxAttn<D>::DVT]) {
+  constexpr int DKS = CtxAttn<D>::DKS, DVT = CtxAttn<D>::DVT, KVT = CtxAttn<D>::KVT;
+  const __amdgpu_buffer_rsrc_t rsrc_k = __builtin_amdgcn_make_buffer_rsrc((void*)k_bh, 0, nkv * D * 2, 0x00020000);
+  const __amdgpu_buffer_rsrc_t rsrc_v = __builtin_amdgcn_make_buffer_rsrc((void*)vt_bh, 0, D * nkv_pad * 2, 0x00020000);
+#pragma unroll
+  for (int kvb = 0; kvb < 2; ++kvb) {
+    const int row = kvb * 32 + l31;
+    const int key = t * KVT + ((row & ~12) | ((row & 4) << 1) | ((row & 8) >> 1));
+#pragma unroll
+    for (int ks = 0; ks < DKS; ++ks) kf[kvb][ks] = __builtin_amdgcn_raw_buffer_load_b128(rsrc_k, key * (D * 2) + (ks * 2 + lg) * 16, 0, 0);
+#pragma unroll
+    for (int s2 = 0; s2 < 2; ++s2)
+#pragma unroll
+      for (int dt = 0; dt < DVT; ++dt) {
+        const int d = dt * 32 + l31;
+        const unsigned one2 = d == D ? 0x3C003C00u : 0u;
+        ca_u32x4 v = {one2, one2, one2, one2};
+        if (d < D) v = __builtin_amdgcn_raw_buffer_load_b128(rsrc_v, d * (nkv_pad * 2) + t * (KVT * 2) + (4 * kvb + 2 * s2 + lg) * 16, 0, 0);
+        vf[kvb][s2][dt] = v;
+      }
+  }
+}
+#endif
+
+}
+}
diff --git a/stable-diffusion_amd/csrc/igemm_dev.h b/stable-diffusion_amd/csrc/igemm_dev.h
--- a/stable-diffusion_amd/csrc/igemm_dev.h
+++ b/stable-diffusion_amd/csrc/igemm_dev.h
@@ -129,6 +129,9 @@
   const float var = fmaxf(q * inv_c - mu * mu, 0.f);
   *mean = mu;
   *rstd = 1.0f / sqrtf(var + p.lnf_eps);
+}
+__device__ __forceinline__ float lnf_apply(const float acc, const float2 mr, const float cs, const float dn) {
+  return fmaf(mr.y, acc - mr.x * cs, dn);
 }
 __device__ __forceinline__ float sum8_dpp(float v) {
   v += __builtin_bit_cast(float, __builtin_amdgcn_update_dpp(0, __builtin_bit_cast(int, v), 0xB1, 0xF, 0xF, true));
@@ -247,7 +250,7 @@
 #pragma unroll
         for (int r = 0; r < 16; ++r) {
           const float2 mr = tab[wm * WTM + i * 32 + (r & 3) + 8 * (r >> 2) + 4 * lg];
-          acc[i][j][r] = fmaf(mr.y, acc[i][j][r] - mr.x * cs, dn);
+          acc[i][j][r] = lnf_apply(acc[i][j][r], mr, cs, dn);
         }
     }
     __syncthreads();
diff --git a/stable-diffusion_amd/csrc/qctx.hip b/stable-diffusion_amd/csrc/qctx.hip
--- /dev/null
+++ b/stable-diffusion_amd/csrc/qctx.hip
@@ -0,0 +1,252 @@
+#include <string>
+
+#include "ctx_attn.h"
+#include "igemm_dev.h"
+
+namespace sdmi {
+namespace {
+
+constexpr int QC_BN = 160;
+
+template <int BM, int D, int NS>
+__global__ void __launch_bounds__(5 * 64) q_ctx_kernel(const QCtxParams qp) {
+#if defined(__HIP_DEVICE_COMPILE__)
+  const IGemmParams& p = qp.g;
+  constexpr int BN = QC_BN, TM = BM / 32, NW = BN / 32;
+  constexpr int STAGE = (BM + BN) * 128, RING = NS * STAGE;
+  constexpr int LPT = (BM + BN) / 8;
+  constexpr int PPW = (LPT + NW - 1) / NW;
+  constexpr int QP = BN * 2 + 16;
+  constexpr int OFF_Q = RING, OFF_TAB = OFF_Q + BM * QP, LDS_TOTAL = OFF_TAB + BM * 8;
+  using CA = CtxAttn<D>;
+  constexpr int DKS = CA::DKS, DVT = CA::DVT, KVT = CA::KVT;
+  constexpr int HPT = BN / D;
+  constexpr bool KV_LDS = D > 80;
+  constexpr int NCH = (D + 63) / 64, KROWS = NCH * 64, VROWS = DVT * 32, KV_STAGE = (KROWS + VROWS) * 128;
+  constexpr int PK = NCH * 8, PV = D / 8, PT = PK + PV;
+  static_assert(BN % D == 0 && D % 16 == 0, "whole heads, whole k-steps");
+  static_assert(!KV_LDS || (2 * KV_STAGE <= RING && !CA::ONES), "two key tiles in the dead ring; no padding rows to fill");
+  static_assert(NS >= 3 && PPW * (NS - 2) <= 48 && LDS_TOTAL <= 160 * 1024, "vmcnt literal, LDS budget");
+  __shared__ __attribute__((aligned(16))) unsigned char smem[LDS_TOTAL];
+
+  const int nblk = gridDim.x, bid = blockIdx.x;
+  const int q8 = nblk >> 3, r8 = nblk & 7, xcd = bid & 7;
+  const int wgid = (xcd < r8 ? xcd * (q8 + 1) : r8 * (q8 + 1) + (xcd - r8) * q8) + (bid >> 3);
+  const int tiles_m = p.M / BM, tiles_n = p.N / BN;
+  int tile_m, tile_n;
+  if (p.tile_n_fastest) { tile_m = wgid / tiles_n; tile_n = wgid - tile_m * tiles_n; }
+  else { tile_n = wgid / tiles_m; tile_m = wgid - tile_n * tiles_m; }
+  const int m0 = tile_m * BM, n0 = tile_n * BN;
+  const int nkt = p.K / BK;
+
+  const int tid = threadIdx.x, lane = tid & 63;
+  const int wave_u = __builtin_amdgcn_readfirstlane(tid >> 6);
+  const int wn = wave_u;
+  const int l31 = lane & 31, lg = lane >> 5;
+  constexpr int OOB = (int)0x80000000;
+
+  const bool unit = wave_u < TM * HPT;
+  const int urow = unit ? wave_u / HPT : 0, uhead = unit ? wave_u - urow * HPT : 0;
+  const int bsample = m0 / p.ntok;
+  const int head = tile_n * HPT + uhead;
+  const int nt = (qp.nkv + KVT - 1) / KVT;
+  const f16* const k_bh = qp.ctx_k + (size_t)(bsample * p.heads + head) * qp.nkv * D;
+  const f16* const vt_bh = qp.ctx_vt + (size_t)(bsample * p.heads + head) * D * qp.nkv_pad;
+  u32x4 kfa[KV_LDS ? 1 : 2][KV_LDS ? 1 : DKS], vfa[KV_LDS ? 1 : 2][2][KV_LDS ? 1 : DVT];
+  u32x4 kfb[KV_LDS ? 1 : 2][KV_LDS ? 1 : DKS], vfb[KV_LDS ? 1 : 2][2][KV_LDS ? 1 : DVT];
+  if constexpr (!KV_LDS) {
+    if (unit) ctx_load_frags<D>(k_bh, vt_bh, qp.nkv, qp.nkv_pad, 0, l31, lg, kfa, vfa);
+  }
+  const int ncol = n0 + wn * 32 + l31;
+  float cs = 0.f, dn = 0.f, bv = 0.f;
+  if (p.lnf_part) { cs = p.lnf_cs[ncol]; dn = p.lnf_d[ncol]; }
+  if (p.bias) bv = p.bias[ncol];
+  float2 lnf_pv[LNF_MAXP];
+  float lnf_mean = 0.f, lnf_rstd = 1.f;
+  const bool lnf_mine = p.lnf_part != nullptr && tid < BM;
+  if (lnf_mine) lnf_request(p, m0 + tid, lnf_pv);
+
+  const int l8 = lane >> 3, cpos = lane & 7;
+  const __amdgpu_buffer_rsrc_t rs_a = __builtin_amdgcn_make_buffer_rsrc((void*)p.a0, 0, OOB, 0x00020000);
+  const __amdgpu_buffer_rsrc_t rs_w = __builtin_amdgcn_make_buffer_rsrc((void*)p.w, 0, OOB, 0x00020000);
+  int pc_voff[PPW], pc_row0[PPW];
+#pragma unroll
+  for (int j = 0; j < PPW; ++j) {
+    const int q = min(wave_u + j * NW, LPT - 1);
+    const int row = q * 8 + l8;
+    const int gch = cpos ^ ((row >> 1) & 7);
+    const int grow = row < BM ? m0 + row : n0 + row - BM;
+    pc_voff[j] = (grow * p.K + gch * 8) * 2;
+    pc_row0[j] = q * 8;
+  }
+  auto issue_tile = [&](int kt, int stage) {
+    const int soff = min(kt, nkt - 1) * (BK * 2);
+#pragma unroll
+    for (int j = 0; j < PPW; ++j) {
+      auto dst = (__attribute__((address_space(3))) void*)(smem + stage * STAGE + pc_row0[j] * 128);
+      if (pc_row0[j] < BM) __builtin_amdgcn_raw_ptr_buffer_load_lds(rs_a, dst, 16, pc_voff[j], soff, 0, 0);
+      else __builtin_amdgcn_raw_ptr_buffer_load_lds(rs_w, dst, 16, pc_voff[j], soff, 0, SDMI_W_AUX);
+    }
+  };
+
+  const int rsw = (l31 >> 1) & 7;
+  const int a_lds = l31 * 128, b_lds = (BM + wn * 32 + l31) * 128;
+  auto read_frags = [&](int stage, int ks, f16x8 (&a)[TM], f16x8& b) {
+    const unsigned char* st = smem + stage * STAGE + (((ks * 2 + lg) ^ rsw) << 4);
+#pragma unroll
+    for (int i = 0; i < TM; ++i) a[i] = *(const f16x8*)(st + a_lds + i * 32 * 128);
+    b = *(const f16x8*)(st + b_lds);
+  };
+  f32x16 acc[TM];
+#pragma unroll
+  for (int i = 0; i < TM; ++i)
+#pragma unroll
+    for (int r = 0; r < 16; ++r) acc[i][r] = 0.f;
+  auto mfma_step = [&](const f16x8 (&a)[TM], const f16x8& b) {
+#pragma unroll
+    for (int i = 0; i < TM; ++i) acc[i] = __builtin_amdgcn_mfma_f32_32x32x16_f16(a[i], b, acc[i], 0, 0, 0);
+  };
+#pragma unroll
+  for (int s = 0; s < NS - 1; ++s) issue_tile(s, s);
+  wait_vmcnt<0>();
+  if (lnf_mine) lnf_finish(p, lnf_pv, &lnf_mean, &lnf_rstd);
+  asm volatile("s_waitcnt lgkmcnt(0)\n\ts_barrier" ::: "memory");
+  f16x8 fa[2][2][TM], fb[2][2];
+  read_frags(0, 0, fa[0][0], fb[0][0]);
+  read_frags(0, 1, fa[0][1], fb[0][1]);
+  int cur = 0, nxt = NS - 1;
+  for (int kt = 0; kt < nkt; ++kt) {
+    const int cur1 = (cur + 1 == NS) ? 0 : cur + 1;
+    read_frags(cur, 2, fa[1][0], fb[1][0]);
+    read_frags(cur, 3, fa[1][1], fb[1][1]);
+    issue_tile(kt + NS - 1, nxt);
+    mfma_step(fa[0][0], fb[0][0]);
+    mfma_step(fa[0][1], fb[0][1]);
+    wait_vmcnt<PPW*(NS - 2)>();
+    asm volatile("s_waitcnt lgkmcnt(0)\n\ts_barrier" ::: "memory");
+    read_frags(cur1, 0, fa[0][0], fb[0][0]);
+    read_frags(cur1, 1, fa[0][1], fb[0][1]);
+    mfma_step(fa[1][0], fb[1][0]);
+    mfma_step(fa[1][1], fb[1][1]);
+    cur = cur1;
+    nxt = (nxt + 1 == NS) ? 0 : nxt + 1;
+  }
+  wait_vmcnt<0>();
+
+  if constexpr (!KV_LDS) {
+    if (unit && nt > 1) ctx_load_frags<D>(k_bh, vt_bh, qp.nkv, qp.nkv_pad, 1, l31, lg, kfb, vfb);
+  }
+  float2* const tab = (float2*)(smem + OFF_TAB);
+  if (tid < BM) tab[tid] = float2{lnf_mean, lnf_rstd};
+  asm volatile("s_waitcnt lgkmcnt(0)\n\ts_barrier" ::: "memory");
+  if constexpr (KV_LDS) {
+    const __amdgpu_buffer_rsrc_t rsrc_k = __builtin_amdgcn_make_buffer_rsrc((void*)k_bh, 0, qp.nkv * D * 2, 0x00020000);
+    const __amdgpu_buffer_rsrc_t rsrc_v = __builtin_amdgcn_make_buffer_rsrc((void*)vt_bh, 0, D * qp.nkv_pad * 2, 0x00020000);
+    for (int j = wave_u; j < nt * PT; j += NW) {
+      const int t = j >= PT ? 1 : 0, q = j - t * PT;
+      if (q < PK) {
+        const int c = q >> 3, row = (q & 7) * 8 + l8;
+        const int key = (row & ~12) | ((row & 4) << 1) | ((row & 8) >> 1);
+        const int gch = cpos ^ ((row >> 1) & 7);
+        auto dst = (__attribute__((address_space(3))) void*)(smem + t * KV_STAGE + (c * 64 + (q & 7) * 8) * 128);
+        __builtin_amdgcn_raw_ptr_buffer_load_lds(rsrc_k, dst, 16, (t * KVT + key) * (D * 2) + c * 128 + gch * 16, 0, 0, 0);
+      } else {
+        const int qv = q - PK, dt = qv >> 2, row = (qv & 3) * 8 + l8;
+        const int gch = cpos ^ ((row >> 1) & 7);
+        auto dst = (__attribute__((address_space(3))) void*)(smem + t * KV_STAGE + (KROWS + dt * 32 + (qv & 3) * 8) * 128);
+        __builtin_amdgcn_raw_ptr_buffer_load_lds(rsrc_v, dst, 16, (dt * 32 + row) * (qp.nkv_pad * 2) + t * (KVT * 2) + gch * 16, 0, 0, 0);
+      }
+    }
+  }
+
+#pragma unroll
+  for (int i = 0; i < TM; ++i)
+#pragma unroll
+    for (int r = 0; r < 16; ++r) {
+      const int row = i * 32 + (r & 3) + 8 * (r >> 2) + 4 * lg;
+      float v = acc[i][r];
+      if (p.lnf_part) v = lnf_apply(v, tab[row], cs, dn);
+      if (p.bias) v += bv;
+      *(f16*)(smem + OFF_Q + row * QP + (wn * 32 + l31) * 2) = (f16)v;
+    }
+  if constexpr (KV_LDS) wait_vmcnt<0>();
+  asm volatile("s_waitcnt lgkmcnt(0)\n\ts_barrier" ::: "memory");
+  if (!unit) return;
+
+  const float sc = qp.scale * 1.4426950408889634f;
+  f16x8 qf[DKS];
+#pragma unroll
+  for (int ks = 0; ks < DKS; ++ks) qf[ks] = *(const f16x8*)(smem + OFF_Q + (urow * 32 + l31) * QP + (uhead * D + ks * 16 + lg * 8) * 2);
+  CA ca;
+  ca.begin();
+  if constexpr (KV_LDS) {
+    for (int t = 0; t < nt; ++t) {
+      const unsigned char* Ks = smem + t * KV_STAGE;
+      const unsigned char* Vs = Ks + KROWS * 128;
+      ca.tile(qf, [&](int kvb, int ks) { return *(const f16x8*)(Ks + ((ks >> 2) * 64 + kvb * 32 + l31) * 128 + ((((ks & 3) * 2 + lg) ^ rsw) << 4)); },
+              [&](int kvb, int s2, int dt) { return *(const f16x8*)(Vs + (dt * 32 + l31) * 128 + (((4 * kvb + 2 * s2 + lg) ^ rsw) << 4)); },
+              t * KVT, qp.nkv, sc, lg);
+    }
+  } else {
+    ca.tile(qf, [&](int kvb, int ks) { return __builtin_bit_cast(f16x8, kfa[kvb][ks]); },
+            [&](int kvb, int s2, int dt) { return __builtin_bit_cast(f16x8, vfa[kvb][s2][dt]); }, 0, qp.nkv, sc, lg);
+    if (nt > 1)
+      ca.tile(qf, [&](int kvb, int ks) { return __builtin_bit_cast(f16x8, kfb[kvb][ks]); },
+              [&](int kvb, int s2, int dt) { return __builtin_bit_cast(f16x8, vfb[kvb][s2][dt]); }, KVT, qp.nkv, sc, lg);
+  }
+  ca.finish(qp.out + (size_t)(m0 + urow * 32 + l31) * p.N + (size_t)head * D, lg);
+#endif
+}
+
+constexpr int QC_NS = 4;
+
+template <int BM, int D>
+void q_ctx_launch(const QCtxParams& q, hipStream_t stream) {
+  const dim3 grid((q.g.M / BM) * (q.g.N / QC_BN)), block(5 * 64);
+  SDMI_LAUNCH((q_ctx_kernel<BM, D, QC_NS>), grid, block, 0, stream, q);
+}
+
+}
+
+int q_ctx_row_block(int bm) {
+  if (bm <= 0) bm = env_int("SDMI_Q_CTX_BM", 32);
+  return bm;
+}
+
+bool q_ctx_supported(const QCtxParams& q) {
+  const IGemmParams& p = q.g;
+  const int bm = q_ctx_row_block(q.bm);
+  auto al16 = [](const void* x) { return ((uintptr_t)x & 15) == 0; };
+  return (bm == 32 || bm == 64) && (p.dh == 80 || p.dh == 160) && p.heads > 0 && p.N == p.heads * p.dh && p.K == p.N && p.N % QC_BN == 0 &&
+         p.K % BK == 0 && p.K <= 1280 && p.ksize == 1 && !p.split16 && p.a1 == nullptr && p.a2 == nullptr && p.c0 == p.K && p.lda0 == p.K &&
+         p.ntok > 0 && p.ntok % bm == 0 && p.M > 0 && p.M % p.ntok == 0 && (int64_t)p.M * p.K * 2 < ((int64_t)1 << 31) &&
+         (int64_t)p.N * p.K * 2 < ((int64_t)1 << 31) && (p.lnf_part == nullptr || (p.lnf_npart == p.K / 32 && p.lnf_cs && p.lnf_d && !p.bias)) &&
+         q.nkv >= 1 && q.nkv <= 128 && q.nkv_pad % 8 == 0 && q.nkv_pad >= q.nkv && al16(p.a0) && al16(p.w) && al16(q.ctx_k) && al16(q.ctx_vt) &&
+         ((uintptr_t)q.out & 7) == 0;
+}
+
+int launch_q_ctx(const QCtxParams& qp, hipStream_t stream) {
+  SDMI_CHECK(qp.g.a0 && qp.g.w && qp.ctx_k && qp.ctx_vt && qp.out, "q_ctx: null operand");
+  SDMI_CHECK(q_ctx_supported(qp), "q_ctx: head dim 80 / 160, N = K = heads * dh a multiple of 160, rows per sample a multiple of the row block "
+                                  "(32 / 64), 1 .. 128 context keys, V^T rows padded to a multiple of 8");
+  QCtxParams q = qp;
+  IGemmParams& p = q.g;
+  const int bm = q_ctx_row_block(q.bm);
+  q.bm = bm;
+  p.mode = EPI_HEADS; p.splitk = 1; p.nkt = p.K / BK;
+  p.tile_n_fastest = tile_order_n_fastest(p);
+  static const int by_shape = env_int("SDMI_PROF_SHAPES", 0);
+  std::string pname = std::string("igemm_qctx_") + std::to_string(bm) + "x160w5s" + std::to_string(QC_NS);
+  if (by_shape && prof_enabled())
+    pname += "_M" + std::to_string(p.M) + "_N" + std::to_string(p.N) + "_K" + std::to_string(p.K) + "_k1_m2_s1";
+  ProfScope ps(pname.c_str(), 2.0 * p.M * (double)p.N * p.K,
+               (double)p.M * p.K * 2.0 + (double)p.N * p.K * 2.0 + 2.0 * (p.M / p.ntok) * (double)q.nkv * p.N * 2.0 + (double)p.M * p.N * 2.0, stream);
+  if (bm == 32) { if (p.dh == 80) q_ctx_launch<32, 80>(q, stream); else q_ctx_launch<32, 160>(q, stream); }
+  else { if (p.dh == 80) q_ctx_launch<64, 80>(q, stream); else q_ctx_launch<64, 160>(q, stream); }
+  SDMI_HIP_OK(hipGetLastError());
+  ps.end();
+  if (range_check_enabled()) return range_scan("attention output", q.out, (int64_t)p.M * p.N, stream);
+  return 0;
+}
+
+}
diff --git a/stable-diffusion_amd/csrc/rowchain.hip b/stable-diffusion_amd/csrc/rowchain.hip
--- a/stable-diffusion_amd/csrc/rowchain.hip
+++ b/stable-diffusion_amd/csrc/rowchain.hip
@@ -1,5 +1,6 @@
 #include <utility>
 
+#include "ctx_attn.h"
 #include "igemm_dev.h"
 
 namespace sdmi {
@@ -436,17 +437,6 @@
 }
 
 
-typedef float f32x2 __attribute__((ext_vector_type(2)));
-#if defined(__HIP_DEVICE_COMPILE__)
-__device__ __forceinline__ void rc_swap_halves(float& a, float& b) {
-  asm volatile("s_nop 1\n\tv_permlane32_swap_b32 %0, %1\n\ts_nop 1" : "+v"(a), "+v"(b));
-}
-__device__ __forceinline__ float rc_max_across_halves(float x) {
-  float a = x, b = x;
-  rc_swap_halves(a, b);
-  return fmaxf(a, b);
-}
-#endif
 constexpr int SH_NU = 2 * FT_BLK + 3 * FT_BLK;
 struct ShUnitTab { int soff[2][SH_NU]; int sel[2][SH_NU]; };
 constexpr ShUnitTab sh_make_tab() {
@@ -763,7 +753,7 @@
 #pragma unroll
       for (int r = 0; r < 16; ++r) {
         const float2 mr = ltab[(r & 3) + 8 * (r >> 2) + 4 * lg];
-        a[j][r] = fmaf(mr.y, a[j][r] - mr.x * cs_[j], dn_[j]);
+        a[j][r] = lnf_apply(a[j][r], mr, cs_[j], dn_[j]);
       }
   };
   auto rows_out = [&](f32x16 (&a)[2], f16* dst) {
@@ -785,7 +775,8 @@
   SH_STAMP();
   if constexpr (KIND == 1 && CTX) {
     static_assert(C == 320, "head dim 40: eight heads of five 16-byte chunks");
-    constexpr int D = 40, DKS = 3, DVT = 2, KVT = 64;
+    using CA = CtxAttn<40>;
+    constexpr int D = 40, DKS = CA::DKS, DVT = CA::DVT, KVT = CA::KVT;
     const float sc = rp.ctx_scale * 1.4426950408889634f;
     const int nt = (rp.ctx_nkv + KVT - 1) / KVT;
     const int nheads = (rp.heads - wave + RC_NWC - 1) / RC_NWC;
@@ -793,29 +784,10 @@
     auto load_frags = [&](int i, u32x4 (&kf)[2][DKS], u32x4 (&vf)[2][2][DVT]) {
       const int head = wave + RC_NWC * (nt == 2 ? (i >> 1) : i), t = nt == 2 ? (i & 1) : 0;
       const int bh = bsample * rp.heads + head;
-      const __amdgpu_buffer_rsrc_t rsrc_k = __builtin_amdgcn_make_buffer_rsrc((void*)(rp.ctx_k + (size_t)bh * rp.ctx_nkv * D), 0, rp.ctx_nkv * D * 2, 0x00020000);
-      const __amdgpu_buffer_rsrc_t rsrc_v = __builtin_amdgcn_make_buffer_rsrc((void*)(rp.ctx_vt + (size_t)bh * D * rp.ctx_nkv_pad), 0, D * rp.ctx_nkv_pad * 2, 0x00020000);
-#pragma unroll
-      for (int kvb = 0; kvb < 2; ++kvb) {
-        const int row = kvb * 32 + l31;
-        const int key = t * KVT + ((row & ~12) | ((row & 4) << 1) | ((row & 8) >> 1));
-#pragma unroll
-        for (int ks = 0; ks < DKS; ++ks) kf[kvb][ks] = __builtin_amdgcn_raw_buffer_load_b128(rsrc_k, key * (D * 2) + (ks * 2 + lg) * 16, 0, 0);
-#pragma unroll
-        for (int s2 = 0; s2 < 2; ++s2)
-#pragma unroll
-          for (int dt = 0; dt < DVT; ++dt) {
-            const int d = dt * 32 + l31;
-            const unsigned one2 = d == D ? 0x3C003C00u : 0u;
-            u32x4 v = {one2, one2, one2, one2};
-            if (d < D) v = __builtin_amdgcn_raw_buffer_load_b128(rsrc_v, d * (rp.ctx_nkv_pad * 2) + t * (KVT * 2) + (4 * kvb + 2 * s2 + lg) * 16, 0, 0);
-            vf[kvb][s2][dt] = v;
-          }
-      }
+      ctx_load_frags<D>(rp.ctx_k + (size_t)bh * rp.ctx_nkv * D, rp.ctx_vt + (size_t)bh * D * rp.ctx_nkv_pad, rp.ctx_nkv, rp.ctx_nkv_pad, t, l31, lg, kf, vf);
     };
     f16x8 qf[DKS];
-    f32x16 o[DVT];
-    float m_run = -1e30f;
+    CA ca;
     auto step = [&](int i, const u32x4 (&kf)[2][DKS], const u32x4 (&vf)[2][2][DVT]) {
       const int head = wave + RC_NWC * (nt == 2 ? (i >> 1) : i), t = nt == 2 ? (i & 1) : 0;
       if (t == 0) {
@@ -826,83 +798,11 @@
           if (dcol < D) v = *(const f16x8*)(smem + OFF_XN + strip_off(l31, head * D + dcol));
           qf[ks] = v;
         }
-#pragma unroll
-        for (int dt = 0; dt < DVT; ++dt)
-#pragma unroll
-          for (int r = 0; r < 16; ++r) o[dt][r] = 0.f;
-        m_run = -1e30f;
-      }
-      f32x16 sa[2];
-#pragma unroll
-      for (int kvb = 0; kvb < 2; ++kvb) {
-#pragma unroll
-        for (int r = 0; r < 16; ++r) sa[kvb][r] = 0.f;
-#pragma unroll
-        for (int ks = 0; ks < DKS; ++ks)
-          sa[kvb] = __builtin_amdgcn_mfma_f32_32x32x16_f16(__builtin_bit_cast(f16x8, kf[kvb][ks]), qf[ks], sa[kvb], 0, 0, 0);
-      }
-      const int kv0 = t * KVT;
-      if (kv0 + KVT > rp.ctx_nkv) {
-#pragma unroll
-        for (int kvb = 0; kvb < 2; ++kvb)
-#pragma unroll
-          for (int r = 0; r < 16; ++r) {
-            const int kv = kv0 + kvb * 32 + (r & 3) + 4 * ((r >> 2) & 1) + 8 * lg + 16 * (r >> 3);
-            if (kv >= rp.ctx_nkv) sa[kvb][r] = -1e30f;
-          }
-      }
-      float mx = -1e30f;
-#pragma unroll
-      for (int kvb = 0; kvb < 2; ++kvb)
-#pragma unroll
-        for (int r = 0; r < 16; ++r) mx = fmaxf(mx, sa[kvb][r]);
-      mx = rc_max_across_halves(mx);
-      const float m_new = fmaxf(m_run, mx * sc);
-      if (__any(m_new > m_run)) {
-        const float alpha = __builtin_amdgcn_exp2f(m_run - m_new);
-        m_run = m_new;
-#pragma unroll
-        for (int dt = 0; dt < DVT; ++dt)
-#pragma unroll
-          for (int r = 0; r < 16; ++r) o[dt][r] *= alpha;
-      }
-      const f32x2 sc2 = {sc, sc}, nm2 = {-m_run, -m_run};
-#pragma unroll
-      for (int kvb = 0; kvb < 2; ++kvb)
-#pragma unroll
-        for (int r = 0; r < 16; r += 2) {
-          const f32x2 sv = {sa[kvb][r], sa[kvb][r + 1]};
-          const f32x2 e = __builtin_elementwise_fma(sv, sc2, nm2);
-          sa[kvb][r] = __builtin_amdgcn_exp2f(e[0]);
-          sa[kvb][r + 1] = __builtin_amdgcn_exp2f(e[1]);
-        }
-#pragma unroll
-      for (int kvb = 0; kvb < 2; ++kvb)
-#pragma unroll
-        for (int s2 = 0; s2 < 2; ++s2) {
-          f16x8 pf;
-#pragma unroll
-          for (int e = 0; e < 8; ++e) pf[e] = (f16)sa[kvb][8 * s2 + e];
-#pragma unroll
-          for (int dt = 0; dt < DVT; ++dt)
-            o[dt] = __builtin_amdgcn_mfma_f32_32x32x16_f16(__builtin_bit_cast(f16x8, vf[kvb][s2][dt]), pf, o[dt], 0, 0, 0);
-        }
-      if (t == nt - 1) {
-        float la = o[D / 32][4], lb = la;
-        rc_swap_halves(la, lb);
-        const float inv = 1.0f / la;
-        f16* orow = rp.ao_out + (size_t)(m0 + l31) * C + (size_t)head * D;
-#pragma unroll
-        for (int dt = 0; dt < DVT; ++dt)
-#pragma unroll
-          for (int r4 = 0; r4 < 4; ++r4) {
-            const int dd = dt * 32 + 8 * r4 + 4 * lg;
-            if (dd < D) {
-              const f16x4 v = {(f16)(o[dt][r4 * 4 + 0] * inv), (f16)(o[dt][r4 * 4 + 1] * inv), (f16)(o[dt][r4 * 4 + 2] * inv), (f16)(o[dt][r4 * 4 + 3] * inv)};
-              SDMI_ST(f16x4, orow + dd, v);
-            }
-          }
-      }
+        ca.begin();
+      }
+      ca.tile(qf, [&](int kvb, int ks) { return __builtin_bit_cast(f16x8, kf[kvb][ks]); },
+              [&](int kvb, int s2, int dt) { return __builtin_bit_cast(f16x8, vf[kvb][s2][dt]); }, t * KVT, rp.ctx_nkv, sc, lg);
+      if (t == nt - 1) ca.finish(rp.ao_out + (size_t)(m0 + l31) * C + (size_t)head * D, lg);
     };
     u32x4 kfa[2][DKS], vfa[2][2][DVT], kfb[2][DKS], vfb[2][2][DVT];
     if (nsteps > 0) load_frags(0, kfa, vfa);
diff --git a/stable-diffusion_amd/csrc/unet.cpp b/stable-diffusion_amd/csrc/unet.cpp
--- a/stable-diffusion_amd/csrc/unet.cpp
+++ b/stable-diffusion_amd/csrc/unet.cpp
@@ -21,6 +21,7 @@
 thread_local Tape* g_tape_rec = nullptr;
 
 namespace {
+constexpr bool SDMI_Q_CTX_DEFAULT = true;
 uint64_t sdmi_env_hash() {
   uint64_t h = 1469598103934665603ull;
   for (char** e = environ; e && *e; ++e) {
@@ -402,6 +403,7 @@
   bool st_mid_on = false;
   bool st_tail_on = false;
   bool st_mid_ctx_on = false;
+  bool q_ctx_on = false;
   bool ctx1_on = false;
   bool gn_conv_on = false;
   float* emb_all = nullptr;
@@ -674,8 +676,14 @@
         p.mode = EPI_HEADS; p.seg_dst[0] = q; p.seg_kind[0] = 0;
         p.heads = L.heads; p.dh = L.dh; p.ntok = N; p.ntok_pad = Np; p.segC = C; p.splitk = 1;
         fold_in(p, T.lnf[2], T.lnf[3]);
-        gemm(p);
-        attention(q, T.ck, T.cvt, ao, L, N, Lctx, Lp, scale);
+        QCtxParams qc = QCtxParams();
+        qc.g = p; qc.ctx_k = T.ck; qc.ctx_vt = T.cvt; qc.nkv = Lctx; qc.nkv_pad = Lp; qc.scale = scale; qc.out = ao;
+        if (q_ctx_on && (L.dh == 80 || L.dh == 160) && Lctx <= 128 && N % q_ctx_row_block(0) == 0 && q_ctx_supported(qc)) {
+          if (!dry && !rc) ok(launch_q_ctx(qc, s));
+        } else {
+          gemm(p);
+          attention(q, T.ck, T.cvt, ao, L, N, Lctx, Lp, scale);
+        }
       }
       if (!chain_tail) {
         IGemmParams p = dense(ao, M, C, T.wo2, C, N);
@@ -1035,12 +1043,14 @@
     f.st_tail_on = e_st ? atoi(e_st) != 0 : ff_tail_;
     const char* e_mc = getenv("SDMI_ST_MID_CTX");
     f.st_mid_ctx_on = e_mc ? atoi(e_mc) != 0 : st_head_;
+    const char* e_qc = getenv("SDMI_Q_CTX");
+    f.q_ctx_on = e_qc ? atoi(e_qc) != 0 : SDMI_Q_CTX_DEFAULT;
     const char* e_c1 = getenv("SDMI_CTX1");
     f.ctx1_on = !(e_c1 && atoi(e_c1) == 0);
     const char* e_gc = getenv("SDMI_GN_CONV");
     f.gn_conv_on = e_gc ? atoi(e_gc) != 0 : false;
     if (full()) {
-      f.ln_fold_on = f.ff_tail_on = f.st_head_on = f.st_mid_on = f.st_tail_on = f.st_mid_ctx_on = f.gn_conv_on = false;
+      f.ln_fold_on = f.ff_tail_on = f.st_head_on = f.st_mid_on = f.st_tail_on = f.st_mid_ctx_on = f.q_ctx_on = f.gn_conv_on = false;
     }
   }
   int64_t persist_bytes = 0, scratch_bytes = 0;
```
